# CWBudde/go-pocket-tts

Measured on AMD Instinct MI355X. Metric: synthesized audio sec/sec (xRT), higher is better.
Workload: dtype bf16; 1 GPU; b64_10s_bf16: 64 utterances/GPU x 125 frames (10.0 s each), 25-token prompt + 125-frame voice state, greedy (temperature 0), hipGraph-captured AR step, Mimi decode to 24 kHz PCM written to host; batch_per_gpu=64, frames=125, weights=BF16, kv=bf16, checkpoint=synthetic, shapes of tts_b6369a24 (seed 1234)

## Files before the change

go-pocket-tts_amd/csrc/attn_window.hip:

```cpp
#include <cstdlib>
#include <type_traits>

#include "common.h"
#include "kernels.h"
#include "device_util.h"
#include "mfma_util.h"

namespace ptts {

template <bool KVBF16, bool RAGGED>
__global__ __launch_bounds__(256) void k_attn_window(AttnArgs a, int qtiles) {
    const int lane = threadIdx.x & 63, wave = threadIdx.x >> 6;
    const int h = blockIdx.x;
    const int groups = (qtiles + 3) >> 2;
    const int seg = blockIdx.y / groups, qt = (blockIdx.y % groups) * 4 + wave;
    if (qt >= qtiles) return;
    const int r0 = qt * 32;
    const int seg_row0 = RAGGED ? a.rag_off[seg] : seg * a.rows_per_seg;
    const int seg_rows = RAGGED ? a.rag_off[seg + 1] - seg_row0 : a.rows_per_seg;
    if (r0 >= seg_rows) return;
    const int nq = min(32, seg_rows - r0);
    const int j = lane & 31, half = lane >> 5;
    const int my_q = min(j, nq - 1);
    const int p_first = (RAGGED ? a.rag_pos0[seg] : a.pos_base) + r0, p_last = p_first + nq - 1;
    const int my_pos = p_first + my_q;
    const int ctx = a.context > 0 ? a.context : (1 << 30);
    const int j_lo = max(0, p_first - ctx + 1);
    const RowMap qm{a.q_ld, a.q_rows_per_batch, a.q_batch_stride}, om{a.out_ld, a.o_rows_per_batch, a.o_batch_stride};
    const int row = seg_row0 + r0 + my_q;

    Frag qh[4], ql[4];
    {
        const float* qp = a.q + row_off(qm, row) + a.q_col0 + h * 64 + half * 8;
#pragma unroll
        for (int i = 0; i < 4; i++) {
            const float4 t0 = *reinterpret_cast<const float4*>(qp + 16 * i), t1 = *reinterpret_cast<const float4*>(qp + 16 * i + 4);
            split2(t0.x * 0.125f, t0.y * 0.125f, qh[i].u[0], ql[i].u[0]);
            split2(t0.z * 0.125f, t0.w * 0.125f, qh[i].u[1], ql[i].u[1]);
            split2(t1.x * 0.125f, t1.y * 0.125f, qh[i].u[2], ql[i].u[2]);
            split2(t1.z * 0.125f, t1.w * 0.125f, qh[i].u[3], ql[i].u[3]);
        }
    }
    typedef typename std::conditional<KVBF16, unsigned short, float>::type KvT;
    const KvT* kb = (const KvT*)a.k + (int64_t)seg * a.k_seg_stride + (int64_t)h * a.k_head_stride;
    const KvT* vb = (const KvT*)a.v + (int64_t)seg * a.k_seg_stride + (int64_t)h * a.k_head_stride;
    f32x16 o0, o1;
#pragma unroll
    for (int r = 0; r < 16; r++) { o0[r] = 0.0f; o1[r] = 0.0f; }
    float m = -INFINITY, l = 0.0f;

    for (int kt = j_lo; kt <= p_last; kt += 32) {
        Frag kh[4], kl[4];
        {
            const KvT* kp = kb + (int64_t)min(kt + j, p_last) * a.k_row_stride + half * 8;
            if constexpr (KVBF16) {
#pragma unroll
                for (int i = 0; i < 4; i++) kh[i].q = *reinterpret_cast<const uint4*>(kp + 16 * i);
            } else {
                float4 t[4][2];
#pragma unroll
                for (int i = 0; i < 4; i++) {
                    t[i][0] = *reinterpret_cast<const float4*>(kp + 16 * i);
                    t[i][1] = *reinterpret_cast<const float4*>(kp + 16 * i + 4);
                }
#pragma unroll
                for (int i = 0; i < 4; i++) split8(t[i][0], t[i][1], kh[i], kl[i]);
            }
        }
        float v0[16], v1[16];
#pragma unroll
        for (int r = 0; r < 16; r++) {
            const int key = min(kt + (r & 3) + 8 * (r >> 2) + 4 * half, p_last);
            const KvT* vp = vb + (int64_t)key * a.k_row_stride + j;
            if constexpr (KVBF16) {
                v0[r] = __uint_as_float((unsigned)vp[0] << 16);
                v1[r] = __uint_as_float((unsigned)vp[32] << 16);
            } else {
                v0[r] = vp[0];
                v1[r] = vp[32];
            }
        }
        f32x16 s;
#pragma unroll
        for (int r = 0; r < 16; r++) s[r] = 0.0f;
#pragma unroll
        for (int i = 0; i < 4; i++) {
            s = __builtin_amdgcn_mfma_f32_32x32x16_bf16(kh[i].v, qh[i].v, s, 0, 0, 0);
            if constexpr (!KVBF16) PTTS_LO_MFMA(s = __builtin_amdgcn_mfma_f32_32x32x16_bf16(kl[i].v, qh[i].v, s, 0, 0, 0));
            PTTS_LO_MFMA(s = __builtin_amdgcn_mfma_f32_32x32x16_bf16(kh[i].v, ql[i].v, s, 0, 0, 0));
        }
        float tmax = -INFINITY;
#pragma unroll
        for (int r = 0; r < 16; r++) {
            const int key = kt + (r & 3) + 8 * (r >> 2) + 4 * half;
            const bool ok = key <= my_pos && key > my_pos - ctx;
            s[r] = ok ? s[r] : -INFINITY;
            tmax = fmaxf(tmax, s[r]);
        }
        tmax = fmaxf(tmax, __shfl_xor(tmax, 32, WAVE));
        const float m_new = fmaxf(m, tmax);
        const float m_use = m_new == -INFINITY ? 0.0f : m_new;
        const float alpha = __expf(m - m_use);
        m = m_new;
        l *= alpha;
#pragma unroll
        for (int r = 0; r < 16; r++) { o0[r] *= alpha; o1[r] *= alpha; }
#pragma unroll
        for (int r = 0; r < 16; r++) {
            s[r] = __expf(s[r] - m_use);
            l += s[r];
        }
#pragma unroll
        for (int i = 0; i < 2; i++) {
            Frag ph, pl, vh0, vl0, vh1, vl1;
#pragma unroll
            for (int e = 0; e < 4; e++) {
                split2(s[8 * i + 2 * e], s[8 * i + 2 * e + 1], ph.u[e], pl.u[e]);
                split2(v0[8 * i + 2 * e], v0[8 * i + 2 * e + 1], vh0.u[e], vl0.u[e]);
                split2(v1[8 * i + 2 * e], v1[8 * i + 2 * e + 1], vh1.u[e], vl1.u[e]);
            }
            o0 = __builtin_amdgcn_mfma_f32_32x32x16_bf16(vh0.v, ph.v, o0, 0, 0, 0);
            if constexpr (!KVBF16) PTTS_LO_MFMA(o0 = __builtin_amdgcn_mfma_f32_32x32x16_bf16(vl0.v, ph.v, o0, 0, 0, 0));
            PTTS_LO_MFMA(o0 = __builtin_amdgcn_mfma_f32_32x32x16_bf16(vh0.v, pl.v, o0, 0, 0, 0));
            o1 = __builtin_amdgcn_mfma_f32_32x32x16_bf16(vh1.v, ph.v, o1, 0, 0, 0);
            if constexpr (!KVBF16) PTTS_LO_MFMA(o1 = __builtin_amdgcn_mfma_f32_32x32x16_bf16(vl1.v, ph.v, o1, 0, 0, 0));
            PTTS_LO_MFMA(o1 = __builtin_amdgcn_mfma_f32_32x32x16_bf16(vh1.v, pl.v, o1, 0, 0, 0));
// ... 227 lines not shown
```

go-pocket-tts_amd/csrc/batch.cpp:

```cpp
#include "launch_args.h"

#include <algorithm>
#include <cmath>

namespace ptts {

Batch::~Batch() {
    if (fc_stamps.p) {
        constexpr int kWg = 8 * kFlowClusterMaxTiles;
        std::vector<unsigned long long> h((size_t)kWg * 64);
        if (const char* path = getenv("PTTS_FC_STAMPS"))
            if (hipDeviceSynchronize() == hipSuccess && hipMemcpy(h.data(), fc_stamps.p, h.size() * 8, hipMemcpyDeviceToHost) == hipSuccess)
                if (FILE* f = fopen(path, "a")) {
                    for (int blk = 0; blk < kWg; blk++) {
                        if (!h[(size_t)blk * 64]) continue;
                        fprintf(f, "wg %d:", blk);
                        for (int i = 0; i < 64; i++) fprintf(f, " %llu", h[(size_t)blk * 64 + i]);
                        fprintf(f, "\n");
                    }
                    fprintf(f, "\n");
                    fclose(f);
                }
    }
    drop_graphs();
    if (n_active_pinned) (void)hipHostFree(n_active_pinned);
    if (rows_pinned) (void)hipHostFree(rows_pinned);
}

void Batch::drop_graphs() {
    for (auto& set : graphs) for (auto& row : set) for (hipGraphExec_t& g : row) if (g) { (void)hipGraphExecDestroy(g); g = nullptr; }
    for (auto& gs : graph_steps) gs[0] = gs[1] = 0;
}

Batch* batch_new(Model& m, int n_slots, int cap, int max_steps) {
    if (n_slots <= 0) throw Error(PTTS_EINVAL, "ptts-hip: batch needs at least one slot");
    if (n_slots > kStepMaxRows) throw Error(PTTS_EINVAL, strfmt("ptts-hip: a batch takes at most %d slots (the AR step's kernels), asked for %d", kStepMaxRows, n_slots));
    if (cap <= 0 || cap > ROPE_SEQ) throw Error(PTTS_EINVAL, strfmt("ptts-hip: kv capacity %d outside (0, %d] (RoPE table rows, flow_transformer.go:505)", cap, ROPE_SEQ));
    m.use_device();
    const Desc& d = m.d;
    std::unique_ptr<Batch> b(new Batch());
    b->m = &m;
    b->B = n_slots;
    b->cap = cap;
    b->max_steps = std::max(1, max_steps);
    const size_t B = (size_t)n_slots;
    size_t kvbytes = (size_t)d.n_layers * B * d.heads * cap * d.hd * b->kv_elem();
    b->kcache.ensure(kvbytes);
    b->vcache.ensure(kvbytes);
    PTTS_HIP(hipMemsetAsync(b->kcache.p, 0, kvbytes, m.stream));
    PTTS_HIP(hipMemsetAsync(b->vcache.p, 0, kvbytes, m.stream));
    b->state_i32.ensure((9 * B + 1) * sizeof(int32_t));
    b->state_f32.ensure(B * sizeof(float));
    int32_t* s = b->state_i32.as<int32_t>();
    b->st.kv_len = s; b->st.active = s + B; b->st.step = s + 2 * B; b->st.countdown = s + 3 * B;
    b->st.n_frames = s + 4 * B; b->st.eos_step = s + 5 * B; b->st.max_steps = s + 6 * B;
    b->st.frames_after_eos = s + 7 * B; b->st.broke = s + 8 * B; b->st.n_active = s + 9 * B;
    b->st.eos_threshold = b->state_f32.as<float>();
    b->kv_len_host.assign(B, 0);
    b->pre_k.ensure((size_t)B * sizeof(void*)); b->pre_v.ensure((size_t)B * sizeof(void*)); b->pre_len.ensure((size_t)B * sizeof(int32_t));
    b->pre_k_host.assign(B, nullptr); b->pre_v_host.assign(B, nullptr); b->pre_len_host.assign(B, 0);
    const size_t f = sizeof(float);
    const int NA = d.ada_all.out;
    b->in_raw.ensure(B * d.ldim * f); b->in32.ensure(B * d.ldim * f);
    b->x.ensure(B * d.d_model * f); b->xn.ensure(B * std::max(d.d_model, d.flow_dim) * f);
    b->qkv.ensure(B * 3 * d.d_model * f); b->attn.ensure(B * d.d_model * f);
    b->ff.ensure(B * d.ffn * f); b->last.ensure(B * d.d_model * f); b->eos.ensure(B * f);
    b->sy.ensure(B * d.flow_dim * f); b->ada.ensure(B * NA * f);
    b->fx.ensure(B * d.flow_dim * f); b->fh.ensure(B * d.flow_dim * f); b->fh2.ensure(B * d.flow_dim * f);
    b->cur.ensure(B * d.ldim * f);
    b->partial.ensure((size_t)16 * B * std::max(d.d_model, d.flow_dim) * f);
    b->latents.ensure(B * b->max_steps * d.ldim * f);
    {
        StepFinish sf{b->st, b->eos.as<float>(), b->latents.as<float>(), (int64_t)b->max_steps * d.ldim, (int32_t)d.ldim, StepChain{}};
        StepOpenLinears lin;
        b->chain_ok = open_linears(*b, lin) && step_open_mfma_ok(lin, d.ldim) && ((int64_t)b->max_steps * d.ldim) % 2 == 0 &&
                      (lin.w_bf16 != 0) == (d.final_linear.bf16 != 0 || d.final_linear.wt_i8 != 0);
        b->fx2.ensure(B * d.flow_dim * f); b->cur2.ensure(B * d.ldim * f);
        StepFinish sf2[2] = {sf, sf};
        sf2[0].ch = StepChain{lin.w_in, lin.b_in, lin.x, lin.d_in, lin.w_pj, lin.b_pj, b->fx2.as<float>(), lin.d_pj, m.at<float>(d.bos), b->cur2.as<float>(), lin.w_bf16, b->chain_ok ? 1 : 0};
        sf2[1].ch = StepChain{lin.w_in, lin.b_in, lin.x, lin.d_in, lin.w_pj, lin.b_pj, b->fx.as<float>(), lin.d_pj, m.at<float>(d.bos), b->cur.as<float>(), lin.w_bf16, b->chain_ok ? 1 : 0};
        b->fin_dev.ensure(sizeof sf2);
        h2d(b->fin_dev.p, sf2, sizeof sf2, m.stream);
    }
    {
        const char* sw = getenv("PTTS_FLOW_CLUSTER");
        const bool off = sw && sw[0] == '0';
        bool ok = !off && !m.fc_disabled.load() && d.flow_dim == 512 && d.flow_depth > 0 && d.flow_depth <= FC_MAX_DEPTH && n_slots <= kStepMaxRows &&
                  flow_cluster_fits(n_slots, m.device);
        for (int r = 0; ok && r < d.flow_depth; r++) {
            const auto& rb = d.rb[r];
            for (const Lin* l : {&rb.mlp0, &rb.mlp2}) ok = ok && l->in == 512 && l->out == 512 && l->bf16 && !l->wt_i8 && l->wt != NONE && l->b != NONE;
            ok = ok && rb.ln.w != NONE && rb.ln.b != NONE && rb.ln.d == 512;
        }
        b->fc_ok = ok;
        if (ok) {
            b->fc_xbuf.ensure(flow_cluster_xbuf_bytes(n_slots)); b->fc_sync.ensure(kFlowClusterSyncBytes);
            PTTS_HIP(hipMemsetAsync(b->fc_xbuf.p, 0, flow_cluster_xbuf_bytes(n_slots), m.stream));
            PTTS_HIP(hipMemsetAsync(b->fc_sync.p, 0, kFlowClusterSyncBytes, m.stream));
            if (getenv("PTTS_FC_STAMPS")) { b->fc_stamps.ensure((size_t)8 * kFlowClusterMaxTiles * 64 * 8); PTTS_HIP(hipMemsetAsync(b->fc_stamps.p, 0, (size_t)8 * kFlowClusterMaxTiles * 64 * 8, m.stream)); }
        }
    }
    {
        const char* sw = getenv("PTTS_TALL");
        bool ok = !(sw && sw[0] == '0') && n_slots >= kTallMinRows && (d.d_model == 512 || d.d_model == 1024) && d.ffn % 128 == 0;
        for (int l = 0; ok && l < d.n_layers; l++) {
            const auto& L = d.layers[l];
            for (const Lin* li : {&L.in_proj, &L.l1, &L.l2}) ok = ok && li->bf16 && !li->wt_i8 && li->wt != NONE && li->out % 4 == 0;
            ok = ok && L.in_proj.in == d.d_model && L.l1.in == d.d_model && L.l1.out == d.ffn && L.l2.in == d.ffn && L.l2.out == d.d_model;
            ok = ok && L.n1.w != NONE && L.n1.b != NONE && L.n2.w != NONE && L.n2.b != NONE;
        }
        b->tall_ok = ok;
        if (ok) { b->tp_a.ensure(2 * B * d.d_model * sizeof(uint16_t)); b->tp_f.ensure(2 * B * d.ffn * sizeof(uint16_t)); }
    }
    PTTS_HIP(hipHostMalloc((void**)&b->n_active_pinned, sizeof(int32_t) * (size_t)(2 + 2 * B), hipHostMallocDefault));
    PTTS_HIP(hipHostMalloc((void**)&b->rows_pinned, sizeof(PcmRow) * std::max<size_t>((size_t)B, 1), hipHostMallocDefault));
    batch_reset(*b);
    return b.release();
}

void batch_reset(Batch& b) {
    b.opened = false;
    hipStream_t s = b.m->stream;
    const int B = b.B;
    launch_fill_i32(b.st.kv_len, 0, B, s);
    b.kv_bound = 0;
    PTTS_HIP(hipMemsetAsync(b.latents.p, 0, (size_t)B * b.max_steps * b.m->d.ldim * sizeof(float), s));
    launch_fill_i32(b.st.active, 1, B, s);
    launch_fill_i32(b.st.step, 0, B, s);
    launch_fill_i32(b.st.countdown, -1, B, s);
    launch_fill_i32(b.st.n_frames, 0, B, s);
    launch_fill_i32(b.st.eos_step, -1, B, s);
    launch_fill_i32(b.st.max_steps, 0x7fffffff, B, s);
    launch_fill_i32(b.st.frames_after_eos, 0, B, s);
    launch_fill_i32(b.st.broke, 0, B, s);
    launch_fill_i32(b.st.n_active, B, 1, s);
    std::vector<float> thr((size_t)B, INFINITY);
    h2d(b.st.eos_threshold, thr.data(), thr.size() * sizeof(float), s);
    std::fill(b.kv_len_host.begin(), b.kv_len_host.end(), 0);
    std::fill(b.pre_len_host.begin(), b.pre_len_host.end(), 0);
    launch_fill_i32(b.pre_len.as<int32_t>(), 0, B, s);
    b.has_noise = false;
}

static void check_voice(const Desc& d, const float* const* caches, const int64_t* steps, const int64_t* offsets, int64_t cap) {
    for (int l = 0; l < d.n_layers; l++) {
        if (!caches[l]) throw Error(PTTS_EINVAL, strfmt("native: voice model state module \"transformer.layers.%d.self_attn\" missing cache", l));
        if (offsets[l] < 0) throw Error(PTTS_EINVAL, strfmt("native: voice model state module \"transformer.layers.%d.self_attn\" has negative offset %lld", l, (long long)offsets[l]));
        if (offsets[l] > steps[l]) throw Error(PTTS_EINVAL, strfmt("native: voice model state module \"transformer.layers.%d.self_attn\" offset %lld exceeds cache length %lld", l, (long long)offsets[l], (long long)steps[l]));
        if (offsets[l] != offsets[0]) throw Error(PTTS_EINVAL, "ptts-hip: per-layer voice offsets differ; one offset per utterance is supported");
        if (offsets[l] > cap) throw Error(PTTS_EINVAL, "ptts-hip: voice state longer than the KV capacity");
    }
}

Voice* voice_create(Model& m, const float* const* caches, const int64_t* steps, const int64_t* offsets) {
    const Desc& d = m.d;
    check_voice(d, caches, steps, offsets, ROPE_SEQ);
    std::unique_ptr<Voice> v(new Voice());
    v->m = &m;
    v->device = m.device;
    v->offset = (int)offsets[0];
    const size_t lb = v->layer_bytes();
    v->k.ensure(std::max<size_t>(lb * d.n_layers, 256));
    v->v.ensure(std::max<size_t>(lb * d.n_layers, 256));
    for (int l = 0; l < d.n_layers; l++) {
        size_t n = (size_t)2 * steps[l] * d.heads * d.hd;
        DevBuf& raw = m.work(WORK_VOICE_RAW, n * sizeof(float));
        h2d(raw.p, caches[l], n * sizeof(float), m.stream);
        launch_voice_scatter(raw.as<float>(), (int)steps[l], d.heads, d.hd, v->offset, 0, (char*)v->k.p + lb * l, (char*)v->v.p + lb * l,
                             m.opts.kv == PTTS_KV_BF16, v->offset, m.stream);
        PTTS_HIP(hipStreamSynchronize(m.stream));
    }
    return v.release();
}

bool voice_usable_by(const Voice& v, const Model& m) {
    return v.m == &m || (v.m && v.m->device == m.device && v.m->opts.kv == m.opts.kv && v.m->d.n_layers == m.d.n_layers && v.m->d.heads == m.d.heads &&
                         v.m->d.hd == m.d.hd);
}

void batch_apply_voice(Batch& b, const Voice& v, const std::vector<int32_t>& slots) {
    Model& m = *b.m;
    hipStream_t io = b.io_stream ? b.io_stream : m.stream;
    const Desc& d = m.d;
    if (!voice_usable_by(v, m)) throw Error(PTTS_EINVAL, "ptts-hip: voice belongs to another model");
    if (v.offset > b.cap) throw Error(PTTS_EINVAL, "ptts-hip: voice state longer than the KV capacity");
    DevBuf& ds = m.work(WORK_VOICE_SLOTS, slots.size() * sizeof(int32_t));
    h2d(ds.p, slots.data(), slots.size() * sizeof(int32_t), io);
    const size_t lb = v.layer_bytes();
    for (int l = 0; l < d.n_layers; l++)
        launch_voice_apply((const char*)v.k.p + lb * l, (const char*)v.v.p + lb * l, v.offset, d.heads, d.hd, ds.as<int32_t>(), (int)slots.size(),
                           b.kc(l), b.vc(l), (int)b.kv_elem(), b.cap, io);
    for (int32_t sl : slots) {
        b.kv_len_host[sl] = v.offset;
        b.kv_bound = std::max(b.kv_bound, (int)v.offset);
        b.pre_k_host[sl] = v.k.p; b.pre_v_host[sl] = v.v.p; b.pre_len_host[sl] = v.offset;
    }
    if (b.slot_local) return;
    h2d(b.st.kv_len, b.kv_len_host.data(), (size_t)b.B * sizeof(int32_t), io);
    h2d(b.pre_k.p, b.pre_k_host.data(), (size_t)b.B * sizeof(void*), io);
    h2d(b.pre_v.p, b.pre_v_host.data(), (size_t)b.B * sizeof(void*), io);
    h2d(b.pre_len.p, b.pre_len_host.data(), (size_t)b.B * sizeof(int32_t), io);
}

void batch_set_voice(Batch& b, int slot, const float* const* caches, const int64_t* steps, const int64_t* offsets) {
    Model& m = *b.m;
    hipStream_t io = b.io_stream ? b.io_stream : m.stream;
    const Desc& d = m.d;
    if (slot < 0 || slot >= b.B) throw Error(PTTS_EINVAL, "ptts-hip: voice state slot out of range");
    check_voice(d, caches, steps, offsets, b.cap);
    for (int l = 0; l < d.n_layers; l++) {
        size_t n = (size_t)2 * steps[l] * d.heads * d.hd;
        DevBuf& raw = m.work(WORK_VOICE_RAW, n * sizeof(float));
        h2d(raw.p, caches[l], n * sizeof(float), io);
        launch_voice_scatter(raw.as<float>(), (int)steps[l], d.heads, d.hd, (int)offsets[l], slot, b.kc(l), b.vc(l),
                             m.opts.kv == PTTS_KV_BF16, b.cap, io);
        PTTS_HIP(hipStreamSynchronize(io));
    }
    b.kv_len_host[slot] = (int32_t)offsets[0];
    b.kv_bound = std::max(b.kv_bound, (int)offsets[0]);
    b.pre_len_host[slot] = 0;
    if (b.slot_local) return;
    h2d(b.st.kv_len + slot, &b.kv_len_host[slot], sizeof(int32_t), io);
    h2d(b.pre_len.as<int32_t>() + slot, &b.pre_len_host[slot], sizeof(int32_t), io);
}

void batch_prompt(Batch& b, const float* rows_dev, const int64_t* row_offsets) {
    Model& m = *b.m;
    const Desc& d = m.d;
    hipStream_t s = b.io_stream ? b.io_stream : m.stream;
    const int B = b.B, D = d.d_model;
    const int64_t R64 = row_offsets[B];
    if (R64 == 0) return;
    if (R64 < 0 || R64 > (1 << 24)) throw Error(PTTS_EINVAL, "ptts-hip: prompt row count out of range");
    const int R = (int)R64;
    std::vector<int32_t> off((size_t)B + 1);
    for (int sl = 0; sl < B; sl++) {
        int64_t t = row_offsets[sl + 1] - row_offsets[sl];
        if (t < 0) throw Error(PTTS_EINVAL, "ptts-hip: prompt row offsets must be non-decreasing");
        if (b.kv_len_host[sl] + t > b.cap) throw Error(PTTS_EINVAL, strfmt("ptts-hip: prompt of %lld rows does not fit KV capacity %d (offset %d)", (long long)t, b.cap, b.kv_len_host[sl]));
        off[(size_t)sl] = (int32_t)row_offsets[sl];
    }
    off[(size_t)B] = R;
    const size_t f = sizeof(float);
    const RaggedMeta meta = ragged_meta(off.data(), b.kv_len_host.data(), B);
    int32_t* d_meta = m.work(WORK_PROMPT_META, meta.table.size() * sizeof(int32_t)).as<int32_t>();
    const int32_t* d_slot = meta.row_seg(d_meta);
    const int32_t* d_pos = meta.row_pos(d_meta);
    h2d(d_meta, meta.table.data(), meta.table.size() * sizeof(int32_t), s);
    DevBuf& wsb = m.work(WORK_PROMPT_ACT, ((size_t)R * (size_t)(D + D + 3 * D + D + d.ffn)) * f);
    float* px = wsb.as<float>();
    float* pxn = px + (size_t)R * D;
    float* pqkv = pxn + (size_t)R * D;
    float* pattn = pqkv + (size_t)R * 3 * D;
    float* pff = pattn + (size_t)R * D;
    PTTS_HIP(hipMemcpyAsync(px, rows_dev, (size_t)R * D * f, hipMemcpyDeviceToDevice, s));
    const bool kvb = m.opts.kv == PTTS_KV_BF16;
    PendingSum pend;
    for (int l = 0; l < d.n_layers; l++) {
        const auto& L = d.layers[l];
        {
            LnArgs ln = mkln(m, px, flat(D), L.n1, pxn, D, R);
            ln.pend = pend;
            launch_layernorm(ln, s);
            pend = PendingSum{};
        }
        {
            GemmArgs gq = mk(m, pxn, flat(D), L.in_proj, pqkv, flat(3 * D), R);
            gq.rope_cos = m.at<float>(d.rope_cos); gq.rope_sin = m.at<float>(d.rope_sin);
            gq.rope_cols = 2 * D; gq.rope_hd = d.hd; gq.rope_row_pos = d_pos;
            if (!launch_gemm_rope(gq, s)) {
                gq.rope_cos = gq.rope_sin = nullptr; gq.rope_row_pos = nullptr;
                launch_gemm(gq, s);
                launch_rope_rows(pqkv, flat(3 * D), 0, d.heads, d.hd, d_pos, 0, 0, R, m.at<float>(d.rope_cos), m.at<float>(d.rope_sin), s);
                launch_rope_rows(pqkv, flat(3 * D), D, d.heads, d.hd, d_pos, 0, 0, R, m.at<float>(d.rope_cos), m.at<float>(d.rope_sin), s);
            }
        }
        launch_kv_append(pqkv, 3 * D, D, d.heads, d.hd, d_slot, d_pos, R, b.kc(l), b.vc(l), kvb, b.cap, s);
        if (l == d.n_layers - 1) break;
        launch_attention(attn_ragged_args(kv_layer(b, l), meta, d_meta, pqkv, 3 * D, -1, pattn, D), s);
        GemmArgs go = mk(m, pattn, flat(D), L.out_proj, px, flat(D), R);
        go.R = px; go.epi = EPI_RESADD;
        launch_gemm(go, s);
        launch_layernorm(mkln(m, px, flat(D), L.n2, pxn, D, R), s);
        GemmArgs g1 = mk(m, pxn, flat(D), L.l1, pff, flat(d.ffn), R);
        g1.epi = EPI_GELU;
        launch_gemm(g1, s);
        GemmArgs g2 = mk(m, pff, flat(d.ffn), L.l2, px, flat(D), R);
        const int S = R <= kSkinnyChunkRows ? pick_split(std::min(R, 64), D, d.ffn) : 1;
        GemmArgs g2c = g2;
        g2c.M = std::min(R, 64);
        if (S > 1 && skinny_supported(g2c, S)) {
            DevBuf& pb = m.work(WORK_PREFILL_PLANES, (size_t)S * R * D * f);
            for (int r0 = 0; r0 < R; r0 += 64) {
                g2c = g2;
                g2c.M = std::min(64, R - r0);
                g2c.A = g2.A + (int64_t)r0 * d.ffn;
                g2c.zstride = (int64_t)R * D;
                launch_skinny(g2c, SkinnyFuse{}, S, pb.as<float>() + (size_t)r0 * D, s);
            }
            pend = PendingSum{pb.as<float>(), S, (int64_t)R * D, m.at<float>(L.l2.b)};
        } else {
            GemmArgs gs = g2;
            gs.bias = nullptr; gs.kslice = 1024; gs.zstride = (int64_t)R * D;
            const int Sg = (d.ffn + gs.kslice - 1) / gs.kslice;
            if (R < 16384 && Sg > 1 && Sg <= 8) {
                DevBuf& pb = m.work(WORK_PREFILL_PLANES, (size_t)Sg * R * D * f);
                gs.C = pb.as<float>(); gs.cmap = flat(D);
                if (gemm5_supported(gs) || gemm3_supported(gs)) {
                    if (gemm5_supported(gs)) launch_gemm5(gs, s);
                    else launch_gemm3(gs, s);
                    pend = PendingSum{pb.as<float>(), Sg, (int64_t)R * D, m.at<float>(L.l2.b)};
                    continue;
                }
            }
            g2.R = px; g2.epi = EPI_RESADD;
            launch_gemm(g2, s);
        }
    }
    for (int sl = 0; sl < B; sl++) {
        b.kv_len_host[sl] += (int32_t)(row_offsets[sl + 1] - row_offsets[sl]);
        b.kv_bound = std::max(b.kv_bound, (int)b.kv_len_host[sl]);
    }
    if (!b.slot_local) h2d(b.st.kv_len, b.kv_len_host.data(), (size_t)B * sizeof(int32_t), s);
}

}
```

go-pocket-tts_amd/csrc/capi_hooks.cpp:

```cpp
#include "capi_internal.h"
#include "launch_args.h"
#include "../../include/ptts_debug.h"
#include "scan_block.h"
#include "true_peak.h"

#include <memory>

using namespace ptts;
using namespace ptts::capi;

namespace {

template <class T> class Scoped {
    T& var_;
    T old_;
public:
    Scoped(T& var, T value) : var_(var), old_(var) { var = value; }
    ~Scoped() { var_ = old_; }
    Scoped(const Scoped&) = delete;
    Scoped& operator=(const Scoped&) = delete;
};

using Census = std::map<std::string, int64_t>;

// ... 243 lines not shown
        }
        dsp_windows_device(*h->m, in, n, rows, spec, cuts, n_cuts, out);
    });
}

int ptts_debug_loudness_energies(ptts_model* h, const float* const* in, const int64_t* n, int32_t rows, double* const* out) {
    return guard([&] {
        if (rows < 0 || (rows > 0 && (!in || !n || !out))) throw Error(PTTS_EINVAL, "ptts-hip: loudness: null argument");
        for (int i = 0; i < rows; i++)
            if (n[i] < 0 || (n[i] > 0 && !in[i]) || (n[i] >= kLoudSub && !out[i])) throw Error(PTTS_EINVAL, strfmt("ptts-hip: loudness: row %d is negative or null", i));
        std::vector<std::vector<double>> sub((size_t)rows);
        if (h) {
            if (!h->m) throw Error(PTTS_EINVAL, "native: model is not fully initialized");
            DspSpec spec;
            dsp_spec_loudness(spec, nullptr);
            dsp_rows_device(*h->m, in, n, rows, std::vector<DspSpec>((size_t)rows, spec).data(), false, {nullptr, nullptr, sub.data()});
        } else {
            for (int i = 0; i < rows; i++) loud_sub_energies(in[i], n[i], sub[(size_t)i]);
        }
        for (int i = 0; i < rows; i++)
            if (n[i] >= kLoudSub) std::memcpy(out[i], sub[(size_t)i].data(), (size_t)(n[i] / kLoudSub) * sizeof(double));
    });
}

int ptts_debug_kweighting(int32_t sample_rate, double out[10]) {
    return guard([&] {
        if (!out || sample_rate <= 0) throw Error(PTTS_EINVAL, "ptts-hip: loudness: bad argument");
        loud_kweight_coeffs(sample_rate, out);
    });
}

int64_t ptts_debug_dsp_opts_error(const ptts_dsp_opts* opts, char* out, int64_t cap) {
    const std::string s = opts ? dsp_opts_error(*opts) : std::string();
    put_str(out, cap, s);
    return (int64_t)s.size();
}

int ptts_debug_true_peak_taps(float* out, int32_t* L, int32_t* K, int32_t* dlo) {
    if (L) *L = kTpPhases;
    if (K) *K = kTpTaps;
    if (dlo) *dlo = kTpDlo;
    const TpTaps& t = tp_taps();
    if (out)
        for (int p = 0; p < kTpPhases; p++)
            for (int k = 0; k < kTpTaps; k++) out[p * kTpTaps + k] = t.h[k][p];
    return PTTS_OK;
}

int ptts_debug_true_peak_oversample(const float* samples, int64_t n, float* y) {
    return guard([&] {
        if (n < 0 || (n > 0 && (!samples || !y))) throw Error(PTTS_EINVAL, "ptts-hip: true peak: null argument");
        (void)tp_measure(samples, n, y);
    });
}

int64_t ptts_debug_launch_counts(int32_t on, char* out, int64_t cap) {
    static thread_local Census census;
    const std::string s = census_str(census);
    put_str(out, cap, s);
    census.clear();
    g_launch_census = on ? &census : nullptr;
    return (int64_t)s.size();
}

int ptts_debug_time_skinny(int32_t M, int32_t N, int32_t K, int32_t w_bf16, int32_t splitk, int32_t fuse_ln, int32_t iters, float* avg_us) {
    return guard([&] {
        require_device();
        SkinnyProbe p(M, N, K, w_bf16, splitk, fuse_ln);
        hipEvent_t e0, e1;
        PTTS_HIP(hipEventCreate(&e0)); PTTS_HIP(hipEventCreate(&e1));
        for (int i = 0; i < 5; i++) p.launch(splitk);
        PTTS_HIP(hipDeviceSynchronize());
        PTTS_HIP(hipEventRecord(e0, nullptr));
        for (int i = 0; i < iters; i++) p.launch(splitk);
        PTTS_HIP(hipEventRecord(e1, nullptr));
        PTTS_HIP(hipEventSynchronize(e1));
        float ms = 0;
        PTTS_HIP(hipEventElapsedTime(&ms, e0, e1));
        *avg_us = ms * 1e3f / (float)iters;
        (void)hipEventDestroy(e0); (void)hipEventDestroy(e1);
    });
}

int ptts_debug_skinny_stamps(int32_t M, int32_t N, int32_t K, int32_t w_bf16, int32_t splitk, int32_t fuse_ln, uint64_t* out, int32_t max_blocks,
                             int32_t* n_blocks) {
    return guard([&] {
        require_device();
        SkinnyProbe p(M, N, K, w_bf16, splitk, fuse_ln);
        const int blocks = ((N + 15) / 16) * ((M + 15) / 16) * (splitk > 1 ? splitk : 1);
        Tmp dS((size_t)blocks * 8 * 8);
        PTTS_HIP(hipMemset(dS.p, 0, (size_t)blocks * 64));
        for (int i = 0; i < 3; i++) p.launch(splitk);
        PTTS_HIP(hipDeviceSynchronize());
        {
            Scoped<unsigned long long*> stamped(g_skinny_stamps, dS.as<unsigned long long>());
            p.launch(splitk);
        }
        PTTS_HIP(hipDeviceSynchronize());
        *n_blocks = blocks;
        down(out, dS.p, (size_t)std::min(blocks, max_blocks) * 64);
    });
}

int ptts_debug_step_stamps(ptts_batch* hb, int32_t lsd_steps, uint64_t* out, int64_t cap_blocks, int32_t* desc, int32_t cap_desc, int32_t* n_desc) {
    return guard([&] {
        if (!hb || !hb->b || !out || !desc || !n_desc) throw Error(PTTS_EINVAL, "ptts-hip: null argument");
// ... 894 lines not shown
```

go-pocket-tts_amd/csrc/continuous.cpp:

```cpp
#include <algorithm>
#include <chrono>
#include <cmath>
#include <deque>
#include <map>
#include <mutex>

#include "runtime.h"

namespace ptts {

namespace {
constexpr int kDecoderShare = 2;
constexpr int kDecodeMin = 16;
constexpr int kDecodeSerialFrames = 2400;
constexpr int kDecodeMaxAge = 8;
constexpr int kBandFrames = 16, kBandPercent = 48;

std::mutex g_dec_mu;
std::map<int, std::pair<hipStream_t, int>> g_dec_streams;
hipStream_t decoder_stream_acquire(int device) {
    std::lock_guard<std::mutex> lock(g_dec_mu);
    auto& ent = g_dec_streams[device];
    if (!ent.first) {
        int cus = 0, cur = 0;
// ... 160 lines not shown
        e->dec = decoder_stream_acquire(m.device);
    }
    b.io_stream = e->io;
    for (DevBuf& db : e->adm_dev) db.ensure((size_t)slots * sizeof(SlotAdmit));
    e->stage.ensure((size_t)2 * slots * b.max_steps * m.d.ldim * sizeof(float));
    for (int i = 2 * slots - 1; i >= 0; i--) e->stage_free.push_back(i);
    PTTS_HIP(hipEventCreateWithFlags(&e->ev_steps, hipEventDisableTiming));
    for (hipEvent_t& ev : e->lat_free) PTTS_HIP(hipEventCreateWithFlags(&ev, hipEventDisableTiming));
    for (DevBuf& l : e->lat) l.ensure((size_t)2 * slots * (size_t)max_steps * m.d.ldim * sizeof(float));
    PTTS_HIP(hipHostMalloc((void**)&e->rows_host, sizeof(PcmRow) * ContEngine::kLat * 2 * (size_t)slots, hipHostMallocDefault));
    e->rows_dev.ensure(sizeof(PcmRow) * ContEngine::kLat * 2 * (size_t)slots);
    m.tcomb_for(1);
    { MimiWs w; mimi_setup(m, w, 1, kFramesPerDecode + kFramesPerDecode / 8); }
    m.work(WORK_CONT_PCM, (size_t)(kFramesPerDecode + kFramesPerDecode / 8) * m.d.samples_per_frame * sizeof(float));
    m.work(WORK_EGRESS_S16, (size_t)(kFramesPerDecode + kFramesPerDecode / 8) * m.d.samples_per_frame * sizeof(int16_t));
    m.work(WORK_CONT_RESERVE, (size_t)(kFramesPerDecode + kFramesPerDecode / 8) * m.d.ldim * sizeof(float));
    static const int env_graph = [] { const char* g = getenv("PTTS_GRAPH"); return g ? atoi(g) : -1; }();
    e->use_graph = env_graph >= 0 ? env_graph != 0 : m.opts.use_graph != 0;
    PTTS_HIP(hipStreamSynchronize(m.stream));
    return e.release();
}

void cont_destroy(ContEngine* e) { delete e; }
int cont_free_slots(const ContEngine& e) { return e.free_slots(); }
int cont_busy(const ContEngine& e) { return e.busy(); }
void cont_counts(const ContEngine& e, int64_t* admissions, int64_t* admitted) { *admissions = e.admissions; *admitted = e.admitted; }
void cont_occupancy(const ContEngine& e, int64_t* steps, int64_t* slot_steps) { *steps = e.steps_run; *slot_steps = e.slot_steps; }

bool cont_accepts(const ContEngine& e, const ptts_request& r) {
    if (r.step_callback || r.pcm_callback || r.lsd_steps > 1) return false;
    const int ms = resolve_max_steps(r);
    const int tp = (int)r.n_tokens + (r.voice_embedding ? (int)r.voice_frames : 0);
    const int off = r.voice ? reinterpret_cast<const Voice*>(r.voice)->offset : (r.voice_caches ? (int)r.voice_offsets[0] : 0);
    return ms <= e.max_steps && off + tp + ms <= e.cap && ms <= mimi_frame_limit(e.m.d);
}

void cont_admit(ContEngine& e, const ptts_request* const* reqs, ptts_result* const* results, void* const* tags, int n) {
    struct Timer { ContEngine& e; std::chrono::steady_clock::time_point t0 = std::chrono::steady_clock::now();
                   ~Timer() { e.tr_acc_admit_us += std::chrono::duration<double, std::micro>(std::chrono::steady_clock::now() - t0).count(); } } admit_timer{e};
    if (n <= 0) return;
    e.lock_model();
    Batch& b = *e.b;
    hipStream_t s = e.io;
    const int turn = e.arena_turn;
    e.arena_turn ^= 1;
    UploadScope upload_scope(e.arenas[turn], e.arena_free[turn]);
    std::vector<SlotReq> list((size_t)n);
    for (int i = 0, next = 0; i < n; i++, next++) {
        while (next < e.B && e.slots[(size_t)next].busy) next++;
        if (next >= e.B) throw Error(PTTS_EINVAL, "continuous batch: more requests admitted than free slots");
        list[(size_t)i] = SlotReq{next, reqs[i], resolve_max_steps(*reqs[i])};
        b.kv_len_host[(size_t)next] = 0;
        b.pre_k_host[(size_t)next] = nullptr; b.pre_v_host[(size_t)next] = nullptr; b.pre_len_host[(size_t)next] = 0;
    }
    stage_prompt(b, list, s);
    stage_noise(b, list, s);
    ContEngine::Joining j;
    std::vector<SlotAdmit> adm((size_t)n);
    for (int i = 0; i < n; i++) {
        const ptts_request& r = *reqs[i];
        const int sl = list[(size_t)i].slot;
        adm[(size_t)i] = SlotAdmit{sl, list[(size_t)i].max_steps, r.frames_after_eos, r.eos_threshold, b.kv_len_host[(size_t)sl], b.pre_len_host[(size_t)sl],
                                   b.pre_k_host[(size_t)sl], b.pre_v_host[(size_t)sl]};
        ContEngine::Slot& so = e.slots[(size_t)sl];
        so = ContEngine::Slot{};
        so.busy = true; so.req = reqs[i]; so.res = results[i]; so.tag = tags[i];
        so.ms = list[(size_t)i].max_steps;
        so.base_kv = b.kv_len_host[(size_t)sl];
        so.joining = true;
        j.slots.push_back(sl);
    }
    j.ring = e.adm_turn;
    e.adm_turn = (e.adm_turn + 1) & 3;
    h2d(e.adm_dev[j.ring].p, adm.data(), adm.size() * sizeof(SlotAdmit), s);
    j.ready = e.event();
    j.seq = e.seq;
    PTTS_HIP(hipEventRecord(j.ready, s));
    PTTS_HIP(hipEventRecord(e.arena_free[turn], s));
    e.joining.push_back(std::move(j));
    e.admissions++;
    e.admitted += n;
    e.tr_admitted += n;
    e.last_admit_seq = e.seq;
}

static void activate_ready(ContEngine& e, bool wait) {
    Batch& b = *e.b;
    while (!e.joining.empty()) {
        ContEngine::Joining& j = e.joining.front();
        if (wait) PTTS_HIP(hipEventSynchronize(j.ready));
        else {
            hipError_t q = hipEventQuery(j.ready);
            if (q == hipErrorNotReady) {
                PTTS_HIP(hipStreamWaitEvent(e.m.stream, j.ready, 0));
            } else if (q != hipSuccess) throw Error(PTTS_ENODEVICE, strfmt("hip: hipEventQuery failed: %s", hipGetErrorString(q)));
        }
        launch_slot_admit(b.st, b.pre_len.as<int32_t>(), b.pre_k.as<const void*>(), b.pre_v.as<const void*>(), e.adm_dev[j.ring].as<SlotAdmit>(), (int)j.slots.size(),
                          e.m.stream);
        b.opened = false;
        for (int sl : j.slots) { e.slots[(size_t)sl].joining = false; e.slots[(size_t)sl].admit_seq = e.seq; e.slots[(size_t)sl].seen_seq = e.seq; }
        e.n_gen += (int)j.slots.size();
        e.free_events.push_back(j.ready);
        e.joining.pop_front();
    }
}

static void start_decode(ContEngine& e, std::vector<ContEngine::Staged>& fin) {
    Model& m = e.m;
    Batch& b = *e.b;
// ... 249 lines not shown
```

go-pocket-tts_amd/csrc/generate.cpp:

```cpp
#include "runtime.h"

#include <chrono>

#include <algorithm>
#include <cmath>

namespace ptts {

void stage_prompt(Batch& b, const std::vector<SlotReq>& list, hipStream_t s, hipEvent_t before_prefill) {
    Model& m = *b.m;
    const int D = m.d.d_model;
    std::map<const Voice*, std::vector<int32_t>> by_voice;
    for (const SlotReq& q : list) {
        if (q.req->voice) by_voice[reinterpret_cast<const Voice*>(q.req->voice)].push_back(q.slot);
        else if (q.req->voice_caches) batch_set_voice(b, q.slot, q.req->voice_caches, q.req->voice_cache_steps, q.req->voice_offsets);
    }
    for (auto& kv : by_voice) batch_apply_voice(b, *kv.first, kv.second);
    std::vector<int64_t> row_off((size_t)b.B + 1, 0), ids;
    for (const SlotReq& q : list) {
        row_off[(size_t)q.slot + 1] = q.req->n_tokens + (q.req->voice_embedding ? q.req->voice_frames : 0);
        ids.insert(ids.end(), q.req->tokens, q.req->tokens + q.req->n_tokens);
    }
    for (int sl = 0; sl < b.B; sl++) row_off[(size_t)sl + 1] += row_off[(size_t)sl];
    DevBuf& rows = m.work(WORK_PROMPT_ROWS, (size_t)row_off[(size_t)b.B] * D * sizeof(float));
    DevBuf& dids = m.work(WORK_PROMPT_IDS, ids.size() * sizeof(int64_t));
    h2d(dids.p, ids.data(), ids.size() * sizeof(int64_t), s);
    int64_t id0 = 0, run_id0 = 0, run_n = 0;
    float* run_dst = rows.as<float>();
    auto flush = [&]() {
        if (run_n > 0) launch_embed_gather(m.at<float>(m.d.embed), dids.as<int64_t>() + run_id0, (int)run_n, D, run_dst, s);
        run_n = 0;
    };
    for (const SlotReq& q : list) {
        const ptts_request& r = *q.req;
        float* dst = rows.as<float>() + row_off[(size_t)q.slot] * D;
        const int64_t tv = r.voice_embedding ? r.voice_frames : 0;
        if (tv) {
            flush();
            h2d(dst, r.voice_embedding, (size_t)tv * D * sizeof(float), s);
        }
        if (run_n == 0) { run_id0 = id0; run_dst = dst + tv * D; }
        run_n += r.n_tokens;
        id0 += r.n_tokens;
    }
    flush();
    if (before_prefill) PTTS_HIP(hipEventRecord(before_prefill, s));
    batch_prompt(b, rows.as<float>(), row_off.data());
}

void stage_noise(Batch& b, const std::vector<SlotReq>& list, hipStream_t s) {
    Model& m = *b.m;
    const int ld = m.d.ldim;
    const int64_t slot_rows = (int64_t)b.max_steps * ld;
    float* noise = b.noise.as<float>();
    for (size_t i = 0; i < list.size();) {
        size_t j = i + 1;
        while (j < list.size() && list[j].slot == list[j - 1].slot + 1) j++;
        PTTS_HIP(hipMemsetAsync(noise + list[i].slot * slot_rows, 0, (j - i) * slot_rows * sizeof(float), s));
        i = j;
    }
    std::vector<NoiseSpec> spec((size_t)b.B, NoiseSpec{0, 0.0f, 0});
    int draw_rows = 0;
    for (const SlotReq& q : list) {
        const ptts_request& r = *q.req;
        if (r.noise) h2d(noise + q.slot * slot_rows, r.noise, (size_t)q.max_steps * ld * sizeof(float), s);
        else if (r.temperature > 0.0f) {
            if (ld % 4) throw Error(PTTS_EINVAL, "ptts-hip: the device noise draw needs a latent width that is a multiple of 4");
            spec[(size_t)q.slot] = NoiseSpec{r.noise_seed ? r.noise_seed : m.next_noise_seed(), std::sqrt(r.temperature), q.max_steps};
            draw_rows = std::max(draw_rows, q.max_steps);
        }
    }
    if (draw_rows == 0) return;
    DevBuf& sb = m.work(WORK_NOISE_SPECS, spec.size() * sizeof(NoiseSpec));
    h2d(sb.p, spec.data(), spec.size() * sizeof(NoiseSpec), s);
    launch_noise_fill(sb.as<NoiseSpec>(), b.B, draw_rows, noise, slot_rows, ld, s);
}

const PcmRow* results_alloc(const Model& m, const std::vector<Delivery>& g, PcmRow* host_rows, PcmRow* dev_rows, hipStream_t s) {
    const int64_t spf = m.d.samples_per_frame;
    bool all_pinned = true, converts = false;
    for (size_t i = 0; i < g.size(); i++) {
        if (host_rows) host_rows[i] = PcmRow{nullptr, 0, 0};
        const Delivery& u = g[i];
        if (!u.res || u.filled) continue;
        const int fmt = u.req->pcm_format;
        const bool s16 = fmt == PTTS_PCM_S16;
        const int64_t ns = egress_length(*u.req, u.samples(spf));
        void* p = result_alloc((size_t)std::max<int64_t>(1, ns) * pcm_bytes(fmt));
        set_result_buffer(*u.res, fmt, p);
        if (!p) continue;
        all_pinned = all_pinned && result_is_pinned(p);
        converts = converts || request_converts(*u.req);
        if (host_rows) host_rows[i] = PcmRow{p, (int32_t)std::min<int64_t>(ns, INT32_MAX), s16 ? 1 : 0};
    }
    if (!host_rows || !dev_rows || !all_pinned || converts) return nullptr;
    PTTS_HIP(hipMemcpyAsync(dev_rows, host_rows, g.size() * sizeof(PcmRow), hipMemcpyHostToDevice, s));
    return dev_rows;
}

void results_deliver(Model& m, const std::vector<Delivery>& g, bool stored, const float* pcm, int64_t pcm_stride, const float* lat, int64_t lat_stride,
                     hipStream_t s) {
    const int ld = m.d.ldim;
    const int64_t spf = m.d.samples_per_frame;
    const int64_t n = (int64_t)g.size();
    const int16_t* pcm16 = nullptr;
    std::vector<int64_t> conv;
    if (!stored) {
        std::vector<DspJob> jobs;
        for (int64_t i = 0; i < n; i++) {
            const Delivery& u = g[(size_t)i];
            if (u.res && !u.filled && u.samples(spf) > 0 && (u.req->dsp || u.req->loudness) && result_buffer(*u.res, u.req->pcm_format)) {
                DspJob j{const_cast<float*>(pcm) + i * pcm_stride, u.samples(spf), DspSpec()};
                const std::string e = dsp_resolve(u.req->dsp, &j.spec);
                if (!e.empty()) throw Error(PTTS_EINVAL, "ptts-hip: " + e);
                const double target_lufs = (double)u.req->loudness / 100.0;
                if (u.req->loudness) dsp_spec_loudness(j.spec, &target_lufs);
                if (j.spec.any()) jobs.push_back(j);
            }
        }
        if (!jobs.empty()) dsp_launch(m, jobs, s);
    }
    for (int64_t i = 0; i < n; i++) {
        const Delivery& u = g[(size_t)i];
        if (!u.res) continue;
        ptts_result& r = *u.res;
        const int fmt = u.req->pcm_format;
        r.n_frames = u.nf; r.eos_step = u.eos; r.n_samples = egress_length(*u.req, u.samples(spf));
        const bool s16 = fmt == PTTS_PCM_S16;
// ... 111 lines not shown
    std::chrono::steady_clock::time_point t_last = std::chrono::steady_clock::now();

    ~Chunk() {
        (void)hipStreamSynchronize(m.stream2);
        (void)hipStreamSynchronize(m.stream);
        for (auto& r : stream_ranges) (void)hipHostFree(r->nf);
        for (void* p : stream_host) result_free(p);
    }
    const ptts_request& req(int i) const { return reqs[idx[(size_t)i]]; }
    Error too_long(int frames) const {
        return Error(PTTS_EINVAL, strfmt("generate: mimi_decode: ops: rope cos/sin sequence length too small for pos=0 seq=%lld", (long long)frames * m.d.up_stride));
    }
    void mark(const char* what) {
        static const bool trace = getenv("PTTS_TRACE") != nullptr;
        if (!trace) return;
        (void)hipStreamSynchronize(s);
        (void)hipStreamSynchronize(m.stream2);
        auto now = std::chrono::steady_clock::now();
        fprintf(stderr, "[ptts] %-12s %8.3f ms\n", what, std::chrono::duration<double, std::milli>(now - t_last).count());
        t_last = now;
    }
    hipEvent_t phase_event(int i) {
        if (!m.prof.phases_on) return nullptr;
        if (!m.prof.phase[i]) PTTS_HIP(hipEventCreate(&m.prof.phase[i]));
        return m.prof.phase[i];
    }
    void phase(int i, hipStream_t st) { if (hipEvent_t e = phase_event(i)) PTTS_HIP(hipEventRecord(e, st)); }
    int slot_status(int i, int nf) const { return cancelled[(size_t)i] ? PTTS_ECANCELLED : nf > t_limit ? PTTS_EINVAL : PTTS_OK; }
    void setup(); void decoder_setup(); void ar_loop(); void deliver();
    void deliver_joined(const int32_t* nf, const int32_t* eos);
    void decode_upto(int f1, const PcmRow* rows = nullptr, bool* rows_used = nullptr);
    void decode_rest(int f1, const PcmRow* rows = nullptr, bool* rows_used = nullptr);
    void emit_upto(int f1, bool last = false);
};

void Chunk::setup() {
    int cap_need = 0;
    for (int i = 0; i < B; i++) {
        const ptts_request& r = req(i);
        const int ms = resolve_max_steps(r);
        const int tp = (int)r.n_tokens + (r.voice_embedding ? (int)r.voice_frames : 0);
        const int off = r.voice ? reinterpret_cast<const Voice*>(r.voice)->offset : (r.voice_caches ? (int)r.voice_offsets[0] : 0);
        list.push_back(SlotReq{i, &r, ms});
        cap_need = std::max(cap_need, off + tp + ms);
        ms_max = std::max(ms_max, ms);
    }
    int cap = (cap_need + 63) / 64 * 64;
    if (cap > ROPE_SEQ) throw Error(PTTS_EINVAL, strfmt("ops: rope cos/sin sequence length too small for pos=%d seq=1", cap_need));
    if (!m.cached_batch || m.cached_batch->B != B || m.cached_batch->cap < cap || m.cached_batch->max_steps < ms_max) {
        m.cached_batch.reset();
        m.cached_batch.reset(batch_new(m, B, cap, ms_max));
    }
    b = m.cached_batch.get();
    batch_reset(*b);
    std::vector<int32_t> v_ms((size_t)B), v_fae((size_t)B);
    std::vector<float> v_thr((size_t)B);
    for (int i = 0; i < B; i++) { v_ms[i] = std::min(list[i].max_steps, t_limit + 1); v_fae[i] = req(i).frames_after_eos; v_thr[i] = req(i).eos_threshold; }
    h2d(b->st.max_steps, v_ms.data(), (size_t)B * 4, s);
    h2d(b->st.frames_after_eos, v_fae.data(), (size_t)B * 4, s);
    h2d(b->st.eos_threshold, v_thr.data(), (size_t)B * 4, s);
    mark("setup");
    m.prof.phases = false;
    stage_prompt(*b, list, s, phase_event(0));
    phase(1, s);
    mark("prefill");
    b->has_noise = false;
    for (int i = 0; i < B; i++) b->has_noise |= req(i).noise != nullptr || req(i).temperature > 0.0f;
    if (!b->has_noise) return;
    b->noise.ensure((size_t)B * b->max_steps * ld * sizeof(float));
    stage_noise(*b, list, s);
}

void Chunk::decoder_setup() {
    T = std::min(ms_max, t_limit);
    pcm = &m.work(WORK_PCM, (size_t)B * T * spf * sizeof(float));
    const char* env_chunk = getenv("PTTS_MIMI_CHUNK");
    chunk = env_chunk && atoi(env_chunk) > 0 ? atoi(env_chunk) : 1 << 30;
    for (int i = 0; i < B; i++) streaming |= req(i).pcm_callback != nullptr;
    if (streaming) {
        chunk = 1 << 30;
        bool any_s16 = false;
        for (int i = 0; i < B; i++) {
            const ptts_request& r = req(i);
            if (!r.pcm_callback) continue;
            chunk = std::min(chunk, r.stream_frames > 0 ? (int)r.stream_frames : 12);
            const size_t bytes = (size_t)std::max<int64_t>(1, egress_length(r, (int64_t)list[i].max_steps * spf)) * pcm_bytes(r.pcm_format);
            stream_host[(size_t)i] = result_alloc(bytes);
            if (!stream_host[(size_t)i]) throw Error(PTTS_ENOMEM, "ptts-hip: out of host memory");
            const bool conv = request_converts(r);
            any_s16 |= r.pcm_format == PTTS_PCM_S16 && !conv;
            any_conv |= conv;
            if (conv) stage_row = std::max(stage_row, (bytes + 255) & ~(size_t)255);
        }
        if (any_s16) stream_s16 = &m.work(WORK_STREAM_S16, (size_t)B * T * spf * sizeof(int16_t));
        if (stage_row) stream_stage = m.work(WORK_STREAM_STAGE, stage_row * (size_t)B).as<char>();
    }
    dec_group = (B > kMimiGroup && !streaming && chunk > ms_max) ? kMimiGroup : B;
    mimi_setup(m, mw, dec_group, T);
    mimi_zero_history(m, mw, m.stream2);
}

void Chunk::ar_loop() {
    m.tcomb_for(lsd);
    static const int env_graph = [] { const char* e = getenv("PTTS_GRAPH"); return e ? atoi(e) : -1; }();
    const bool use_graph = (env_graph >= 0 ? env_graph != 0 : m.opts.use_graph != 0) && !m.prof.on;
    bool may_stop = false, any_cb = false, any_cancel_flag = false;
    for (int i = 0; i < B; i++) {
        may_stop |= req(i).eos_threshold < 1e30f;
        any_cb |= req(i).step_callback != nullptr;
        any_cancel_flag |= req(i).cancel != nullptr;
    }
    std::vector<int32_t> act((size_t)B, 1);
    static const int env_gsteps = [] { const char* e = getenv("PTTS_GRAPH_STEPS"); return e ? std::max(1, atoi(e)) : 0; }();
    const int gsteps = (use_graph && !any_cb && !any_cancel_flag && chunk > ms_max) ? (env_gsteps ? env_gsteps : (may_stop ? 5 : 25)) : 1;
    const int ms_loop = std::min(ms_max, t_limit + 1);
    for (int step = 0; step < ms_loop;) {
        int n_cancel = 0;
        for (int i = 0; i < B; i++) {
            const ptts_request& r = req(i);
            if (r.cancel && *r.cancel) cancelled[i] = 1;
            n_cancel += cancelled[i];
        }
        if (n_cancel == B) break;
// ... 595 lines not shown
```

go-pocket-tts_amd/csrc/kernels.h:

```cpp
#pragma once

#include <hip/hip_runtime.h>
#include <atomic>
#include <cstddef>
#include <cstdint>
#include <map>
#include <string>
#include <vector>

#include "deesser.h"
#include "limiter.h"
#include "pitch.h"
#include "tempo.h"
#include "trim.h"

namespace ptts {

struct RowMap {
    int64_t ld = 0;
    int64_t rows_per_batch = 0;
    int64_t batch_stride = 0;
};

enum AOp : int { AOP_NONE = 0, AOP_ELU = 1 };
// ... 436 lines not shown
};
constexpr int kFlowClusterRows = 12;
constexpr int kFlowClusterMaxTiles = (kStepMaxRows + kFlowClusterRows - 1) / kFlowClusterRows;
constexpr size_t kFlowClusterTileBytes = (size_t)2 * 16 * 512 * 8;
constexpr size_t kFlowClusterSyncBytes = (size_t)(32 * kFlowClusterMaxTiles + 32) * 4;
inline size_t flow_cluster_xbuf_bytes(int rows) { return (size_t)((rows + kFlowClusterRows - 1) / kFlowClusterRows) * kFlowClusterTileBytes; }
bool flow_cluster_fits(int rows, int device);
bool flow_cluster_supported(const FlowClusterArgs& a, int C);
void launch_flow_cluster(const FlowClusterArgs& a, hipStream_t stream, hipEvent_t ev0 = nullptr, hipEvent_t ev1 = nullptr);

struct StepState {
    int32_t* kv_len;
    int32_t* active;
    int32_t* step;
    int32_t* countdown;
    int32_t* n_frames;
    int32_t* eos_step;
    int32_t* max_steps;
    int32_t* frames_after_eos;
    float*   eos_threshold;
    int32_t* n_active;
    int32_t* broke;
};
struct StepChain {
    const void* w_in; const float* b_in; float* x; int32_t d_in;
    const void* w_pj; const float* b_pj; float* fx; int32_t d_pj;
    const float* bos; float* x0; int32_t w_bf16; int32_t ok;
};
struct StepFinish {
    StepState s;
    const float* eos_logit;
    float* latents;
    int64_t lat_stride;
    int32_t ldim;
    StepChain ch;
};
struct StepOpenLinears {
    const void* w_in = nullptr; const float* b_in = nullptr; int d_in = 0; float* x = nullptr;
    const void* w_pj = nullptr; const float* b_pj = nullptr; int d_pj = 0; float* fx = nullptr;
    int w_bf16 = 0;
};
bool step_open_mfma_ok(const StepOpenLinears& lin, int ldim);
void launch_step_begin(const StepState& s, const float* latents, int64_t lat_stride, const float* bos, const float* noise, int64_t noise_stride,
                       int ldim, int b, float* in32, float* x0, const StepOpenLinears* lin, hipStream_t stream);
void launch_step_finish(const StepState& s, const float* frame, const float* eos_logit, int ldim, int b, float* latents,
                        int64_t lat_stride, hipStream_t stream);
struct NoiseSpec { uint64_t seed; float sigma; int32_t rows; };
void launch_noise_fill(const NoiseSpec* spec_dev, int n_slots, int max_rows, float* out, int64_t out_stride, int ldim, hipStream_t stream);
struct GatherTable { struct Row { int32_t src_row, dst_off, nf, T; }; Row rows[128]; };
void launch_gather_frames(const GatherTable& t, int n, const float* stage, int64_t row_stride, float* dst, int ld, hipStream_t stream);
void launch_readback_i32(const int32_t* a, int na, const int32_t* b, int nb, int32_t* host, hipStream_t stream);
struct SlotAdmit { int32_t slot, max_steps, frames_after_eos; float eos_threshold; int32_t kv_len, pre_len; const void* pre_k; const void* pre_v; };
void launch_slot_admit(const StepState& s, int32_t* pre_len, const void** pre_k, const void** pre_v, const SlotAdmit* dev, int n, hipStream_t stream);
void launch_slot_retire(const StepState& s, const int32_t* slots_dev, int n, hipStream_t stream);
void launch_fill_i32(int32_t* p, int32_t v, int n, hipStream_t stream);
void launch_add_i32(int32_t* p, const int32_t* inc, int n, hipStream_t stream);

void launch_enc_head(const float* pcm, const void* w, int w_bf16, const float* b, int64_t L, int C, int k, float* out, int64_t ldo, hipStream_t stream);
int enc_ds_splits(int M, int N, int K);
void launch_enc_downsample(const float* A, int64_t lda, const void* W, int w_bf16, const float* bias, int M, int N, int K, float* partial, float* out,
                           hipStream_t stream);

void launch_bct_to_btc(const float* in, int b, int c, int t, float* out, int out_pad_rows, hipStream_t stream);
void launch_btc_to_bct(const float* in, int in_pad_rows, int b, int c, int t, float* out, hipStream_t stream);

}
```

go-pocket-tts_amd/csrc/kernels.hip:

```cpp
#include <cstdlib>
#include "kernels.h"
#include "device_util.h"
#include "gemm_tile.h"
#include "step_open.h"

namespace ptts {

constexpr int GM = 64, GN = 64, GK = 32, GLD = GK + 4;

template <bool WBF16>
__global__ __launch_bounds__(256) void k_gemm(GemmArgs a, int a_vec, int w_vec) {
    __shared__ __attribute__((aligned(16))) float As[GM * GLD];
    __shared__ __attribute__((aligned(16))) float Ws[GN * GLD];
    const int tid = threadIdx.x, lane = tid & 63, wave = tid >> 6;
    const int m0 = blockIdx.y * GM, n0 = blockIdx.x * GN;
    const int wm = wave >> 1, wn = wave & 1;

    int srow[2], sc4[2];
    const float* aptr[2];
    const char* wptr[2];
    bool arow_ok[2], wrow_ok[2];
#pragma unroll
    for (int i = 0; i < 2; i++) {
        int idx = tid + i * 256;
// ... 164 lines not shown
void launch_copy_rows(const float* src, int64_t lds, float* dst, int64_t ldd, int rows, int d, hipStream_t stream) {
    int64_t n = (int64_t)rows * d;
    if (n <= 0) return;
    hipLaunchKernelGGL(k_copy_rows, dim3((unsigned)((n + 255) / 256)), dim3(256), 0, stream, src, lds, dst, ldd, rows, d);
}

__global__ void k_timestep_features(float t, const float* freqs, int nf, float* out) {
    int i = blockIdx.x * blockDim.x + threadIdx.x;
    if (i >= nf) return;
    float arg = t * freqs[i];
    out[i] = (float)cos((double)arg);
    out[nf + i] = (float)sin((double)arg);
}
void launch_timestep_features(float t, const float* freqs, int nf, float* out, hipStream_t stream) {
    hipLaunchKernelGGL(k_timestep_features, dim3((nf + 63) / 64), dim3(64), 0, stream, t, freqs, nf, out);
}

__global__ void k_avg2(const float* a, const float* b, float* y, int n) {
    int i = blockIdx.x * blockDim.x + threadIdx.x;
    if (i < n) y[i] = (a[i] + b[i]) * 0.5f;
}
void launch_avg2(const float* a, const float* b, float* y, int n, hipStream_t stream) {
    hipLaunchKernelGGL(k_avg2, dim3((n + 255) / 256), dim3(256), 0, stream, a, b, y, n);
}

__global__ __launch_bounds__(256) void k_gather_frames(GatherTable t, const float* stage, int64_t row_stride, float* dst, int ld) {
    const GatherTable::Row r = t.rows[blockIdx.x];
    const float4* src = reinterpret_cast<const float4*>(stage + (int64_t)r.src_row * row_stride);
    float4* out = reinterpret_cast<float4*>(dst + r.dst_off);
    const int n_copy = r.nf * ld / 4, n_all = r.T * ld / 4;
    for (int i = threadIdx.x; i < n_all; i += 256) out[i] = i < n_copy ? src[i] : make_float4(0.f, 0.f, 0.f, 0.f);
}
void launch_gather_frames(const GatherTable& t, int n, const float* stage, int64_t row_stride, float* dst, int ld, hipStream_t stream) {
    if (n <= 0) return;
    hipLaunchKernelGGL(k_gather_frames, dim3((unsigned)n), dim3(256), 0, stream, t, stage, row_stride, dst, ld);
}

__global__ void k_readback_i32(const int32_t* a, int na, const int32_t* b, int nb, int32_t* host) {
    const int i = blockIdx.x * blockDim.x + threadIdx.x;
    if (i < na) host[i] = a[i];
    else if (i < na + nb) host[i] = b[i - na];
}
void launch_readback_i32(const int32_t* a, int na, const int32_t* b, int nb, int32_t* host, hipStream_t stream) {
    const int n = na + (b ? nb : 0);
    if (n <= 0) return;
    hipLaunchKernelGGL(k_readback_i32, dim3((unsigned)((n + 255) / 256)), dim3(256), 0, stream, a, na, b, b ? nb : 0, host);
}

__global__ void k_fill_i32(int32_t* p, int32_t v, int n) {
    int i = blockIdx.x * blockDim.x + threadIdx.x;
    if (i < n) p[i] = v;
}
void launch_fill_i32(int32_t* p, int32_t v, int n, hipStream_t stream) {
    hipLaunchKernelGGL(k_fill_i32, dim3((n + 255) / 256), dim3(256), 0, stream, p, v, n);
}
__global__ void k_add_i32(int32_t* p, const int32_t* inc, int n) {
    int i = blockIdx.x * blockDim.x + threadIdx.x;
    if (i < n) p[i] += inc[i];
}
void launch_add_i32(int32_t* p, const int32_t* inc, int n, hipStream_t stream) {
    hipLaunchKernelGGL(k_add_i32, dim3((n + 255) / 256), dim3(256), 0, stream, p, inc, n);
}

__global__ void k_slot_admit(StepState s, int32_t* pre_len, const void** pre_k, const void** pre_v, const SlotAdmit* a, int n) {
    const int i = blockIdx.x * blockDim.x + threadIdx.x;
    if (i >= n) return;
    const int sl = a[i].slot;
    s.kv_len[sl] = a[i].kv_len; pre_len[sl] = a[i].pre_len; pre_k[sl] = a[i].pre_k; pre_v[sl] = a[i].pre_v;
    s.active[sl] = 1; s.step[sl] = 0; s.countdown[sl] = -1; s.n_frames[sl] = 0; s.eos_step[sl] = -1; s.broke[sl] = 0;
    s.max_steps[sl] = a[i].max_steps; s.frames_after_eos[sl] = a[i].frames_after_eos; s.eos_threshold[sl] = a[i].eos_threshold;
    if (i == 0) atomicAdd(s.n_active, n);
}
void launch_slot_admit(const StepState& s, int32_t* pre_len, const void** pre_k, const void** pre_v, const SlotAdmit* dev, int n, hipStream_t stream) {
    if (n > 0) hipLaunchKernelGGL(k_slot_admit, dim3((n + 63) / 64), dim3(64), 0, stream, s, pre_len, pre_k, pre_v, dev, n);
}
__global__ void k_slot_retire(StepState s, const int32_t* slots, int n) {
    const int i = blockIdx.x * blockDim.x + threadIdx.x;
    if (i >= n) return;
    const int sl = slots[i];
    if (s.active[sl]) { s.active[sl] = 0; atomicSub(s.n_active, 1); }
}
void launch_slot_retire(const StepState& s, const int32_t* slots_dev, int n, hipStream_t stream) {
    if (n > 0) hipLaunchKernelGGL(k_slot_retire, dim3((n + 63) / 64), dim3(64), 0, stream, s, slots_dev, n);
}

__global__ void k_rope_rows(float* x, RowMap xmap, int col0, int heads, int hd, const int32_t* pos, int pos_base,
                            int rows_per_seg, int rows, const float* cos_t, const float* sin_t) {
    const int half = hd / 2;
    int64_t i = (int64_t)blockIdx.x * blockDim.x + threadIdx.x;
    int64_t tot = (int64_t)rows * heads * half;
    if (i >= tot) return;
    int j = (int)(i % half);
    int h = (int)((i / half) % heads);
    int r = (int)(i / ((int64_t)half * heads));
    int p = pos ? pos[r] : pos_base + (rows_per_seg ? r % rows_per_seg : r);
    float* v = x + row_off(xmap, r) + col0 + h * hd + 2 * j;
    float a = v[0], b = v[1];
    float c = cos_t[(int64_t)p * half + j], s = sin_t[(int64_t)p * half + j];
    {
#pragma clang fp contract(off)
        v[0] = a * c - b * s;
        v[1] = a * s + b * c;
    }
}
void launch_rope_rows(float* x, RowMap xmap, int col0, int heads, int hd, const int32_t* pos, int pos_base, int rows_per_seg,
                      int rows, const float* cos_t, const float* sin_t, hipStream_t stream) {
    int64_t tot = (int64_t)rows * heads * (hd / 2);
    if (tot <= 0) return;
    hipLaunchKernelGGL(k_rope_rows, dim3((unsigned)((tot + 255) / 256)), dim3(256), 0, stream, x, xmap, col0, heads, hd, pos,
                       pos_base, rows_per_seg, rows, cos_t, sin_t);
}

template <bool KVBF16>
__global__ void k_kv_append(const float* qkv, int64_t ld, int d_model, int heads, int hd, const int32_t* row_slot,
                            const int32_t* row_pos, int rows, void* kc, void* vc, int64_t cap) {
    int64_t i = (int64_t)blockIdx.x * blockDim.x + threadIdx.x;
    int64_t tot = (int64_t)rows * d_model;
    if (i >= tot) return;
    int c = (int)(i % d_model), r = (int)(i / d_model);
    int h = c / hd, e = c % hd;
    int64_t dst = (((int64_t)row_slot[r] * heads + h) * cap + row_pos[r]) * hd + e;
    float kv = qkv[(int64_t)r * ld + d_model + c], vv = qkv[(int64_t)r * ld + 2 * d_model + c];
    if (KVBF16) {
        reinterpret_cast<unsigned short*>(kc)[dst] = f32_to_bf16_bits(kv);
        reinterpret_cast<unsigned short*>(vc)[dst] = f32_to_bf16_bits(vv);
    } else {
        reinterpret_cast<float*>(kc)[dst] = kv;
        reinterpret_cast<float*>(vc)[dst] = vv;
    }
}
void launch_kv_append(const float* qkv, int64_t ld, int d_model, int heads, int hd, const int32_t* row_slot,
                      const int32_t* row_pos, int rows, void* kcache, void* vcache, int kv_bf16, int64_t cap,
                      hipStream_t stream) {
    int64_t tot = (int64_t)rows * d_model;
    if (tot <= 0) return;
    dim3 g((unsigned)((tot + 255) / 256));
    if (kv_bf16) hipLaunchKernelGGL(k_kv_append<true>, g, dim3(256), 0, stream, qkv, ld, d_model, heads, hd, row_slot, row_pos, rows, kcache, vcache, cap);
    else hipLaunchKernelGGL(k_kv_append<false>, g, dim3(256), 0, stream, qkv, ld, d_model, heads, hd, row_slot, row_pos, rows, kcache, vcache, cap);
}

template <bool KVBF16> __device__ __forceinline__ float4 load_kv4(const void* base, int64_t elem_off) {
    if (KVBF16) {
        uint2 raw = *reinterpret_cast<const uint2*>(reinterpret_cast<const unsigned short*>(base) + elem_off);
        return make_float4(__uint_as_float(raw.x << 16), __uint_as_float(raw.x & 0xffff0000u), __uint_as_float(raw.y << 16),
                           __uint_as_float(raw.y & 0xffff0000u));
    }
    return *reinterpret_cast<const float4*>(reinterpret_cast<const float*>(base) + elem_off);
}

template <int WPQ, bool KVBF16>
__global__ __launch_bounds__(256) void k_attention(AttnArgs a) {
    extern __shared__ __attribute__((aligned(16))) float smem[];
    constexpr int QPB = 4 / WPQ;
    const int tid = threadIdx.x, lane = tid & 63, wave = tid >> 6;
    const int qi = wave / WPQ, wq = wave % WPQ;
    const int h = blockIdx.x;
    const int row = blockIdx.y * QPB + qi;
    const bool row_ok = row < a.rows;
    float* sc = smem + (size_t)qi * a.max_keys;
    float* part = smem + (size_t)QPB * a.max_keys + (size_t)qi * WPQ * 64;
    float* qs = smem + (size_t)QPB * a.max_keys + (size_t)QPB * WPQ * 64;

    int seg = 0, pos = -1;
    if (row_ok) {
        seg = a.row_seg ? a.row_seg[row] : (a.rows_per_seg ? row / a.rows_per_seg : row);
        pos = a.seg_len ? a.seg_len[seg] : (a.row_pos ? a.row_pos[row] : a.pos_base + (a.rows_per_seg ? row % a.rows_per_seg : row));
    }
    const bool live = row_ok && (!a.active || a.active[seg]);
    const char* kbase = (const char*)a.k + ((int64_t)seg * a.k_seg_stride + (int64_t)h * a.k_head_stride) * (KVBF16 ? 2 : 4);
    const char* vbase = (const char*)a.v + ((int64_t)seg * a.k_seg_stride + (int64_t)h * a.k_head_stride) * (KVBF16 ? 2 : 4);

    if (a.fused_step) {
        if (live) {
            const float* qr = a.qkv + (int64_t)row * a.qkv_ld + h * 64;
            if (tid < 32) {
                float c = a.cos_t[(int64_t)pos * 32 + tid], s = a.sin_t[(int64_t)pos * 32 + tid];
                float q0 = qr[2 * tid], q1 = qr[2 * tid + 1];
                qs[2 * tid] = q0 * c - q1 * s;
                qs[2 * tid + 1] = q0 * s + q1 * c;
                float k0 = qr[a.d_model + 2 * tid], k1 = qr[a.d_model + 2 * tid + 1];
                float r0 = k0 * c - k1 * s, r1 = k0 * s + k1 * c;
                int64_t dst = (int64_t)pos * 64 + 2 * tid;
                if (KVBF16) {
                    reinterpret_cast<unsigned short*>(const_cast<char*>(kbase))[dst] = f32_to_bf16_bits(r0);
                    reinterpret_cast<unsigned short*>(const_cast<char*>(kbase))[dst + 1] = f32_to_bf16_bits(r1);
                } else {
                    reinterpret_cast<float*>(const_cast<char*>(kbase))[dst] = r0;
                    reinterpret_cast<float*>(const_cast<char*>(kbase))[dst + 1] = r1;
// ... 208 lines not shown
        hipLaunchKernelGGL(k_upsample_dw4, dim3((unsigned)(b * (f1 - f0))), dim3(128), 0, stream, in, w0, w1, bias, t, f0, f1 - f0, c, stride, out, out_pad_rows);
        return;
    }
    hipLaunchKernelGGL(k_upsample_dw, dim3((unsigned)((tot + 255) / 256)), dim3(256), 0, stream, in, w0, w1, bias, b, t, f0, f1, c, stride, out, out_pad_rows);
}

template <bool KVBF16>
__global__ void k_voice_scatter(const float* raw, int t, int heads, int hd, int offset, int slot, void* kc, void* vc, int64_t cap) {
    int64_t i = (int64_t)blockIdx.x * blockDim.x + threadIdx.x;
    int64_t tot = (int64_t)offset * heads * hd;
    if (i >= tot) return;
    int e = (int)(i % hd);
    int h = (int)((i / hd) % heads);
    int step = (int)(i / ((int64_t)hd * heads));
    float kv = raw[((int64_t)step * heads + h) * hd + e];
    float vv = raw[(((int64_t)t + step) * heads + h) * hd + e];
    int64_t dst = (((int64_t)slot * heads + h) * cap + step) * hd + e;
    if (KVBF16) {
        reinterpret_cast<unsigned short*>(kc)[dst] = f32_to_bf16_bits(kv);
        reinterpret_cast<unsigned short*>(vc)[dst] = f32_to_bf16_bits(vv);
    } else {
        reinterpret_cast<float*>(kc)[dst] = kv;
        reinterpret_cast<float*>(vc)[dst] = vv;
    }
}
void launch_voice_scatter(const float* raw, int t, int heads, int hd, int offset, int slot, void* kcache, void* vcache,
                          int kv_bf16, int64_t cap, hipStream_t stream) {
    int64_t tot = (int64_t)offset * heads * hd;
    if (tot <= 0) return;
    dim3 g((unsigned)((tot + 255) / 256));
    if (kv_bf16) hipLaunchKernelGGL(k_voice_scatter<true>, g, dim3(256), 0, stream, raw, t, heads, hd, offset, slot, kcache, vcache, cap);
    else hipLaunchKernelGGL(k_voice_scatter<false>, g, dim3(256), 0, stream, raw, t, heads, hd, offset, slot, kcache, vcache, cap);
}

__global__ void k_voice_apply(const uint4* vk, const uint4* vv, int offset, int heads, int row16, const int32_t* slots, int n_slots,
                              uint4* kc, uint4* vc, int64_t cap) {
    int64_t per_slot = (int64_t)heads * offset * row16;
    int64_t i = (int64_t)blockIdx.x * blockDim.x + threadIdx.x;
    if (i >= per_slot * n_slots) return;
    int si = (int)(i / per_slot);
    int64_t r = i % per_slot;
    int c = (int)(r % row16);
    int row = (int)((r / row16) % offset);
    int h = (int)(r / ((int64_t)row16 * offset));
    int64_t dst = (((int64_t)slots[si] * heads + h) * cap + row) * row16 + c;
    kc[dst] = vk[r];
    vc[dst] = vv[r];
}
void launch_voice_apply(const void* vk, const void* vv, int offset, int heads, int hd, const int32_t* slots, int n_slots,
                        void* kcache, void* vcache, int elem_bytes, int64_t cap, hipStream_t stream) {
    int row16 = hd * elem_bytes / 16;
    int64_t tot = (int64_t)heads * offset * row16 * n_slots;
    if (tot <= 0) return;
    hipLaunchKernelGGL(k_voice_apply, dim3((unsigned)((tot + 255) / 256)), dim3(256), 0, stream, (const uint4*)vk, (const uint4*)vv, offset,
                       heads, row16, slots, n_slots, (uint4*)kcache, (uint4*)vcache, cap);
}

__global__ void k_voice_extract(const uint4* kc, const uint4* vc, int B, int64_t cap, int heads, int row16, const VoiceDst* dst) {
    const VoiceDst o = dst[blockIdx.y];
    const int l = blockIdx.z;
    const int64_t per_layer = (int64_t)heads * o.offset * row16;
    const int64_t i = (int64_t)blockIdx.x * blockDim.x + threadIdx.x;
    if (i >= per_layer) return;
    const int c = (int)(i % row16);
    const int row = (int)((i / row16) % o.offset);
    const int h = (int)(i / ((int64_t)row16 * o.offset));
    const int64_t src = ((((int64_t)l * B + o.slot) * heads + h) * cap + row) * row16 + c;
    reinterpret_cast<uint4*>(o.k)[(int64_t)l * per_layer + i] = kc[src];
    reinterpret_cast<uint4*>(o.v)[(int64_t)l * per_layer + i] = vc[src];
}
void launch_voice_extract(const void* kcache, const void* vcache, int B, int64_t cap, int heads, int hd, int elem_bytes, int n_layers,
                          const VoiceDst* dst_dev, int n_voices, int max_offset, hipStream_t stream) {
    const int row16 = hd * elem_bytes / 16;
    const int64_t per_layer = (int64_t)heads * max_offset * row16;
    if (per_layer <= 0 || n_voices <= 0 || n_layers <= 0) return;
    note_launch("k_voice_extract");
    hipLaunchKernelGGL(k_voice_extract, dim3((unsigned)((per_layer + 255) / 256), (unsigned)n_voices, (unsigned)n_layers), dim3(256), 0, stream,
                       (const uint4*)kcache, (const uint4*)vcache, B, cap, heads, row16, dst_dev);
}

template <bool KVBF16>
__global__ void k_voice_export(const uint4* vk, const uint4* vv, int offset, int heads, int hd, int n_layers, float* out) {
    constexpr int V = KVBF16 ? 8 : 4;
    const int hdv = hd / V;
    const int64_t per_which = (int64_t)offset * heads * hdv;
    const int64_t i = (int64_t)blockIdx.x * blockDim.x + threadIdx.x;
    if (i >= per_which * 2 * n_layers) return;
    const int c = (int)(i % hdv);
    const int h = (int)((i / hdv) % heads);
    const int t = (int)((i / ((int64_t)hdv * heads)) % offset);
    const int which = (int)((i / per_which) % 2);
    const int l = (int)(i / (per_which * 2));
    const int64_t src = ((int64_t)l * heads * offset + (int64_t)h * offset + t) * hdv + c;
    const uint4 q = (which ? vv : vk)[src];
    float4* o = reinterpret_cast<float4*>(out + i * V);
    if (KVBF16) {
        const unsigned w[4] = {q.x, q.y, q.z, q.w};
        #pragma unroll
        for (int j = 0; j < 2; j++)
            o[j] = make_float4(bf16_bits_to_f32((unsigned short)(w[2 * j] & 0xffff)), bf16_bits_to_f32((unsigned short)(w[2 * j] >> 16)),
                               bf16_bits_to_f32((unsigned short)(w[2 * j + 1] & 0xffff)), bf16_bits_to_f32((unsigned short)(w[2 * j + 1] >> 16)));
    } else {
        o[0] = make_float4(__uint_as_float(q.x), __uint_as_float(q.y), __uint_as_float(q.z), __uint_as_float(q.w));
    }
}
void launch_voice_export(const void* vk, const void* vv, int offset, int heads, int hd, int n_layers, int kv_bf16, float* out, hipStream_t stream) {
    const int V = kv_bf16 ? 8 : 4;
// ... 301 lines not shown
```

go-pocket-tts_amd/csrc/launch_args.h:

```cpp
#pragma once

#include <algorithm>

#include "runtime.h"

namespace ptts {

inline RowMap flat(int64_t ld) { return RowMap{ld, 0, 0}; }
inline RowMap seg(int64_t ld, int64_t rows_per_batch, int64_t batch_stride) { return RowMap{ld, rows_per_batch, batch_stride}; }

inline GemmArgs mk(const Model& m, const float* A, RowMap am, const Lin& l, float* C, RowMap cm, int M) {
    GemmArgs g;
    g.A = A; g.amap = am;
    g.W = m.arena + l.w; g.w_bf16 = l.bf16; g.ldw = l.in;
    g.Wt = l.wt == NONE ? nullptr : m.arena + l.wt;
    g.wt_i8 = l.wt_i8; g.wscale = m.at<float>(l.wscale);
    g.bias = m.at<float>(l.b);
    g.C = C; g.cmap = cm;
    g.M = M; g.N = l.out; g.K = l.in;
    return g;
}
inline GemmArgs mk_rows(const Model& m, const float* A, RowMap am, const Lin& l, float* C, RowMap cm, int M) {
    GemmArgs g = mk(m, A, am, l, C, cm, M);
    g.Wt = nullptr;
// ... 10 lines not shown
}

struct KvLayer { const void* k; const void* v; int bf16, heads, cap, hd; };
inline KvLayer kv_layer(const Batch& b, int layer) { return KvLayer{b.kc(layer), b.vc(layer), b.m->opts.kv == PTTS_KV_BF16 ? 1 : 0, b.m->d.heads, b.cap, b.m->d.hd}; }
inline void attn_on_cache(AttnArgs& a, const KvLayer& c) {
    a.k = c.k; a.v = c.v; a.kv_bf16 = c.bf16;
    a.k_seg_stride = (int64_t)c.heads * c.cap * c.hd; a.k_head_stride = (int64_t)c.cap * c.hd; a.k_row_stride = c.hd;
    a.heads = c.heads; a.hd = c.hd;
}

struct StepAttnRows {
    const float* qkv; int64_t qkv_ld; int d_model;
    const float* cos_t; const float* sin_t;
    const int32_t* seg_len; const int32_t* active;
    const void* const* pre_k; const void* const* pre_v; const int32_t* pre_len;
    int rows;
};
inline AttnArgs attn_step_args(const KvLayer& c, const StepAttnRows& r, int layer, int keys_now, float* out, int64_t out_ld) {
    AttnArgs a;
    attn_on_cache(a, c);
    a.seg_len = r.seg_len; a.active = r.active;
    a.context = -1;
    a.out = out; a.out_ld = out_ld;
    a.rows = r.rows; a.max_keys = c.cap;
    a.keys_now = keys_now;
    a.fused_step = 1; a.qkv = r.qkv; a.qkv_ld = r.qkv_ld; a.d_model = r.d_model;
    a.cos_t = r.cos_t; a.sin_t = r.sin_t; a.cap = c.cap;
    a.pre_k = r.pre_k; a.pre_v = r.pre_v; a.pre_len = r.pre_len; a.layer = layer;
    return a;
}

struct RaggedMeta {
    std::vector<int32_t> table;
    int rows = 0, segs = 0, longest = 0, max_pos = 0;
    const int32_t* row_seg(const int32_t* dev) const { return dev; }
    const int32_t* row_pos(const int32_t* dev) const { return dev + rows; }
};
inline RaggedMeta ragged_meta(const int32_t* rag_off, const int32_t* pos0, int segs) {
    RaggedMeta t;
    t.rows = rag_off[segs]; t.segs = segs;
    t.table.resize((size_t)2 * t.rows + 2 * segs + 1);
    int32_t* const row_seg = t.table.data();
    int32_t* const row_pos = row_seg + t.rows;
    for (int s = 0; s < segs; s++) {
        const int n = rag_off[s + 1] - rag_off[s];
        t.longest = std::max(t.longest, n);
        if (n > 0) t.max_pos = std::max(t.max_pos, pos0[s] + n - 1);
        for (int i = 0; i < n; i++) { row_seg[rag_off[s] + i] = s; row_pos[rag_off[s] + i] = pos0[s] + i; }
    }
    std::copy(rag_off, rag_off + segs + 1, row_pos + t.rows);
    std::copy(pos0, pos0 + segs, row_pos + t.rows + segs + 1);
    return t;
}
inline AttnArgs attn_ragged_args(const KvLayer& c, const RaggedMeta& t, const int32_t* meta_dev, const float* q, int64_t q_ld, int context, float* out, int64_t out_ld) {
    AttnArgs a;
    attn_on_cache(a, c);
    a.q = q; a.q_ld = q_ld; a.q_col0 = 0;
    a.row_seg = t.row_seg(meta_dev); a.row_pos = t.row_pos(meta_dev);
    a.rag_off = a.row_pos + t.rows; a.rag_pos0 = a.rag_off + t.segs + 1; a.rag_segs = t.segs; a.rows_per_seg = t.longest;
    a.context = context;
    a.out = out; a.out_ld = out_ld;
    a.rows = t.rows; a.max_keys = t.max_pos + 1;
    return a;
}

inline AttnArgs attn_dense_args(const float* qkv, int64_t ld, int D, int segs, int T1, int t0, int CT, int heads, int hd, int context, float* out, int64_t out_ld) {
    AttnArgs a;
    a.q = qkv + (size_t)t0 * ld; a.q_ld = ld; a.q_col0 = 0; a.q_rows_per_batch = CT; a.q_batch_stride = (int64_t)T1 * ld;
    a.k = qkv + D; a.v = qkv + 2 * D; a.kv_bf16 = 0;
    a.k_seg_stride = (int64_t)T1 * ld; a.k_head_stride = hd; a.k_row_stride = ld;
    a.rows_per_seg = CT; a.pos_base = t0;
    a.context = context;
    a.out = out; a.out_ld = out_ld;
    a.rows = segs * CT; a.heads = heads; a.hd = hd; a.max_keys = std::min(T1, context);
    return a;
}

}
```

go-pocket-tts_amd/csrc/runtime.h:

```cpp
#pragma once

#include <atomic>
#include <functional>
#include <type_traits>

#include "kernels.h"
#include "model.h"
#include "row_ring.h"
#include "dsp_spec.h"
#include "host_rows.h"
#include "join.h"

namespace ptts {

struct DevBuf {
    void* p = nullptr;
    size_t n = 0;
    DevBuf() = default;
    DevBuf(const DevBuf&) = delete;
    DevBuf& operator=(const DevBuf&) = delete;
    ~DevBuf() { release(); }
    void release() {
        if (p) (void)hipFree(p);
        p = nullptr;
// ... 4 lines not shown
        release();
        if (bytes == 0) bytes = 256;
        PTTS_HIP(hipMalloc(&p, bytes));
        n = bytes;
    }
    template <class T> T* as() const { return reinterpret_cast<T*>(p); }
};

struct Batch;

struct PinnedBuf {
    void* p = nullptr;
    size_t n = 0;
    PinnedBuf() = default;
    PinnedBuf(const PinnedBuf&) = delete;
    PinnedBuf& operator=(const PinnedBuf&) = delete;
    ~PinnedBuf() { if (p) (void)hipHostFree(p); }
    void* ensure(size_t bytes) {
        if (bytes <= n && p) return p;
        if (p) (void)hipHostFree(p);
        p = nullptr;
        n = 0;
        PTTS_HIP(hipHostMalloc(&p, std::max<size_t>(bytes, 256), hipHostMallocDefault));
        n = std::max<size_t>(bytes, 256);
        return p;
    }
};

enum WorkSlot : size_t {
    WORK_TCOMB = 0,
    WORK_VOICE_RAW = 1,
    WORK_PROMPT_META = 2,
    WORK_PROMPT_ACT = 3,
    WORK_DECODER = 4,
    WORK_PROMPT_ROWS = 5,
    WORK_TEXT_ROWS = 5,
    WORK_PROMPT_UPLOAD = 5,
    WORK_PROMPT_IDS = 6,
    WORK_TEXT_IDS = 6,
    WORK_PCM = 7,
    WORK_CONT_PCM = 7,
    WORK_STREAM_S16 = 8,
    WORK_EGRESS_S16 = 8,
    WORK_DECODE_IO = 8,
    WORK_SPEAKER_IO = 8,
    WORK_NOISE_ROWS = 8,
    WORK_PREFILL_PLANES = 9,
    WORK_FLOW_DIRECTION = 9,
    WORK_VOICE_SLOTS = 10,
    WORK_PCM_ROWS = 11,
    WORK_NOISE_SPECS = 12,
    WORK_NOISE_ROWS_SPEC = 12,
    WORK_CONT_RESERVE = 13,
    WORK_CONT_RETIRE = 15,
    WORK_ENCODER = 16,
    WORK_ENCODER_LATENTS = 17,
    WORK_EMBEDDING_IO = 17,
    WORK_VOICE_BUILD_ROWS = 18,
    WORK_VOICE_EXPORT = 19,
    WORK_VOICE_BUILD_TABLE = 20,
    WORK_EGRESS_PAGEABLE = 24,
    WORK_CONVERT_IN = 25,
    WORK_CONVERT_OUT = 26,
    WORK_ENCODER_CLIP = 26,
    WORK_STREAM_SNAP = 27,
    WORK_STREAM_STAGE = 28,
    WORK_DSP_SCRATCH = 29,
    WORK_HOST_ROWS = 30,
    WORK_JOINED = 31,
    WORK_TRIMMED = 32,
    WORK_TRIM_SCRATCH = 33,
    WORK_TEMPO = 34,
    WORK_TEMPO_SCRATCH = 35,
    WORK_JOIN_CARRY = 36,
    WORK_JOIN_STAGE = 37,
    WORK_PITCH = 38,
    WORK_FORMANT_COEFFS = 39,
    WORK_FORMANT_RESIDUAL = 40,
    WORK_FORMANT_SHIFTED = 41,
    WORK_PART_LEVEL = 42,
};
constexpr size_t kWorkSlots = 43;

constexpr int kNativeRate = 24000;
constexpr int kResampleMaxL = 512;
constexpr int kResampleMaxTaps = 65536;
struct RateFilter {
    int L = 1, M = 1, K = 0, dlo = 0, tile = 0;
    int64_t A = 0;
    size_t n_taps = 0;
    float* staged = nullptr;
    DevBuf taps;
    hipEvent_t ready = nullptr;
    hipStream_t up = nullptr;
    RateFilter() = default;
    RateFilter(const RateFilter&) = delete;
    RateFilter& operator=(const RateFilter&) = delete;
    ~RateFilter();
};
struct UploadedTable {
    void* staged = nullptr;
    DevBuf image;
    hipEvent_t ready = nullptr;
    hipStream_t up = nullptr;
    UploadedTable() = default;
    UploadedTable(const UploadedTable&) = delete;
// ... 45 lines not shown
    std::unique_ptr<UploadedTable> formant_tables;
    PinnedBuf part_gains;
    PinnedBuf trim_info;
    RowRing<DspRow, kDspMaxEq * kDspEqBytes> dsp_ring;
    int fc_inject = 0;
    std::atomic<int64_t> fc_fallbacks{0};
    std::atomic<bool> fc_disabled{false};

    ~Model();
    template <class T> const T* at(size_t off) const { return off == NONE ? nullptr : reinterpret_cast<const T*>(arena + off); }
    UploadArena upload;
    DevBuf& work(WorkSlot slot, size_t bytes) {
        ws[slot].ensure(bytes);
        return ws[slot];
    }
    static_assert(!std::is_convertible<int, WorkSlot>::value && !std::is_convertible<size_t, WorkSlot>::value, "Model::work takes a WorkSlot name, never a number");
    void use_device() const { PTTS_HIP(hipSetDevice(device)); }
    uint64_t noise_state = 0;
    uint64_t next_noise_seed() {
        uint64_t z = (noise_state += 0x9E3779B97F4A7C15ull);
        z = (z ^ (z >> 30)) * 0xBF58476D1CE4E5B9ull;
        z = (z ^ (z >> 27)) * 0x94D049BB133111EBull;
        z ^= z >> 31;
        return z ? z : 1;
    }
    const float* tcomb_for(int lsd_steps);
    void compute_tcomb(float s, float t, float* dst );
};

struct PackedRows {
    std::vector<size_t> bytes, off;
    char* base = nullptr;
    PackedRows(Model& m, WorkSlot slot, std::vector<size_t> row_bytes, const bool* skip = nullptr) : bytes(std::move(row_bytes)), off(bytes.size()) {
        base = m.work(slot, std::max<size_t>(pack_rows(bytes.data(), skip, (int)bytes.size(), off.data()), kRowAlign)).as<char>();
    }
    char* row(int i) const { return base + off[(size_t)i]; }
    void upload(int i, const void* src, hipStream_t s) const { PTTS_HIP(hipMemcpyAsync(row(i), src, bytes[(size_t)i], hipMemcpyHostToDevice, s)); }
    void download(int i, void* dst, hipStream_t s) const { PTTS_HIP(hipMemcpyAsync(dst, row(i), bytes[(size_t)i], hipMemcpyDeviceToHost, s)); }
};

struct Batch {
    Model* m = nullptr;
    int B = 0;
    int cap = 0;
    int max_steps = 0;
    DevBuf kcache, vcache;
    DevBuf state_i32;
    DevBuf state_f32;
    StepState st{};
    std::vector<int32_t> kv_len_host;
    DevBuf pre_k, pre_v, pre_len;
    std::vector<const void*> pre_k_host, pre_v_host;
    std::vector<int32_t> pre_len_host;
    DevBuf in_raw, in32, x, xn, qkv, attn, ff, last, eos, sy, ada, fx, fh, fh2, cur, noise_step, partial;
    DevBuf latents;
    DevBuf noise;
    bool has_noise = false;
    bool opened = false;
    bool chain_ok = false;
    DevBuf fx2, cur2;
    DevBuf fc_xbuf, fc_sync, fc_stamps;
    bool fc_ok = false;
    DevBuf tp_a, tp_f;
    bool tall_ok = false;
    bool tail_fused = false;
    unsigned* fc_fault() const { return fc_sync.as<unsigned>() + 32 * kFlowClusterMaxTiles; }
    int par = 0;
    float* fx_now() const { return (par ? fx2 : fx).as<float>(); }
    float* cur_now() const { return (par ? cur2 : cur).as<float>(); }
    hipStream_t io_stream = nullptr;
    bool slot_local = false;
    int kv_bound = 0;
    bool capturing = false;
    hipGraphExec_t graphs[2][17][3] = {};
    int graph_steps[2][2] = {{0, 0}, {0, 0}};
    int graph_lsd = 0;
    int capture_keys = 0;
    int32_t* n_active_pinned = nullptr;
    PcmRow* rows_pinned = nullptr;
    DevBuf fin_dev;

    ~Batch();
    void drop_graphs();
    size_t kv_elem() const { return m->opts.kv == PTTS_KV_BF16 ? 2 : 4; }
    void* kc(int layer) const { return (char*)kcache.p + (size_t)layer * B * m->d.heads * cap * m->d.hd * kv_elem(); }
    void* vc(int layer) const { return (char*)vcache.p + (size_t)layer * B * m->d.heads * cap * m->d.hd * kv_elem(); }
};

void* result_alloc(size_t bytes);
void result_free(void* p);
bool result_is_pinned(const void* p);

struct Voice {
    Model* m = nullptr;
    int device = 0;
    int offset = 0;
    DevBuf k, v;
    size_t layer_bytes() const { return (size_t)m->d.heads * offset * m->d.hd * (m->opts.kv == PTTS_KV_BF16 ? 2 : 4); }
};
Voice* voice_create(Model& m, const float* const* caches, const int64_t* steps, const int64_t* offsets);
void batch_apply_voice(Batch& b, const Voice& v, const std::vector<int32_t>& slots);
bool voice_usable_by(const Voice& v, const Model& m);
std::vector<std::unique_ptr<Voice>> voice_build(Model& m, const float* const* emb, const int64_t* frames, int64_t width, int n);
void voice_export(const Voice& v, int layer0, int n_layers, float* out);
void voice_read_state(const Voice& v, int layer, float* out);
std::vector<uint8_t> voice_state_bytes(const Voice& v);

struct MimiWs {
    int B = 0, T = 0, P0 = 0;
    int Ls[4] = {0, 0, 0, 0}, Ps[4] = {0, 0, 0, 0};
    float *xp = nullptr, *up = nullptr, *n1 = nullptr, *qkv[MAX_LAYERS] = {nullptr}, *attn = nullptr, *ff = nullptr, *c0 = nullptr;
    float *u[3] = {nullptr, nullptr, nullptr}, *uo[3] = {nullptr, nullptr, nullptr}, *h[3] = {nullptr, nullptr, nullptr};
    bool zeroed = false;
};
constexpr int kMimiGroup = 64;
void mimi_setup(Model& m, MimiWs& w, int B, int T);
void mimi_range(Model& m, MimiWs& w, const float* lat, int64_t lat_bstride, int f0, int f1, float* pcm, float* mimi_latent, hipStream_t s,
                const PcmRow* pcm_rows = nullptr, bool* rows_used = nullptr, float* xformer_out = nullptr);

void mimi_layer_qkv(Model& m, int layer, const float* x, RowMap xmap, int R, float* qkv, RowMap qmap, int pos0, int rows_per_seg, float* n1, hipStream_t s);
void mimi_layer_ffn(Model& m, int layer, float* x, RowMap xmap, int R, float* n1, float* ffb, hipStream_t s);
void mimi_layer_qkv(Model& m, const Desc::ML& L, const float* x, RowMap xmap, int R, float* qkv, RowMap qmap, int pos0, int rows_per_seg, float* n1, hipStream_t s);
void mimi_layer_ffn(Model& m, const Desc::ML& L, float* x, RowMap xmap, int R, float* n1, float* ffb, hipStream_t s);

constexpr int kEncStages = 10;
int64_t mimi_encode_max_frames(const Desc& d);
void mimi_encode(Model& m, const float* const* pcm, const int64_t* n_samples, int n_clips, float* const* latent_out, float* const* stages = nullptr,
                 const int32_t* rates = nullptr);
int64_t mimi_encode_clip(Model& m, const float* pcm, int64_t n_samples, float* lat_dev, float* const* stages = nullptr, int rate = kNativeRate);
int64_t mimi_encode_samples(int64_t n_samples, int rate);
void require_encoder(const Desc& d);
void mimi_encode_stage_shapes(const Desc& d, int64_t n_samples, int64_t* shapes );
Model* model_open(Plan* plan, void* device_arena, int fill);
void profile_read(Model& m, ptts_profile* out);
Batch* batch_new(Model& m, int n_slots, int cap, int max_steps);
void batch_reset(Batch& b);
void batch_set_voice(Batch& b, int slot, const float* const* caches, const int64_t* steps, const int64_t* offsets);
void batch_prompt(Batch& b, const float* rows_dev, const int64_t* row_offsets);
bool step_core(Batch& b, int lsd_steps, bool opened = false, bool fuse_finish = false, bool chain = false);
void step_open(Batch& b);
struct FlowClusterFault : Error { using Error::Error; };
void flow_cluster_recover(Batch& b);
void flow_cluster_fault(Batch& b);
void step_flow_again(Batch& b, int lsd_steps);
void mimi_decode(Model& m, const float* lat_dev, int64_t lat_bstride, int B, int T, float* pcm_dev, float* mimi_latent_dev, float* xformer_out = nullptr);
struct UploadScope { UploadScope(UploadArena& a, hipStream_t s); UploadScope(UploadArena& a, hipEvent_t last_use); ~UploadScope(); };
void h2d(void* dst, const void* src, size_t bytes, hipStream_t s);
void d2h(void* dst, const void* src, size_t bytes, hipStream_t s);
int resolve_max_steps(const ptts_request& r);
inline int request_lsd(const ptts_request& r) { return r.lsd_steps <= 0 ? 1 : r.lsd_steps; }
inline int mimi_frame_limit(const Desc& d) { return ROPE_SEQ / d.up_stride; }
void enqueue_step(Batch& b, int lsd, bool use_graph, int nsteps = 1);
int pick_split(int M, int N, int K, bool w_bf16 = false);
bool open_linears(Batch& b, StepOpenLinears& lin);
void mimi_zero_history(Model& m, MimiWs& w, hipStream_t s);
struct SlotReq { int slot; const ptts_request* req; int max_steps; };
void stage_prompt(Batch& b, const std::vector<SlotReq>& list, hipStream_t s, hipEvent_t before_prefill = nullptr);
void stage_noise(Batch& b, const std::vector<SlotReq>& list, hipStream_t s);
struct Delivery {
    const ptts_request* req = nullptr;
    ptts_result* res = nullptr;
    int nf = 0, eos = -1;
    bool filled = false;
    int64_t n24 = -1;
    int64_t samples(int64_t spf) const { return n24 >= 0 ? n24 : (int64_t)nf * spf; }
};
const PcmRow* results_alloc(const Model& m, const std::vector<Delivery>& g, PcmRow* host_rows, PcmRow* dev_rows, hipStream_t s);
void results_deliver(Model& m, const std::vector<Delivery>& g, bool stored, const float* pcm, int64_t pcm_stride, const float* lat, int64_t lat_stride,
                     hipStream_t s);
std::string rate_error(int64_t rate, bool input);
std::string rate_pair_error(int in_rate, int out_rate);
int64_t resample_length(int64_t n_in, int in_rate, int out_rate);
const RateFilter* rate_filter(Model& m, int in_rate, int out_rate, hipStream_t s);
int64_t resample_ready(const RateFilter* f, int64_t n_dec);
ResampleRow resample_row(const RateFilter* f, const float* src, int64_t n_in, void* dst, int64_t o0, int64_t o1, int fmt);
void resample_launch(Model& m, const std::vector<ResampleRow>& rows, hipStream_t s);
inline int request_rate(const ptts_request& r) { return r.sample_rate ? r.sample_rate : kNativeRate; }
inline bool request_postprocesses(const ptts_request& r) { return dsp_active(r.dsp) || (r.dsp && r.dsp->ext) || r.loudness != 0; }
inline bool request_converts(const ptts_request& r) {
    return request_rate(r) != kNativeRate || r.pcm_format == PTTS_PCM_ULAW || r.pcm_format == PTTS_PCM_ALAW || request_postprocesses(r);
}
double loud_target_power(double target_lufs);
inline void dsp_spec_loudness(DspSpec& spec, const double* target_lufs) { spec.loud = true; spec.target_power = target_lufs ? loud_target_power(*target_lufs) : 1.0; }
struct DspJob {
    float* x; int64_t n; DspSpec spec; double* loud_out = nullptr; uint32_t* tp_out = nullptr;
    int64_t t0 = 0; bool open = false; int64_t n_row = INT64_MAX; double* carry = nullptr;
};
void dsp_launch(Model& m, std::vector<DspJob>& jobs, hipStream_t s, bool apply = true);
struct DspRowsOut { float* const* out = nullptr; double* M = nullptr; std::vector<double>* sub = nullptr; float* true_peaks = nullptr; };
void dsp_rows_device(Model& m, const float* const* in, const int64_t* n, int32_t rows, const DspSpec* per_row, bool apply, const DspRowsOut& o);
void dsp_windows_device(Model& m, const float* const* in, const int64_t* n, int32_t rows, const DspSpec& spec, const int64_t* cuts, int32_t n_cuts, float* const* out);
inline size_t pcm_bytes(int fmt) { return fmt == PTTS_PCM_F32 ? 4 : fmt == PTTS_PCM_S16 ? 2 : 1; }
inline void* result_buffer(const ptts_result& r, int fmt) {
    return fmt == PTTS_PCM_F32 ? (void*)r.pcm : fmt == PTTS_PCM_S16 ? (void*)r.pcm16 : (void*)r.pcm8;
}
inline void set_result_buffer(ptts_result& r, int fmt, void* p) {
    if (fmt == PTTS_PCM_F32) r.pcm = (float*)p;
    else if (fmt == PTTS_PCM_S16) r.pcm16 = (int16_t*)p;
    else r.pcm8 = (uint8_t*)p;
}
inline int64_t egress_length(const ptts_request& r, int64_t n24) {
    return request_rate(r) == kNativeRate ? n24 : resample_length(n24, kNativeRate, request_rate(r));
}
Model* model_share(Model& base);
Model* model_replicate(Model& base, int device);
void generate(Model& m, const ptts_request* reqs, int n, ptts_result* res);
std::string request_error(const Desc& d, const ptts_request& q);
struct JoinPartsList { const ptts_part_opts* po; float* gains; };
void generate_joined(Model& m, const ptts_request* reqs, int n, const ptts_join_opts& o, const ptts_join_stream_opts* so, ptts_result* out, ptts_join_part* parts,
                     const JoinPartsList* list = nullptr);
void join_launch(Model& m, const std::vector<JoinRow>& rows, hipStream_t s);
void join_rows_device(Model& m, const float* const* in, const int64_t* n, int32_t rows, const JoinLens& l, float* out);
struct PartGain { bool fixed = false; float g = 1.0f; const float* word = nullptr; };
void level_launch(Model& m, const std::vector<const float*>& x, const std::vector<int64_t>& n, const std::vector<double>& target, std::vector<const float*>& words,
                  hipStream_t s);
void join_gain_launch(Model& m, const std::vector<JoinGainRow>& rows, hipStream_t s);
JoinGainRow join_gain_row(const JoinRow& r, const PartGain& mine, const PartGain* prev);
std::vector<PartGain> part_gains_launch(Model& m, const std::vector<const float*>& x, const std::vector<int64_t>& n, const std::vector<PartVolume>& vol, hipStream_t s);
void join_parts_rows_device(Model& m, const float* const* in, const int64_t* n, int32_t rows, const JoinSeams& seams, const std::vector<PartVolume>& vol, float* out,
                            float* gains);
struct PartStages { const TrimScan* trim = nullptr; const PitchScan* pitch = nullptr; const TempoScan* tempo = nullptr; bool formant = false; };
struct PartRow {
    const float* src; int64_t n; PartStages st;
    float* trimmed = nullptr; float* shifted = nullptr; float* scaled = nullptr;
    const float* out = nullptr; int64_t n_out = 0; ptts_trim_info info{};
};
void parts_launch(Model& m, std::vector<PartRow>& rows, hipStream_t s, const std::function<void(const char*)>& phase = nullptr, const char* unit = "row");
void part_rows_device(Model& m, const PartStages* per_row, const float* const* in, const int64_t* n, int32_t rows, float* const* out, int64_t* n_out,
                      ptts_trim_info* info);

void staged_text_embeddings(Model& m, const int64_t* ids, int64_t n, float* out);
void staged_prompt(Batch& b, const float* emb, const int64_t* row_offsets);
void staged_step(Batch& b, const float* frames_in, int lsd_steps, const float* noise, float* frames_out, float* eos_logits, float* last_hidden);
void staged_read_kv(const Batch& b, int slot, int layer, float* k, float* v);
void staged_decode(Model& m, const float* latents, int n_utt, int frames, float* pcm, float* mimi_latent, float* transformer_out);
void staged_noise_rows(Model& m, uint64_t seed, float temperature, int rows, float* out);
void staged_flow_direction(Model& m, const float* c, float sv, float tv, const float* x, int n, float* out);
void staged_convert(Model& m, const float* const* in, const int64_t* n_in, int32_t n, const RateFilter* f, const int64_t* n_out, int fmt, void* const* out);
void speaker_project_device(Model& m, const float* lat, int64_t frames, float* out);
void staged_speaker_project(Model& m, const float* latent, int64_t frames, float* out);
int64_t voice_embedding_device(Model& m, const float* pcm, int64_t n_samples, float* out, int rate = kNativeRate);

struct TextChunk {
    std::string text;
    std::vector<int64_t> token_ids;
    int num_words = 0, max_frames = 0, frames_after_eos = 0;
};
typedef std::function<std::vector<int64_t>(const std::string&)> TextEncodeFn;
int text_count_words(const std::string& s);
int text_estimate_max_frames(int64_t token_count, double frame_rate);
int text_frames_after_eos(int64_t num_words);
std::string text_prepare(const std::string& input);
std::vector<std::string> text_split_sentences(const std::string& text);
std::vector<TextChunk> text_chunks(const std::string& input, const TextEncodeFn& encode, int max_tokens, double frame_rate);

struct Tokenizer;
Tokenizer* tokenizer_from_bytes(const void* data, size_t len);
Tokenizer* tokenizer_from_path(const std::string& path);
std::vector<int64_t> tokenizer_encode(const Tokenizer& t, const std::string& text);
size_t tokenizer_vocab(const Tokenizer& t);
void tokenizer_free(Tokenizer* t);
std::string nfkc_utf8(const std::string& s);

struct VoiceFile {
    StFile st;
    int kind = 0;
    std::vector<float> emb; std::vector<int64_t> emb_shape;
    std::string emb_error;
    struct Tensor { std::vector<int64_t> shape; std::vector<float> data; };
    struct Module { std::string name; std::map<std::string, Tensor> tensors; };
    std::vector<Module> modules;
    std::string state_error;
};
VoiceFile* voice_file_from_path(const std::string& path);
VoiceFile* voice_file_from_bytes(const void* data, size_t len);
void voice_file_embedding(const VoiceFile& v, const float** data, int64_t shape[3]);
void voice_file_require_state(const VoiceFile& v);
void voice_file_state(const VoiceFile& v, int n_layers, int heads, int head_dim, const float** caches, int64_t* steps, int64_t* offsets);
std::vector<uint8_t> voice_state_file(const float* const* caches, int64_t offset, int n_layers, int heads, int head_dim);
std::vector<uint8_t> voice_embedding_file(const float* emb, int64_t frames, int64_t dim);
void write_file(const std::string& path, const std::vector<uint8_t>& bytes);

void dsp_peak_normalize(float* s, int64_t n);
void dsp_dc_block(float* s, int64_t n, int sample_rate);
void dsp_fade_in(float* s, int64_t n, int sample_rate, double ms);
void dsp_fade_out(float* s, int64_t n, int sample_rate, double ms);
struct DspScan;
// ... 41 lines not shown
```

go-pocket-tts_amd/csrc/staged.cpp:

```cpp
#include "launch_args.h"

#include <cmath>
#include <cstring>

namespace ptts {

void staged_text_embeddings(Model& m, const int64_t* ids, int64_t n, float* out) {
    DevBuf& dids = m.work(WORK_TEXT_IDS, (size_t)n * sizeof(int64_t));
    DevBuf& rows = m.work(WORK_TEXT_ROWS, (size_t)n * m.d.d_model * sizeof(float));
    PTTS_HIP(hipMemcpyAsync(dids.p, ids, (size_t)n * sizeof(int64_t), hipMemcpyHostToDevice, m.stream));
    launch_embed_gather(m.at<float>(m.d.embed), dids.as<int64_t>(), (int)n, m.d.d_model, rows.as<float>(), m.stream);
    PTTS_HIP(hipMemcpyAsync(out, rows.p, (size_t)n * m.d.d_model * sizeof(float), hipMemcpyDeviceToHost, m.stream));
    PTTS_HIP(hipStreamSynchronize(m.stream));
}

void staged_prompt(Batch& b, const float* emb, const int64_t* row_offsets) {
    Model& m = *b.m;
    const int64_t R = row_offsets[b.B];
    DevBuf& rows = m.work(WORK_PROMPT_UPLOAD, (size_t)std::max<int64_t>(R, 1) * m.d.d_model * sizeof(float));
    if (R > 0) {
        PTTS_HIP(hipMemcpyAsync(rows.p, emb, (size_t)R * m.d.d_model * sizeof(float), hipMemcpyHostToDevice, m.stream));
        PTTS_HIP(hipStreamSynchronize(m.stream));
    }
    batch_prompt(b, rows.as<float>(), row_offsets);
    PTTS_HIP(hipStreamSynchronize(m.stream));
}

void staged_step(Batch& b, const float* frames_in, int lsd_steps, const float* noise, float* frames_out, float* eos_logits, float* last_hidden) {
    Model& m = *b.m;
    hipStream_t s = m.stream;
    const int B = b.B, ld = m.d.ldim;
    m.tcomb_for(lsd_steps);
    PTTS_HIP(hipMemcpyAsync(b.in_raw.p, frames_in, (size_t)B * ld * sizeof(float), hipMemcpyHostToDevice, s));
    launch_replace_nan(b.in_raw.as<float>(), m.at<float>(m.d.bos), B, ld, b.in32.as<float>(), s);
    if (noise) PTTS_HIP(hipMemcpyAsync(b.cur.p, noise, (size_t)B * ld * sizeof(float), hipMemcpyHostToDevice, s));
    else PTTS_HIP(hipMemsetAsync(b.cur.p, 0, (size_t)B * ld * sizeof(float), s));
    if (b.fc_ok) PTTS_HIP(hipMemcpyAsync(b.cur2.p, b.cur.p, (size_t)B * ld * sizeof(float), hipMemcpyDeviceToDevice, s));
    const bool clustered = b.fc_ok;
    step_core(b, lsd_steps);
    if (clustered) {
        unsigned fault = 0;
        PTTS_HIP(hipMemcpyAsync(&fault, b.fc_fault(), sizeof fault, hipMemcpyDeviceToHost, s));
        PTTS_HIP(hipStreamSynchronize(s));
        if (fault) {
            flow_cluster_recover(b);
            PTTS_HIP(hipMemcpyAsync(b.cur.p, b.cur2.p, (size_t)B * ld * sizeof(float), hipMemcpyDeviceToDevice, s));
            step_flow_again(b, lsd_steps);
        }
    }
    for (int i = 0; i < B; i++) b.kv_len_host[i] += 1;
    PTTS_HIP(hipMemcpyAsync(b.st.kv_len, b.kv_len_host.data(), (size_t)B * sizeof(int32_t), hipMemcpyHostToDevice, s));
    if (frames_out) PTTS_HIP(hipMemcpyAsync(frames_out, b.cur.p, (size_t)B * ld * sizeof(float), hipMemcpyDeviceToHost, s));
    if (eos_logits) PTTS_HIP(hipMemcpyAsync(eos_logits, b.eos.p, (size_t)B * sizeof(float), hipMemcpyDeviceToHost, s));
    if (last_hidden) PTTS_HIP(hipMemcpyAsync(last_hidden, b.last.p, (size_t)B * m.d.d_model * sizeof(float), hipMemcpyDeviceToHost, s));
    PTTS_HIP(hipStreamSynchronize(s));
}

void staged_read_kv(const Batch& b, int slot, int layer, float* k, float* v) {
    const Desc& d = b.m->d;
    const int n = b.kv_len_host[slot];
    const size_t es = b.kv_elem();
    std::vector<uint8_t> tmp((size_t)n * d.hd * es);
    for (int which = 0; which < 2; which++) {
        const char* base = (const char*)(which ? b.vc(layer) : b.kc(layer));
        float* dst = which ? v : k;
        for (int h = 0; h < d.heads; h++) {
            const char* src = base + (((size_t)slot * d.heads + h) * b.cap) * d.hd * es;
            PTTS_HIP(hipMemcpy(tmp.data(), src, tmp.size(), hipMemcpyDeviceToHost));
            float* o = dst + (size_t)h * n * d.hd;
            if (es == 4) std::memcpy(o, tmp.data(), tmp.size());
            else for (size_t i = 0; i < (size_t)n * d.hd; i++) { uint16_t bb; std::memcpy(&bb, tmp.data() + 2 * i, 2); o[i] = bf16_to_f32(bb); }
        }
    }
}

void staged_decode(Model& m, const float* latents, int n_utt, int frames, float* pcm, float* mimi_latent, float* transformer_out) {
    const Desc& d = m.d;
    size_t nl = (size_t)n_utt * frames * d.ldim, np = (size_t)n_utt * frames * d.samples_per_frame, nm = (size_t)n_utt * d.mimi_dim * frames;
    size_t nx = transformer_out ? (size_t)n_utt * frames * d.up_stride * d.mimi_dim : 0;
    DevBuf& io = m.work(WORK_DECODE_IO, (nl + np + nm + nx) * sizeof(float));
    float* dl = io.as<float>();
    float* dp = dl + nl;
    float* dm = dp + np;
    float* dx = dm + nm;
    PTTS_HIP(hipMemcpyAsync(dl, latents, nl * sizeof(float), hipMemcpyHostToDevice, m.stream));
    mimi_decode(m, dl, (int64_t)frames * d.ldim, n_utt, frames, dp, mimi_latent ? dm : nullptr, transformer_out ? dx : nullptr);
    if (pcm) PTTS_HIP(hipMemcpyAsync(pcm, dp, np * sizeof(float), hipMemcpyDeviceToHost, m.stream));
    if (mimi_latent) PTTS_HIP(hipMemcpyAsync(mimi_latent, dm, nm * sizeof(float), hipMemcpyDeviceToHost, m.stream));
    if (transformer_out) PTTS_HIP(hipMemcpyAsync(transformer_out, dx, nx * sizeof(float), hipMemcpyDeviceToHost, m.stream));
    PTTS_HIP(hipStreamSynchronize(m.stream));
}

void staged_noise_rows(Model& m, uint64_t seed, float temperature, int rows, float* out) {
    const int ld = m.d.ldim;
    NoiseSpec sp{seed, temperature > 0.0f ? std::sqrt(temperature) : 0.0f, rows};
    DevBuf& sb = m.work(WORK_NOISE_ROWS_SPEC, sizeof sp);
    DevBuf& ob = m.work(WORK_NOISE_ROWS, (size_t)rows * ld * sizeof(float));
    PTTS_HIP(hipMemcpyAsync(sb.p, &sp, sizeof sp, hipMemcpyHostToDevice, m.stream));
    PTTS_HIP(hipStreamSynchronize(m.stream));
    launch_noise_fill(sb.as<NoiseSpec>(), 1, rows, ob.as<float>(), (int64_t)rows * ld, ld, m.stream);
    PTTS_HIP(hipMemcpyAsync(out, ob.p, (size_t)rows * ld * sizeof(float), hipMemcpyDeviceToHost, m.stream));
    PTTS_HIP(hipStreamSynchronize(m.stream));
}

void staged_flow_direction(Model& m, const float* c, float sv, float tv, const float* x, int B, float* out) {
    const Desc& d = m.d;
    const int C = d.flow_dim, D = d.d_model, NA = d.ada_all.out;
    hipStream_t s = m.stream;
    DevBuf& wsb = m.work(WORK_FLOW_DIRECTION, ((size_t)B * (D + d.ldim + d.ldim + 4 * C + NA) + C) * sizeof(float));
    float* dc = wsb.as<float>();
    float* dx = dc + (size_t)B * D;
    float* dout = dx + (size_t)B * d.ldim;
// ... 90 lines not shown
```

go-pocket-tts_amd/runtime.py:

```python
from __future__ import annotations

import ctypes as C
import os
import subprocess
import sys
from dataclasses import dataclass, field
from typing import Callable, Optional, Sequence

import numpy as np

_HERE = os.path.dirname(os.path.abspath(__file__))
LIB_PATH = os.environ.get("PTTS_LIB_PATH") or os.path.join(_HERE, "libptts_hip.so")

PTTS_OK, PTTS_EINVAL, PTTS_EIO, PTTS_EFORMAT, PTTS_ENODEVICE, PTTS_ECANCELLED, PTTS_ENOMEM = range(7)
WEIGHTS_F32, WEIGHTS_BF16, WEIGHTS_INT8 = 0, 1, 2
KV_F32, KV_BF16 = 0, 1
PCM_F32, PCM_S16, PCM_ULAW, PCM_ALAW = 0, 1, 2, 3
_PCM_DTYPES = {PCM_F32: "<f4", PCM_S16: "<i2", PCM_ULAW: "|u1", PCM_ALAW: "|u1"}

_FP = C.POINTER(C.c_float)
_IP = C.POINTER(C.c_int64)
_DP = C.POINTER(C.c_double)
_I32P = C.POINTER(C.c_int32)
_U16P = C.POINTER(C.c_uint16)
# ... 175 lines not shown


class _Result(C.Structure):
    _fields_ = [("pcm", _FP), ("n_samples", C.c_int64), ("latents", _FP), ("n_frames", C.c_int32), ("eos_step", C.c_int32),
                ("status", C.c_int32), ("pcm16", C.POINTER(C.c_int16)), ("pcm8", C.POINTER(C.c_uint8))]


_RESULT_DTYPE = np.dtype({"names": ["pcm", "n_samples", "latents", "n_frames", "eos_step", "status", "pcm16", "pcm8"],
                          "formats": ["<u8", "<i8", "<u8", "<i4", "<i4", "<i4", "<u8", "<u8"],
                          "offsets": [_Result.pcm.offset, _Result.n_samples.offset, _Result.latents.offset, _Result.n_frames.offset,
                                      _Result.eos_step.offset, _Result.status.offset, _Result.pcm16.offset, _Result.pcm8.offset],
                          "itemsize": C.sizeof(_Result)})

class _VoiceTensor(C.Structure):
    _fields_ = [("data", C.POINTER(C.c_float)), ("count", C.c_int64), ("rank", C.c_int32), ("reserved", C.c_int32), ("shape", C.c_int64 * 8)]


_lib = None

ABI_SYMBOLS = [
    "ptts_default_opts", "ptts_model_open", "ptts_model_open_bytes", "ptts_model_close", "ptts_model_info", "ptts_last_error",
    "ptts_plan_create", "ptts_plan_create_bytes", "ptts_plan_arena_bytes", "ptts_model_open_planned", "ptts_plan_free",
    "ptts_generate", "ptts_free_result", "ptts_text_embeddings", "ptts_batch_new", "ptts_batch_free", "ptts_batch_reset",
    "ptts_batch_set_voice_state", "ptts_batch_prompt", "ptts_batch_step", "ptts_batch_offsets", "ptts_batch_read_kv",
    "ptts_decode_latents", "ptts_noise_rows", "ptts_speaker_project", "ptts_mimi_encode", "ptts_mimi_encode_frames", "ptts_voice_encode_audio", "ptts_flow_direction", "ptts_op_linear", "ptts_op_layernorm", "ptts_op_rope",
    "ptts_op_attention_positions", "ptts_op_conv1d_leftpad", "ptts_op_convtr1d_righttrim", "ptts_version",
        "ptts_voice_create", "ptts_voice_free", "ptts_profile_enable", "ptts_profile_read", "ptts_plan_fill_host", "ptts_wav_header_streaming", "ptts_op_pcm16",
    "ptts_dispatcher_create", "ptts_dispatcher_create_custom", "ptts_dispatch_generate", "ptts_dispatcher_stats", "ptts_dispatcher_close",
    "ptts_model_share", "ptts_model_replicate", "ptts_model_set_use_graph", "ptts_model_set_max_batch", "ptts_text_estimate_max_frames", "ptts_text_frames_after_eos", "ptts_text_prepare", "ptts_text_chunks", "ptts_chunks_count",
    "ptts_chunks_get", "ptts_chunks_free",
    "ptts_tokenizer_open", "ptts_tokenizer_open_bytes", "ptts_tokenizer_free", "ptts_tokenizer_vocab_size", "ptts_tokenizer_encode",
    "ptts_tokenizer_encode_cb", "ptts_text_nfkc", "ptts_rccl_unique_id", "ptts_rccl_broadcast", "ptts_dsp_apply",
    "ptts_voice_file_open", "ptts_voice_file_open_bytes", "ptts_voice_file_close", "ptts_voice_file_kind", "ptts_voice_file_embedding",
    "ptts_voice_file_modules", "ptts_voice_file_module", "ptts_voice_file_state", "ptts_voice_open", "ptts_voice_open_bytes",
    "ptts_voice_from_embeddings", "ptts_voice_from_audio", "ptts_voice_offset", "ptts_voice_read_state", "ptts_voice_write", "ptts_voice_write_bytes",
    "ptts_voice_state_write_bytes", "ptts_voice_embedding_write", "ptts_free_bytes",
    "ptts_resample_length", "ptts_resample", "ptts_pcm_encode", "ptts_mimi_encode_rates", "ptts_voice_from_audio_rates", "ptts_wav_header",
    "ptts_dsp_rows", "ptts_loudness", "ptts_loudness_normalize", "ptts_loudness_rows", "ptts_loudness_normalize_rows",
    "ptts_eq_design", "ptts_eq_response", "ptts_eq_create", "ptts_eq_free", "ptts_eq_apply", "ptts_eq_rows",
    "ptts_dsp_ext_create", "ptts_dsp_ext_free", "ptts_true_peak", "ptts_true_peak_limit", "ptts_true_peak_rows",
    "ptts_dsp_ext_set_compressor", "ptts_compress_gain", "ptts_compress_apply", "ptts_compress_rows",
    "ptts_dsp_ext_set_limiter", "ptts_limit_apply", "ptts_limit_rows",
    "ptts_dsp_ext_set_deesser", "ptts_deess_apply", "ptts_deess_band", "ptts_deess_rows",
    "ptts_join_length", "ptts_join", "ptts_join_rows", "ptts_generate_joined", "ptts_generate_joined_streamed", "ptts_join_stream_ready",
    "ptts_join_parts_length", "ptts_join_parts", "ptts_join_parts_rows", "ptts_join_parts_stream_ready", "ptts_generate_joined_parts",
    "ptts_trim_plan", "ptts_trim_apply", "ptts_trim_rows", "ptts_dsp_ext_set_trim",
    "ptts_tempo_length", "ptts_tempo_plan", "ptts_tempo_apply", "ptts_tempo_rows", "ptts_dsp_ext_set_tempo",
    "ptts_pitch_speed", "ptts_pitch_resample_length", "ptts_pitch_resample", "ptts_pitch_length", "ptts_pitch_apply", "ptts_pitch_table",
    "ptts_pitch_rows", "ptts_dsp_ext_set_pitch",
    "ptts_formant_frames", "ptts_formant_analyse", "ptts_formant_whiten", "ptts_formant_shape", "ptts_formant_apply", "ptts_formant_rows",
    "ptts_dsp_ext_set_formant",
    ]
HOOK_SYMBOLS = [
    "ptts_decode_stages", "ptts_mimi_layer_piece", "ptts_debug_last_attention_kernel", "ptts_debug_launch_counts", "ptts_debug_flow_cluster_inject",
    "ptts_debug_time_skinny", "ptts_debug_skinny_stamps", "ptts_debug_gemm", "ptts_debug_step_stamps", "ptts_debug_tall",
    "ptts_debug_encode_stages", "ptts_debug_resample_launches", "ptts_debug_dsp_blocked_host",
    "ptts_debug_loudness_energies", "ptts_debug_kweighting", "ptts_debug_step_linear", "ptts_debug_true_peak_taps", "ptts_debug_true_peak_oversample",
    "ptts_debug_dsp_opts_error", "ptts_debug_resblock", "ptts_debug_resblock_plan", "ptts_debug_seanet_pack", "ptts_debug_plan_seanet_frags",
    "ptts_debug_gemm_rows", "ptts_debug_attn_step", "ptts_debug_attn_step_rounds", "ptts_debug_attn_window", "ptts_debug_flow_cluster",
    "ptts_debug_mimi_fused", "ptts_debug_mimi_pack", "ptts_debug_dsp_windows", "ptts_debug_step_edge",
]


def build(force: bool = False) -> str:
    args = ["make", "-s", "-C", _HERE, "-j8"]
    if force:
        args.append("-B")
    subprocess.check_call(args)
    return LIB_PATH


def lib():
    global _lib
    if _lib is None:
        if not os.path.exists(LIB_PATH):
            raise PttsError(PTTS_ENODEVICE, f"{LIB_PATH} is missing: run __graft_entry__.build() (no CPU fallback exists)")
        if "torch" not in sys.modules and not os.environ.get("PTTS_NO_TORCH_PRELOAD"):
            try:
                import torch
            except Exception:
                pass
        L = C.CDLL(LIB_PATH)
        L.ptts_last_error.restype = C.c_char_p
        L.ptts_version.restype = C.c_char_p
        L.ptts_plan_arena_bytes.restype = C.c_size_t
        L.ptts_plan_arena_bytes.argtypes = [C.c_void_p]
        L.ptts_plan_free.argtypes = [C.c_void_p]
        L.ptts_model_close.argtypes = [C.c_void_p]
        L.ptts_batch_free.argtypes = [C.c_void_p]
        L.ptts_model_open.argtypes = [C.c_char_p, C.POINTER(_Opts), C.POINTER(C.c_void_p)]
        L.ptts_model_open_bytes.argtypes = [C.c_void_p, C.c_size_t, C.POINTER(_Opts), C.POINTER(C.c_void_p)]
        L.ptts_plan_create.argtypes = [C.c_char_p, C.POINTER(_Opts), C.POINTER(C.c_void_p)]
        L.ptts_plan_create_bytes.argtypes = [C.c_void_p, C.c_size_t, C.POINTER(_Opts), C.POINTER(C.c_void_p)]
        L.ptts_model_open_planned.argtypes = [C.c_void_p, C.c_void_p, C.c_int, C.POINTER(C.c_void_p)]
        L.ptts_plan_fill_host.argtypes = [C.c_void_p, C.c_void_p]
        L.ptts_model_info.argtypes = [C.c_void_p, C.POINTER(_Info)]
        L.ptts_generate.argtypes = [C.c_void_p, C.POINTER(_Request), C.c_int32, C.POINTER(_Result)]
        L.ptts_free_result.argtypes = [C.POINTER(_Result)]
        L.ptts_text_embeddings.argtypes = [C.c_void_p, _IP, C.c_int64, _FP]
        L.ptts_batch_new.argtypes = [C.c_void_p, C.c_int32, C.c_int32, C.POINTER(C.c_void_p)]
        L.ptts_batch_reset.argtypes = [C.c_void_p]
        L.ptts_batch_set_voice_state.argtypes = [C.c_void_p, C.c_int32, C.POINTER(_FP), _IP, _IP]
        L.ptts_batch_prompt.argtypes = [C.c_void_p, _FP, _IP]
        L.ptts_batch_step.argtypes = [C.c_void_p, _FP, C.c_int32, _FP, _FP, _FP, _FP]
        L.ptts_batch_offsets.argtypes = [C.c_void_p, _IP]
        L.ptts_batch_read_kv.argtypes = [C.c_void_p, C.c_int32, C.c_int32, _FP, _FP]
        L.ptts_decode_latents.argtypes = [C.c_void_p, _FP, C.c_int32, C.c_int32, _FP, _FP]
# ... 70 lines not shown
        L.ptts_trim_plan.argtypes = [C.POINTER(TrimOpts), _FP, C.c_int64, C.POINTER(TrimInfo)]
        L.ptts_trim_apply.argtypes = [C.POINTER(TrimOpts), _FP, C.c_int64, _FP, C.POINTER(TrimInfo)]
        L.ptts_trim_rows.argtypes = [C.c_void_p, C.POINTER(C.POINTER(TrimOpts)), C.POINTER(_FP), _IP, C.c_int32, C.POINTER(_FP), C.POINTER(TrimInfo)]
        L.ptts_dsp_ext_set_trim.argtypes = [C.c_void_p, C.POINTER(TrimOpts)]
        L.ptts_tempo_length.argtypes = [C.POINTER(TempoOpts), C.c_int64]
        L.ptts_tempo_length.restype = C.c_int64
        L.ptts_tempo_plan.argtypes = [C.POINTER(TempoOpts), _FP, C.c_int64, C.POINTER(C.c_int32)]
        L.ptts_tempo_apply.argtypes = [C.POINTER(TempoOpts), _FP, C.c_int64, _FP]
        L.ptts_tempo_rows.argtypes = [C.c_void_p, C.POINTER(C.POINTER(TempoOpts)), C.POINTER(_FP), _IP, C.c_int32, C.POINTER(_FP), _IP]
        L.ptts_dsp_ext_set_tempo.argtypes = [C.c_void_p, C.POINTER(TempoOpts)]
        L.ptts_pitch_speed.argtypes = [C.POINTER(PitchOpts), C.POINTER(TempoOpts)]
        L.ptts_pitch_speed.restype = C.c_int32
        L.ptts_pitch_resample_length.argtypes = [C.POINTER(PitchOpts), C.c_int64]
        L.ptts_pitch_resample_length.restype = C.c_int64
        L.ptts_pitch_resample.argtypes = [C.POINTER(PitchOpts), _FP, C.c_int64, _FP]
        L.ptts_pitch_length.argtypes = [C.POINTER(PitchOpts), C.POINTER(TempoOpts), C.c_int64]
        L.ptts_pitch_length.restype = C.c_int64
        L.ptts_pitch_apply.argtypes = [C.POINTER(PitchOpts), C.POINTER(TempoOpts), _FP, C.c_int64, _FP]
        L.ptts_pitch_table.argtypes = [C.POINTER(_FP), C.POINTER(_FP), C.POINTER(C.c_int32)]
        L.ptts_pitch_rows.argtypes = [C.c_void_p, C.POINTER(C.POINTER(PitchOpts)), C.POINTER(C.POINTER(TempoOpts)), C.POINTER(_FP), _IP, C.c_int32,
                                      C.POINTER(_FP), _IP]
        L.ptts_dsp_ext_set_pitch.argtypes = [C.c_void_p, C.POINTER(PitchOpts)]
        L.ptts_formant_frames.argtypes = [C.c_int64]
        L.ptts_formant_frames.restype = C.c_int32
        L.ptts_formant_analyse.argtypes = [_FP, C.c_int64, _FP]
        L.ptts_formant_whiten.argtypes = [_FP, _FP, C.c_int64, _FP]
        L.ptts_formant_shape.argtypes = [_FP, C.c_int64, C.c_int32, _FP, C.c_int64, _FP]
        L.ptts_formant_apply.argtypes = [C.POINTER(FormantOpts), C.POINTER(PitchOpts), C.POINTER(TempoOpts), _FP, C.c_int64, _FP]
        L.ptts_formant_rows.argtypes = [C.c_void_p, C.POINTER(C.POINTER(FormantOpts)), C.POINTER(C.POINTER(PitchOpts)), C.POINTER(C.POINTER(TempoOpts)),
                                        C.POINTER(_FP), _IP, C.c_int32, C.POINTER(_FP), _IP]
        L.ptts_dsp_ext_set_formant.argtypes = [C.c_void_p, C.POINTER(FormantOpts)]
        L.ptts_loudness_rows.argtypes = [C.c_void_p, C.POINTER(_FP), _IP, C.c_int32, _DP]
        L.ptts_loudness_normalize_rows.argtypes = [C.c_void_p, C.POINTER(_FP), _IP, C.c_int32, C.c_double, C.POINTER(_FP), _DP]
        L.ptts_mimi_encode_rates.argtypes = [C.c_void_p, C.POINTER(_FP), _IP, C.POINTER(C.c_int32), C.c_int32, C.POINTER(_FP)]
        L.ptts_voice_from_audio_rates.argtypes = [C.c_void_p, C.POINTER(_FP), _IP, C.POINTER(C.c_int32), C.c_int32, C.POINTER(C.c_void_p)]
        L.ptts_wav_header.argtypes = [C.c_void_p, C.c_int32, C.c_int32, C.c_int32, C.c_int64]
        _lib = L
    return _lib


HOOKS_PATH = os.path.join(_HERE, "libptts_hooks.so")
_hooks = None


def hooks():
    global _hooks
    if _hooks is None:
        lib()
        if not os.path.exists(HOOKS_PATH):
            raise PttsError(PTTS_ENODEVICE, f"{HOOKS_PATH} is missing: run __graft_entry__.build()")
        H = C.CDLL(HOOKS_PATH, mode=C.RTLD_GLOBAL)
        H.ptts_decode_stages.argtypes = [C.c_void_p, _FP, C.c_int32, C.c_int32, _FP, _FP, _FP]
        H.ptts_debug_last_attention_kernel.restype = C.c_char_p
        H.ptts_debug_launch_counts.restype = C.c_int64
        H.ptts_debug_launch_counts.argtypes = [C.c_int32, C.c_char_p, C.c_int64]
        H.ptts_mimi_layer_piece.argtypes = [C.c_void_p, C.c_int32, C.c_int32, _FP, C.c_int64, C.c_int32, C.c_int32, _FP]
        H.ptts_debug_flow_cluster_inject.argtypes = [C.c_void_p, C.c_int32]
        H.ptts_debug_loudness_energies.argtypes = [C.c_void_p, C.POINTER(_FP), _IP, C.c_int32, C.POINTER(_DP)]
        H.ptts_debug_dsp_windows.argtypes = [C.c_void_p, C.POINTER(_FP), _IP, C.c_int32, C.POINTER(DspOpts), _IP, C.c_int32, C.POINTER(_FP)]
        H.ptts_debug_dsp_opts_error.restype = C.c_int64
        H.ptts_debug_dsp_opts_error.argtypes = [C.POINTER(DspOpts), C.c_char_p, C.c_int64]
        for name, args in (("flow_cluster", _FlowClusterArgs), ("step_linear", _StepLinearArgs), ("step_edge", _StepEdgeArgs), ("attn_step", _AttnStepArgs), ("attn_window", _AttnWindowArgs),
                           ("gemm_rows", _GemmRowsArgs), ("mimi_fused", _MimiFusedArgs), ("resblock", _ResblockArgs)):
            getattr(H, "ptts_debug_" + name).argtypes = [C.POINTER(args)]
        _hooks = H
    return _hooks


def _check(rc: int):
    if rc != PTTS_OK:
        msg = lib().ptts_last_error().decode(errors="replace")
        raise (Cancelled if rc == PTTS_ECANCELLED else PttsError)(rc, msg)


def _f32(a) -> np.ndarray:
    return np.ascontiguousarray(np.asarray(a, dtype=np.float32))


def _row_ptrs(arrays, ptr=_FP):
    return (ptr * max(len(arrays), 1))(*[C.cast(a.ctypes.data, ptr) for a in arrays])


def _rows_in(x):
    single = not isinstance(x, (list, tuple))
    rows = [_f32(x).reshape(-1)] if single else [_f32(r).reshape(-1) for r in x]
    return single, rows, len(rows), _row_ptrs(rows), np.array([r.size for r in rows] or [0], np.int64)


def _tempo_size(r, t):
    return r.size if t is None else r.size * 1000 // min(max(int(t.speed_permille), 500), 2000)


def _fp(a: Optional[np.ndarray]):
    return C.cast(a.ctypes.data, _FP) if a is not None else None


def _ip(a: np.ndarray):
    return C.cast(a.ctypes.data, _IP)


class _Keep:

    def __init__(self):
        self.arrays = []

    def _ptr(self, a, dtype, ptr):
# ... 771 lines not shown
        mod = state.modules.get(name)
        if mod is None:
            raise PttsError(PTTS_EINVAL, f'native: voice model state missing module "{name}"')
        if "cache" not in mod:
            raise PttsError(PTTS_EINVAL, f'native: voice model state module "{name}" missing cache')
        if "offset" not in mod:
            raise PttsError(PTTS_EINVAL, f'native: voice model state module "{name}" missing offset')
        c = _f32(mod["cache"])
        if c.ndim != 5 or c.shape[0] != 2:
            raise PttsError(PTTS_EINVAL, f'native: voice model state module "{name}" cache shape {list(c.shape)}, want [2,B,T,H,D]')
        if c.shape[1] != 1:
            raise PttsError(PTTS_EINVAL, f'native: voice model state module "{name}" batch {c.shape[1]}, want 1')
        if c.shape[3] != 16 or c.shape[4] != 64:
            raise PttsError(PTTS_EINVAL, f'native: voice model state module "{name}" heads {c.shape[3]}, want 16')
        off = np.asarray(mod["offset"], np.float32).reshape(-1)
        if off.size == 0:
            raise PttsError(PTTS_EINVAL, f'native: voice model state module "{name}" has empty offset tensor')
        if np.float32(int(off[0])) != off[0]:
            raise PttsError(PTTS_EINVAL, f'native: voice model state module "{name}" offset {off[0]} is not an integer')
        caches.append(c)
        steps.append(c.shape[2])
        offs.append(int(off[0]))
    ptrs = (_FP * n_layers)(*[_fp(c) for c in caches])
    return ptrs, np.array(steps, np.int64), np.array(offs, np.int64), caches


class Batch:

    def __init__(self, model: Model, n_slots: int, kv_capacity: int):
        self.model, self.n = model, n_slots
        h = C.c_void_p()
        _check(lib().ptts_batch_new(model.h, n_slots, kv_capacity, C.byref(h)))
        self.h = h.value

    def close(self):
        if self.h:
            lib().ptts_batch_free(self.h)
            self.h = None

    def __del__(self):
        if sys is None or sys.is_finalizing():
            return
        try:
            self.close()
        except Exception:
            pass

    def reset(self):
        _check(lib().ptts_batch_reset(self.h))

    def set_voice_state(self, slot: int, state: VoiceModelState):
        ptrs, steps, offs, arrs = _voice_arrays(state, self.model.info.n_layers)
        _check(lib().ptts_batch_set_voice_state(self.h, slot, ptrs, _ip(steps), _ip(offs)))

    def prompt(self, embs: Sequence[np.ndarray]):
        d = self.model.info.d_model
        rows = [_f32(e).reshape(-1, d) for e in embs]
        offs = np.zeros(self.n + 1, np.int64)
        offs[1:] = np.cumsum([r.shape[0] for r in rows])
        cat = np.concatenate(rows, 0) if offs[-1] else np.zeros((0, d), np.float32)
        cat = np.ascontiguousarray(cat)
        _check(lib().ptts_batch_prompt(self.h, _fp(cat), _ip(offs)))

    def step(self, frames_in, lsd_steps: int = 1, noise=None):
        m = self.model.info
        fi = _f32(frames_in).reshape(self.n, m.ldim)
        nz = _f32(noise).reshape(self.n, m.ldim) if noise is not None else None
        fo = np.empty((self.n, m.ldim), np.float32)
        eos = np.empty(self.n, np.float32)
        last = np.empty((self.n, m.d_model), np.float32)
        _check(lib().ptts_batch_step(self.h, _fp(fi), lsd_steps, _fp(nz), _fp(fo), _fp(eos), _fp(last)))
        return fo, eos, last

    def offsets(self) -> np.ndarray:
        o = np.zeros(self.n, np.int64)
        _check(lib().ptts_batch_offsets(self.h, _ip(o)))
        return o

    def read_kv(self, slot: int, layer: int):
        n = int(self.offsets()[slot])
        k = np.empty((self.model.info.n_heads, n, 64), np.float32)
        v = np.empty_like(k)
        _check(lib().ptts_batch_read_kv(self.h, slot, layer, _fp(k), _fp(v)))
        return k, v


class Runtime:

    def __init__(self, model: Model):
        self.model = model

    def generate_audio(self, tokens: Sequence[int], cfg: RuntimeGenerateConfig) -> np.ndarray:
        if self.model is None or self.model.h is None:
            raise PttsError(PTTS_EINVAL, "native-safetensors runtime unavailable")
        return self.model.generate_batch([tokens], [cfg])[0].pcm

    def generate(self, tokens: Sequence[int], cfg: RuntimeGenerateConfig) -> GenerateResult:
        if self.model is None or self.model.h is None:
            raise PttsError(PTTS_EINVAL, "native-safetensors runtime unavailable")
        return self.model.generate_batch([tokens], [cfg])[0]

    def mimi_timing(self) -> tuple[float, float, int]:
        i = self.model.info
        return i.frame_rate, i.encoder_frame_rate, i.steps_per_latent

    def close(self):
# ... 1358 lines not shown
```

include/ptts_debug.h:

```cpp
#ifndef PTTS_DEBUG_H
#define PTTS_DEBUG_H

#include "ptts.h"

#ifdef __cplusplus
extern "C" {
#endif

#define PTTS_MIMI_PIECE_QKV 0
#define PTTS_MIMI_PIECE_FFN 1
int  ptts_mimi_layer_piece(ptts_model* m, int32_t layer, int32_t which, const float* x, int64_t rows, int32_t pos0, int32_t rows_per_seg, float* out);

int  ptts_decode_stages(ptts_model* m, const float* latents, int32_t n_utt, int32_t frames,
                        float* pcm, float* mimi_latent, float* transformer_out);

int  ptts_debug_encode_stages(ptts_model* m, const float* pcm, int64_t n_samples, float* const* stages, int64_t* shapes);

int ptts_debug_time_skinny(int32_t M, int32_t N, int32_t K, int32_t w_bf16, int32_t splitk, int32_t fuse_ln, int32_t iters, float* avg_us);
int ptts_debug_skinny_stamps(int32_t M, int32_t N, int32_t K, int32_t w_bf16, int32_t splitk, int32_t fuse_ln, uint64_t* out ,
                             int32_t max_blocks, int32_t* n_blocks);
int ptts_debug_step_stamps(ptts_batch* b, int32_t lsd_steps, uint64_t* out , int64_t cap_blocks, int32_t* desc ,
                           int32_t cap_desc, int32_t* n_desc);
int ptts_debug_gemm(int32_t M, int32_t N, int32_t K, int32_t w_bf16, int32_t variant, int32_t epi, int32_t iters, float* avg_us,
                    float* maxdiff);
// ... 52 lines not shown
    const void* pre_k[4];
    const void* pre_v[4];
    int32_t pre_rows[4];
    void *k, *v;
    float* out;
    char* kernel;
    int32_t* info;
} ptts_attn_step_args;
int ptts_debug_attn_step(const ptts_attn_step_args* a);
int ptts_debug_attn_step_rounds(int32_t keys, int32_t kv_bf16, int32_t* keys_per_round);

typedef struct ptts_attn_window_args {
    int32_t form, ragged, kv_bf16, heads, segs, context, T1, t0, CT, cap, rows, reserved;
    int64_t ld, out_ld, kernel_cap, launched_cap;
    const float* qkv;
    const void *k, *v;
    const int32_t *rag_off, *rag_pos0;
    float* out;
    char *kernel, *launched;
} ptts_attn_window_args;
int ptts_debug_attn_window(const ptts_attn_window_args* a);

typedef struct ptts_gemm_rows_args {
    int32_t M, N, K, ldw, w_bf16, aop, epi, kernel, cfg, rgl, r_in_c, ldg, rope_cols, rope_hd, rope_pos0, rope_rows_per_seg, n_pos, kslice, win_taps, win_c;
    float alpha;
    int32_t reserved;
    int64_t a_elems, a_ld, a_rows_per_batch, a_batch_stride, a_off, c_elems, c_ld, c_rows_per_batch, c_batch_stride, c_off, zstride, launched_cap;
    const float *A, *W, *bias, *addvec, *scale, *gate, *R, *rope_cos, *rope_sin;
    const int32_t* rope_row_pos;
    float* C;
    char* launched;
    int32_t* info;
} ptts_gemm_rows_args;
int ptts_debug_gemm_rows(const ptts_gemm_rows_args* a);

typedef struct ptts_resblock_args {
    int32_t B, L, t0, t1, C, H, pad, slack, w_bf16, final_conv, form, grid, fuse_up, x_pad, x_L, x_slack;
    const float *u, *w1, *w2, *wf, *b1, *b2, *bf, *xin, *wup, *bup;
    const int32_t* rows;
    float *uo, *pcm;
    uint8_t* row_out;
    int64_t row_bytes;
    int32_t* launched;
} ptts_resblock_args;
int ptts_debug_resblock(const ptts_resblock_args* a);
int ptts_debug_resblock_plan(int32_t C, int32_t final_conv, int32_t w_bf16, int32_t fuse_up, int32_t B, int32_t rows, int32_t form, int32_t grid, int32_t cus,
                             int32_t* out);
int ptts_debug_seanet_pack(int32_t kind, const float* rm, int32_t out, int32_t in, uint16_t* hi, uint16_t* lo);
int ptts_debug_plan_seanet_frags(ptts_plan* p, int32_t item, uint16_t* hi, uint16_t* lo, int64_t cap, int64_t* count, int32_t* dims);

const char* ptts_debug_last_attention_kernel(void);

int64_t ptts_debug_launch_counts(int32_t on, char* out, int64_t cap);
int64_t ptts_debug_resample_launches(int32_t reset);

int ptts_debug_dsp_blocked_host(const float* in, int64_t n, float* out);

int ptts_debug_dsp_windows(ptts_model* m, const float* const* in, const int64_t* n, int32_t rows, const ptts_dsp_opts* opts,
                           const int64_t* cuts, int32_t n_cuts, float* const* out);

int ptts_debug_loudness_energies(ptts_model* m, const float* const* in, const int64_t* n, int32_t rows, double* const* out);
int ptts_debug_kweighting(int32_t sample_rate, double out[10]);

int ptts_debug_flow_cluster_inject(ptts_model* m, int32_t block);

typedef struct ptts_flow_cluster_args {
    int32_t rows, depth, n_launch, in_place;
    uint32_t tag_base0;
    int32_t reserved;
    int64_t ldmod, launched_cap;
    const float *fx, *ada, *ln_w, *ln_b, *b0, *b2, *eps, *w0, *w2;
    const int32_t* launch_rows;
    float *out, *fx_back;
    uint32_t* state;
    char* launched;
} ptts_flow_cluster_args;
int ptts_debug_flow_cluster(const ptts_flow_cluster_args* a);

typedef struct ptts_mimi_fused_args {
    int32_t kind, M, D, F, n_pos, rope_cols, pos0, rows_per_seg, ls_off, reserved;
    float eps, reserved_f;
    int64_t x_elems, x_ld, x_rows_per_batch, x_batch_stride, x_off, y_elems, y_ld, y_rows_per_batch, y_batch_stride, y_off, launched_cap;
    const float *x, *ln_w, *ln_b, *w1, *w2, *ls, *rope_cos, *rope_sin;
    float* out;
    char* launched;
} ptts_mimi_fused_args;
int ptts_debug_mimi_fused(const ptts_mimi_fused_args* a);
int ptts_debug_mimi_pack(int32_t kind, const float* w1, const float* w2, int32_t n, uint16_t* dst);

int64_t ptts_debug_dsp_opts_error(const ptts_dsp_opts* opts, char* out, int64_t cap);
int ptts_debug_true_peak_taps(float* out , int32_t* L, int32_t* K, int32_t* dlo);
int ptts_debug_true_peak_oversample(const float* samples, int64_t n, float* y );

#ifdef __cplusplus
}
#endif
#endif
```

Before: 12800 x real-time.

## Read voice prefix KV in place during prefill instead of copying into slots

Prompt prefill attention now reads the shared voice-state KV prefix directly from the voice buffers through per-slot prefix pointers, instead of first copying the prefix into every slot's KV cache. The copy is deferred and only materialised when needed (eager mode, unsupported attention, or reading KV back). Prompt metadata and prefix tables are packed into one host-to-device upload, and the first layer reads prompt rows directly rather than via a device copy. This removes per-slot, per-layer voice copies and some small transfers during admission. In exchange, the attention kernel takes a branch per key, and decode steps after prefill must still see the prefix correctly.

```diff
diff --git a/go-pocket-tts_amd/csrc/attn_window.hip b/go-pocket-tts_amd/csrc/attn_window.hip
--- a/go-pocket-tts_amd/csrc/attn_window.hip
+++ b/go-pocket-tts_amd/csrc/attn_window.hip
@@ -44,6 +44,16 @@
     typedef typename std::conditional<KVBF16, unsigned short, float>::type KvT;
     const KvT* kb = (const KvT*)a.k + (int64_t)seg * a.k_seg_stride + (int64_t)h * a.k_head_stride;
     const KvT* vb = (const KvT*)a.v + (int64_t)seg * a.k_seg_stride + (int64_t)h * a.k_head_stride;
+    int pre = 0;
+    const KvT* pk = kb;
+    const KvT* pv = vb;
+    if constexpr (RAGGED) {
+        if (a.pre_len && (pre = a.pre_len[seg]) > 0) {
+            const int64_t po = ((int64_t)a.layer * a.heads + h) * pre * 64;
+            pk = (const KvT*)a.pre_k[seg] + po;
+            pv = (const KvT*)a.pre_v[seg] + po;
+        }
+    }
     f32x16 o0, o1;
 #pragma unroll
     for (int r = 0; r < 16; r++) { o0[r] = 0.0f; o1[r] = 0.0f; }
@@ -52,7 +62,8 @@
     for (int kt = j_lo; kt <= p_last; kt += 32) {
         Frag kh[4], kl[4];
         {
-            const KvT* kp = kb + (int64_t)min(kt + j, p_last) * a.k_row_stride + half * 8;
+            const int kk = min(kt + j, p_last);
+            const KvT* kp = (RAGGED && kk < pre ? pk + (int64_t)kk * 64 : kb + (int64_t)kk * a.k_row_stride) + half * 8;
             if constexpr (KVBF16) {
 #pragma unroll
                 for (int i = 0; i < 4; i++) kh[i].q = *reinterpret_cast<const uint4*>(kp + 16 * i);
@@ -71,7 +82,7 @@
 #pragma unroll
         for (int r = 0; r < 16; r++) {
             const int key = min(kt + (r & 3) + 8 * (r >> 2) + 4 * half, p_last);
-            const KvT* vp = vb + (int64_t)key * a.k_row_stride + j;
+            const KvT* vp = (RAGGED && key < pre ? pv + (int64_t)key * 64 : vb + (int64_t)key * a.k_row_stride) + j;
             if constexpr (KVBF16) {
                 v0[r] = __uint_as_float((unsigned)vp[0] << 16);
                 v1[r] = __uint_as_float((unsigned)vp[32] << 16);
diff --git a/go-pocket-tts_amd/csrc/batch.cpp b/go-pocket-tts_amd/csrc/batch.cpp
--- a/go-pocket-tts_amd/csrc/batch.cpp
+++ b/go-pocket-tts_amd/csrc/batch.cpp
@@ -2,6 +2,7 @@
 
 #include <algorithm>
 #include <cmath>
+#include <cstring>
 
 namespace ptts {
 
@@ -59,6 +60,7 @@
     b->kv_len_host.assign(B, 0);
     b->pre_k.ensure((size_t)B * sizeof(void*)); b->pre_v.ensure((size_t)B * sizeof(void*)); b->pre_len.ensure((size_t)B * sizeof(int32_t));
     b->pre_k_host.assign(B, nullptr); b->pre_v_host.assign(B, nullptr); b->pre_len_host.assign(B, 0);
+    b->pre_in_slot.assign(B, 0);
     const size_t f = sizeof(float);
     const int NA = d.ada_all.out;
     b->in_raw.ensure(B * d.ldim * f); b->in32.ensure(B * d.ldim * f);
@@ -118,12 +120,19 @@
     return b.release();
 }
 
+void batch_reset_host(Batch& b) {
+    b.opened = false;
+    b.kv_bound = 0;
+    std::fill(b.kv_len_host.begin(), b.kv_len_host.end(), 0);
+    std::fill(b.pre_len_host.begin(), b.pre_len_host.end(), 0);
+    b.has_noise = false;
+}
+
 void batch_reset(Batch& b) {
-    b.opened = false;
+    batch_reset_host(b);
     hipStream_t s = b.m->stream;
     const int B = b.B;
     launch_fill_i32(b.st.kv_len, 0, B, s);
-    b.kv_bound = 0;
     PTTS_HIP(hipMemsetAsync(b.latents.p, 0, (size_t)B * b.max_steps * b.m->d.ldim * sizeof(float), s));
     launch_fill_i32(b.st.active, 1, B, s);
     launch_fill_i32(b.st.step, 0, B, s);
@@ -136,10 +145,7 @@
     launch_fill_i32(b.st.n_active, B, 1, s);
     std::vector<float> thr((size_t)B, INFINITY);
     h2d(b.st.eos_threshold, thr.data(), thr.size() * sizeof(float), s);
-    std::fill(b.kv_len_host.begin(), b.kv_len_host.end(), 0);
-    std::fill(b.pre_len_host.begin(), b.pre_len_host.end(), 0);
     launch_fill_i32(b.pre_len.as<int32_t>(), 0, B, s);
-    b.has_noise = false;
 }
 
 static void check_voice(const Desc& d, const float* const* caches, const int64_t* steps, const int64_t* offsets, int64_t cap) {
@@ -178,31 +184,51 @@
                          v.m->d.hd == m.d.hd);
 }
 
-void batch_apply_voice(Batch& b, const Voice& v, const std::vector<int32_t>& slots) {
-    Model& m = *b.m;
-    hipStream_t io = b.io_stream ? b.io_stream : m.stream;
-    const Desc& d = m.d;
-    if (!voice_usable_by(v, m)) throw Error(PTTS_EINVAL, "ptts-hip: voice belongs to another model");
+bool batch_prefix_lazy(const Batch& b) {
+    const Model& m = *b.m;
+    const int D = m.d.d_model;
+    const StepAttnRows rows{b.qkv.as<float>(), 3 * D, D, m.at<float>(m.d.rope_cos), m.at<float>(m.d.rope_sin), b.st.kv_len, b.st.active,
+                            b.pre_k.as<const void*>(), b.pre_v.as<const void*>(), b.pre_len.as<int32_t>(), b.B};
+    static const bool off = [] { const char* e = getenv("PTTS_VOICE_IN_PLACE"); return e && e[0] == '0'; }();
+    return !off && !b.eager_prefix && m.d.hd == 64 && D % 4 == 0 && attn_step_supported(attn_step_args(kv_layer(b, 0), rows, 0, 0, b.attn.as<float>(), D));
+}
+
+void batch_voice_host(Batch& b, const Voice& v, const std::vector<int32_t>& slots) {
+    if (!voice_usable_by(v, *b.m)) throw Error(PTTS_EINVAL, "ptts-hip: voice belongs to another model");
     if (v.offset > b.cap) throw Error(PTTS_EINVAL, "ptts-hip: voice state longer than the KV capacity");
-    DevBuf& ds = m.work(WORK_VOICE_SLOTS, slots.size() * sizeof(int32_t));
-    h2d(ds.p, slots.data(), slots.size() * sizeof(int32_t), io);
-    const size_t lb = v.layer_bytes();
-    for (int l = 0; l < d.n_layers; l++)
-        launch_voice_apply((const char*)v.k.p + lb * l, (const char*)v.v.p + lb * l, v.offset, d.heads, d.hd, ds.as<int32_t>(), (int)slots.size(),
-                           b.kc(l), b.vc(l), (int)b.kv_elem(), b.cap, io);
     for (int32_t sl : slots) {
         b.kv_len_host[sl] = v.offset;
         b.kv_bound = std::max(b.kv_bound, (int)v.offset);
         b.pre_k_host[sl] = v.k.p; b.pre_v_host[sl] = v.v.p; b.pre_len_host[sl] = v.offset;
-    }
-    if (b.slot_local) return;
-    h2d(b.st.kv_len, b.kv_len_host.data(), (size_t)b.B * sizeof(int32_t), io);
-    h2d(b.pre_k.p, b.pre_k_host.data(), (size_t)b.B * sizeof(void*), io);
-    h2d(b.pre_v.p, b.pre_v_host.data(), (size_t)b.B * sizeof(void*), io);
-    h2d(b.pre_len.p, b.pre_len_host.data(), (size_t)b.B * sizeof(int32_t), io);
-}
-
-void batch_set_voice(Batch& b, int slot, const float* const* caches, const int64_t* steps, const int64_t* offsets) {
+        b.pre_in_slot[sl] = 0;
+    }
+}
+
+static void prefix_copy(Batch& b, const void* vk, const void* vv, int offset, const int32_t* slots_dev, int n, hipStream_t s) {
+    const Desc& d = b.m->d;
+    const size_t lb = (size_t)d.heads * offset * d.hd * b.kv_elem();
+    for (int l = 0; l < d.n_layers; l++)
+        launch_voice_apply((const char*)vk + lb * l, (const char*)vv + lb * l, offset, d.heads, d.hd, slots_dev, n, b.kc(l), b.vc(l), (int)b.kv_elem(), b.cap, s);
+}
+
+void batch_voice_copy(Batch& b, const Voice& v, const std::vector<int32_t>& slots, const int32_t* slots_dev) {
+    prefix_copy(b, v.k.p, v.v.p, v.offset, slots_dev, (int)slots.size(), b.io_stream ? b.io_stream : b.m->stream);
+    for (int32_t sl : slots) b.pre_in_slot[sl] = 1;
+}
+
+void batch_materialise_prefix(Batch& b, int slot, hipStream_t s) {
+    for (int sl = slot < 0 ? 0 : slot; sl < (slot < 0 ? b.B : slot + 1); sl++) {
+        if (b.pre_len_host[sl] <= 0 || b.pre_in_slot[sl]) continue;
+        const int32_t one = sl;
+        DevBuf& ds = b.m->work(WORK_VOICE_SLOTS, sizeof one);
+        h2d(ds.p, &one, sizeof one, s);
+        prefix_copy(b, b.pre_k_host[sl], b.pre_v_host[sl], b.pre_len_host[sl], ds.as<int32_t>(), 1, s);
+        PTTS_HIP(hipStreamSynchronize(s));
+        b.pre_in_slot[sl] = 1;
+    }
+}
+
+void batch_set_voice(Batch& b, int slot, const float* const* caches, const int64_t* steps, const int64_t* offsets, bool upload_state) {
     Model& m = *b.m;
     hipStream_t io = b.io_stream ? b.io_stream : m.stream;
     const Desc& d = m.d;
@@ -219,18 +245,15 @@
     b.kv_len_host[slot] = (int32_t)offsets[0];
     b.kv_bound = std::max(b.kv_bound, (int)offsets[0]);
     b.pre_len_host[slot] = 0;
-    if (b.slot_local) return;
+    if (b.slot_local || !upload_state) return;
     h2d(b.st.kv_len + slot, &b.kv_len_host[slot], sizeof(int32_t), io);
     h2d(b.pre_len.as<int32_t>() + slot, &b.pre_len_host[slot], sizeof(int32_t), io);
 }
 
-void batch_prompt(Batch& b, const float* rows_dev, const int64_t* row_offsets) {
-    Model& m = *b.m;
-    const Desc& d = m.d;
-    hipStream_t s = b.io_stream ? b.io_stream : m.stream;
-    const int B = b.B, D = d.d_model;
+RaggedMeta prompt_plan(const Batch& b, const int64_t* row_offsets) {
+    const int B = b.B;
     const int64_t R64 = row_offsets[B];
-    if (R64 == 0) return;
+    if (R64 == 0) return RaggedMeta{};
     if (R64 < 0 || R64 > (1 << 24)) throw Error(PTTS_EINVAL, "ptts-hip: prompt row count out of range");
     const int R = (int)R64;
     std::vector<int32_t> off((size_t)B + 1);
@@ -241,25 +264,54 @@
         off[(size_t)sl] = (int32_t)row_offsets[sl];
     }
     off[(size_t)B] = R;
+    return ragged_meta(off.data(), b.kv_len_host.data(), B);
+}
+
+void batch_prompt(Batch& b, const float* rows_dev, const int64_t* row_offsets) {
+    Model& m = *b.m;
+    hipStream_t s = b.io_stream ? b.io_stream : m.stream;
+    const RaggedMeta meta = prompt_plan(b, row_offsets);
+    if (meta.rows == 0) return;
+    const bool in_place = batch_prefix_lazy(b);
+    if (!in_place) batch_materialise_prefix(b, -1, s);
+    const size_t B = (size_t)b.B, n_off = meta.table.size() * sizeof(int32_t), k_off = (n_off + B * sizeof(int32_t) + 15) & ~(size_t)15, v_off = k_off + B * sizeof(void*);
+    std::vector<char> img(v_off + B * sizeof(void*));
+    std::memcpy(img.data(), meta.table.data(), n_off);
+    for (size_t sl = 0; sl < B; sl++) {
+        const int32_t n = in_place && !b.pre_in_slot[sl] ? b.pre_len_host[sl] : 0;
+        std::memcpy(img.data() + n_off + sl * sizeof n, &n, sizeof n);
+    }
+    std::memcpy(img.data() + k_off, b.pre_k_host.data(), B * sizeof(void*));
+    std::memcpy(img.data() + v_off, b.pre_v_host.data(), B * sizeof(void*));
+    const char* dev = m.work(WORK_PROMPT_META, img.size()).as<char>();
+    h2d(const_cast<char*>(dev), img.data(), img.size(), s);
+    batch_prefill(b, rows_dev, meta, reinterpret_cast<const int32_t*>(dev),
+                  PrefixDev{reinterpret_cast<const int32_t*>(dev + n_off), reinterpret_cast<const void* const*>(dev + k_off), reinterpret_cast<const void* const*>(dev + v_off)});
+    if (!b.slot_local) h2d(b.st.kv_len, b.kv_len_host.data(), (size_t)b.B * sizeof(int32_t), s);
+}
+
+void batch_prefill(Batch& b, const float* rows_dev, const RaggedMeta& meta, const int32_t* d_meta, PrefixDev pre) {
+    Model& m = *b.m;
+    const Desc& d = m.d;
+    hipStream_t s = b.io_stream ? b.io_stream : m.stream;
+    const int B = b.B, D = d.d_model;
+    const int R = meta.rows;
+    if (R == 0) return;
     const size_t f = sizeof(float);
-    const RaggedMeta meta = ragged_meta(off.data(), b.kv_len_host.data(), B);
-    int32_t* d_meta = m.work(WORK_PROMPT_META, meta.table.size() * sizeof(int32_t)).as<int32_t>();
     const int32_t* d_slot = meta.row_seg(d_meta);
     const int32_t* d_pos = meta.row_pos(d_meta);
-    h2d(d_meta, meta.table.data(), meta.table.size() * sizeof(int32_t), s);
     DevBuf& wsb = m.work(WORK_PROMPT_ACT, ((size_t)R * (size_t)(D + D + 3 * D + D + d.ffn)) * f);
     float* px = wsb.as<float>();
     float* pxn = px + (size_t)R * D;
     float* pqkv = pxn + (size_t)R * D;
     float* pattn = pqkv + (size_t)R * 3 * D;
     float* pff = pattn + (size_t)R * D;
-    PTTS_HIP(hipMemcpyAsync(px, rows_dev, (size_t)R * D * f, hipMemcpyDeviceToDevice, s));
     const bool kvb = m.opts.kv == PTTS_KV_BF16;
     PendingSum pend;
     for (int l = 0; l < d.n_layers; l++) {
         const auto& L = d.layers[l];
         {
-            LnArgs ln = mkln(m, px, flat(D), L.n1, pxn, D, R);
+            LnArgs ln = mkln(m, l == 0 ? rows_dev : px, flat(D), L.n1, pxn, D, R);
             ln.pend = pend;
             launch_layernorm(ln, s);
             pend = PendingSum{};
@@ -277,9 +329,9 @@
         }
         launch_kv_append(pqkv, 3 * D, D, d.heads, d.hd, d_slot, d_pos, R, b.kc(l), b.vc(l), kvb, b.cap, s);
         if (l == d.n_layers - 1) break;
-        launch_attention(attn_ragged_args(kv_layer(b, l), meta, d_meta, pqkv, 3 * D, -1, pattn, D), s);
+        launch_attention(attn_ragged_args(kv_layer(b, l), meta, d_meta, pqkv, 3 * D, -1, pattn, D, pre, l), s);
         GemmArgs go = mk(m, pattn, flat(D), L.out_proj, px, flat(D), R);
-        go.R = px; go.epi = EPI_RESADD;
+        go.R = l == 0 ? rows_dev : px; go.epi = EPI_RESADD;
         launch_gemm(go, s);
         launch_layernorm(mkln(m, px, flat(D), L.n2, pxn, D, R), s);
         GemmArgs g1 = mk(m, pxn, flat(D), L.l1, pff, flat(d.ffn), R);
@@ -317,11 +369,11 @@
             launch_gemm(g2, s);
         }
     }
+    const int32_t* rag_off = meta.table.data() + 2 * (size_t)R;
     for (int sl = 0; sl < B; sl++) {
-        b.kv_len_host[sl] += (int32_t)(row_offsets[sl + 1] - row_offsets[sl]);
+        b.kv_len_host[sl] += rag_off[sl + 1] - rag_off[sl];
         b.kv_bound = std::max(b.kv_bound, (int)b.kv_len_host[sl]);
     }
-    if (!b.slot_local) h2d(b.st.kv_len, b.kv_len_host.data(), (size_t)B * sizeof(int32_t), s);
-}
-
-}
+}
+
+}
diff --git a/go-pocket-tts_amd/csrc/capi_hooks.cpp b/go-pocket-tts_amd/csrc/capi_hooks.cpp
--- a/go-pocket-tts_amd/csrc/capi_hooks.cpp
+++ b/go-pocket-tts_amd/csrc/capi_hooks.cpp
@@ -319,6 +319,35 @@
         if (n < 0 || (n > 0 && (!samples || !y))) throw Error(PTTS_EINVAL, "ptts-hip: true peak: null argument");
         (void)tp_measure(samples, n, y);
     });
+}
+
+int ptts_debug_batch_apply_voice(ptts_batch* hb, const ptts_voice* voice, const int32_t* slots, int32_t n, int32_t eager) {
+    return guard([&] {
+        if (!hb || !hb->b || !voice || !slots || n <= 0) throw Error(PTTS_EINVAL, "ptts_debug_batch_apply_voice: null argument");
+        Model& m = *hb->m;
+        Batch& b = *hb->b;
+        const Voice& v = *reinterpret_cast<const Voice*>(voice);
+        std::vector<int32_t> list(slots, slots + n);
+        for (int32_t sl : list) if (sl < 0 || sl >= b.B) throw Error(PTTS_EINVAL, "ptts_debug_batch_apply_voice: slot out of range");
+        const Locked lock(m);
+        if (eager) b.eager_prefix = true;
+        batch_voice_host(b, v, list);
+        if (!batch_prefix_lazy(b)) {
+            Tmp ds(list.size() * sizeof(int32_t));
+            up(ds.p, list.data(), list.size() * sizeof(int32_t));
+            batch_voice_copy(b, v, list, ds.as<int32_t>());
+            PTTS_HIP(hipStreamSynchronize(m.stream));
+        }
+        h2d(b.st.kv_len, b.kv_len_host.data(), (size_t)b.B * sizeof(int32_t), m.stream);
+        h2d(b.pre_k.p, b.pre_k_host.data(), (size_t)b.B * sizeof(void*), m.stream);
+        h2d(b.pre_v.p, b.pre_v_host.data(), (size_t)b.B * sizeof(void*), m.stream);
+        h2d(b.pre_len.p, b.pre_len_host.data(), (size_t)b.B * sizeof(int32_t), m.stream);
+    });
+}
+
+int ptts_debug_batch_prefix_in_slot(ptts_batch* hb, int32_t slot) {
+    if (!hb || !hb->b || slot < 0 || slot >= hb->b->B) return -1;
+    return hb->b->pre_len_host[(size_t)slot] > 0 && hb->b->pre_in_slot[(size_t)slot] ? 1 : 0;
 }
 
 int64_t ptts_debug_launch_counts(int32_t on, char* out, int64_t cap) {
diff --git a/go-pocket-tts_amd/csrc/continuous.cpp b/go-pocket-tts_amd/csrc/continuous.cpp
--- a/go-pocket-tts_amd/csrc/continuous.cpp
+++ b/go-pocket-tts_amd/csrc/continuous.cpp
@@ -236,9 +236,9 @@
         list[(size_t)i] = SlotReq{next, reqs[i], resolve_max_steps(*reqs[i])};
         b.kv_len_host[(size_t)next] = 0;
         b.pre_k_host[(size_t)next] = nullptr; b.pre_v_host[(size_t)next] = nullptr; b.pre_len_host[(size_t)next] = 0;
-    }
-    stage_prompt(b, list, s);
-    stage_noise(b, list, s);
+        b.pre_in_slot[(size_t)next] = 0;
+    }
+    stage_call(b, list, s, true);
     ContEngine::Joining j;
     std::vector<SlotAdmit> adm((size_t)n);
     for (int i = 0; i < n; i++) {
diff --git a/go-pocket-tts_amd/csrc/generate.cpp b/go-pocket-tts_amd/csrc/generate.cpp
--- a/go-pocket-tts_amd/csrc/generate.cpp
+++ b/go-pocket-tts_amd/csrc/generate.cpp
@@ -1,4 +1,4 @@
-#include "runtime.h"
+#include "launch_args.h"
 
 #include <chrono>
 
@@ -7,28 +7,85 @@
 
 namespace ptts {
 
-void stage_prompt(Batch& b, const std::vector<SlotReq>& list, hipStream_t s, hipEvent_t before_prefill) {
+namespace {
+struct CallRecord {
+    std::vector<char> host;
+    size_t put(const void* src, size_t bytes) {
+        const size_t off = (host.size() + 15) & ~(size_t)15;
+        host.resize(off + bytes);
+        if (bytes) std::memcpy(host.data() + off, src, bytes);
+        return off;
+    }
+};
+}
+
+void stage_call(Batch& b, const std::vector<SlotReq>& list, hipStream_t s, bool with_noise, std::vector<SlotAdmit>* init, StageEvents ev) {
     Model& m = *b.m;
-    const int D = m.d.d_model;
-    std::map<const Voice*, std::vector<int32_t>> by_voice;
-    for (const SlotReq& q : list) {
-        if (q.req->voice) by_voice[reinterpret_cast<const Voice*>(q.req->voice)].push_back(q.slot);
-        else if (q.req->voice_caches) batch_set_voice(b, q.slot, q.req->voice_caches, q.req->voice_cache_steps, q.req->voice_offsets);
-    }
-    for (auto& kv : by_voice) batch_apply_voice(b, *kv.first, kv.second);
+    const int D = m.d.d_model, ld = m.d.ldim;
+    CallRecord rec;
+    struct VoiceRun { const Voice* v; std::vector<int32_t> slots; size_t off; };
+    std::vector<VoiceRun> voices;
+    const bool in_place = batch_prefix_lazy(b);
+    {
+        std::map<const Voice*, std::vector<int32_t>> by_voice;
+        for (const SlotReq& q : list) {
+            if (q.req->voice) by_voice[reinterpret_cast<const Voice*>(q.req->voice)].push_back(q.slot);
+            else if (q.req->voice_caches) batch_set_voice(b, q.slot, q.req->voice_caches, q.req->voice_cache_steps, q.req->voice_offsets, init == nullptr);
+        }
+        for (auto& kv : by_voice) {
+            batch_voice_host(b, *kv.first, kv.second);
+            if (!in_place) { const size_t off = rec.put(kv.second.data(), kv.second.size() * sizeof(int32_t)); voices.push_back(VoiceRun{kv.first, kv.second, off}); }
+        }
+    }
     std::vector<int64_t> row_off((size_t)b.B + 1, 0), ids;
     for (const SlotReq& q : list) {
         row_off[(size_t)q.slot + 1] = q.req->n_tokens + (q.req->voice_embedding ? q.req->voice_frames : 0);
         ids.insert(ids.end(), q.req->tokens, q.req->tokens + q.req->n_tokens);
     }
     for (int sl = 0; sl < b.B; sl++) row_off[(size_t)sl + 1] += row_off[(size_t)sl];
+    const size_t ids_off = rec.put(ids.data(), ids.size() * sizeof(int64_t));
+    std::vector<int32_t> pre_n((size_t)b.B);
+    for (int sl = 0; sl < b.B; sl++) pre_n[(size_t)sl] = in_place && !b.pre_in_slot[(size_t)sl] ? b.pre_len_host[(size_t)sl] : 0;
+    const size_t pre_n_off = rec.put(pre_n.data(), pre_n.size() * sizeof(int32_t));
+    const size_t pre_k_off = rec.put(b.pre_k_host.data(), b.pre_k_host.size() * sizeof(void*));
+    const size_t pre_v_off = rec.put(b.pre_v_host.data(), b.pre_v_host.size() * sizeof(void*));
+    const RaggedMeta meta = prompt_plan(b, row_off.data());
+    const size_t meta_off = rec.put(meta.table.data(), meta.table.size() * sizeof(int32_t));
+    size_t spec_off = 0;
+    int draw_rows = 0, steps_most = 0;
+    for (const SlotReq& q : list) steps_most = std::max(steps_most, q.max_steps);
+    if (with_noise) {
+        std::vector<NoiseSpec> spec((size_t)b.B, NoiseSpec{0, 0.0f, 0});
+        for (const SlotReq& q : list) {
+            const ptts_request& r = *q.req;
+            if (r.noise || !(r.temperature > 0.0f)) continue;
+            if (ld % 4) throw Error(PTTS_EINVAL, "ptts-hip: the device noise draw needs a latent width that is a multiple of 4");
+            spec[(size_t)q.slot] = NoiseSpec{r.noise_seed ? r.noise_seed : m.next_noise_seed(), std::sqrt(r.temperature), q.max_steps};
+            draw_rows = std::max(draw_rows, q.max_steps);
+        }
+        if (draw_rows) spec_off = rec.put(spec.data(), spec.size() * sizeof(NoiseSpec));
+    }
+    size_t init_off = 0;
+    if (init) {
+        for (SlotAdmit& a : *init) {
+            const size_t sl = (size_t)a.slot;
+            a.kv_len = b.kv_len_host[sl] + (int32_t)(row_off[sl + 1] - row_off[sl]);
+            a.pre_len = b.pre_len_host[sl]; a.pre_k = b.pre_k_host[sl]; a.pre_v = b.pre_v_host[sl];
+        }
+        init_off = rec.put(init->data(), init->size() * sizeof(SlotAdmit));
+    }
+    const char* dev = m.work(WORK_CALL_RECORD, (rec.host.size() + 4095) & ~(size_t)4095).as<char>();
+    h2d(const_cast<char*>(dev), rec.host.data(), rec.host.size(), s);
+    if (init)
+        launch_call_unpack(b.st, b.pre_len.as<int32_t>(), b.pre_k.as<const void*>(), b.pre_v.as<const void*>(), reinterpret_cast<const SlotAdmit*>(dev + init_off),
+                           (int)init->size(), b.latents.as<float>(), (int64_t)b.max_steps * ld, (int64_t)std::min(steps_most, b.max_steps) * ld, s);
+    for (const VoiceRun& v : voices) batch_voice_copy(b, *v.v, v.slots, reinterpret_cast<const int32_t*>(dev + v.off));
     DevBuf& rows = m.work(WORK_PROMPT_ROWS, (size_t)row_off[(size_t)b.B] * D * sizeof(float));
-    DevBuf& dids = m.work(WORK_PROMPT_IDS, ids.size() * sizeof(int64_t));
-    h2d(dids.p, ids.data(), ids.size() * sizeof(int64_t), s);
+    const int64_t* dids = reinterpret_cast<const int64_t*>(dev + ids_off);
     int64_t id0 = 0, run_id0 = 0, run_n = 0;
     float* run_dst = rows.as<float>();
     auto flush = [&]() {
-        if (run_n > 0) launch_embed_gather(m.at<float>(m.d.embed), dids.as<int64_t>() + run_id0, (int)run_n, D, run_dst, s);
+        if (run_n > 0) launch_embed_gather(m.at<float>(m.d.embed), dids + run_id0, (int)run_n, D, run_dst, s);
         run_n = 0;
     };
     for (const SlotReq& q : list) {
@@ -44,13 +101,11 @@
         id0 += r.n_tokens;
     }
     flush();
-    if (before_prefill) PTTS_HIP(hipEventRecord(before_prefill, s));
-    batch_prompt(b, rows.as<float>(), row_off.data());
-}
-
-void stage_noise(Batch& b, const std::vector<SlotReq>& list, hipStream_t s) {
-    Model& m = *b.m;
-    const int ld = m.d.ldim;
+    if (ev.before_prefill) PTTS_HIP(hipEventRecord(ev.before_prefill, s));
+    batch_prefill(b, rows.as<float>(), meta, reinterpret_cast<const int32_t*>(dev + meta_off),
+                  PrefixDev{reinterpret_cast<const int32_t*>(dev + pre_n_off), reinterpret_cast<const void* const*>(dev + pre_k_off), reinterpret_cast<const void* const*>(dev + pre_v_off)});
+    if (ev.after_prefill) PTTS_HIP(hipEventRecord(ev.after_prefill, s));
+    if (!with_noise) return;
     const int64_t slot_rows = (int64_t)b.max_steps * ld;
     float* noise = b.noise.as<float>();
     for (size_t i = 0; i < list.size();) {
@@ -59,21 +114,9 @@
         PTTS_HIP(hipMemsetAsync(noise + list[i].slot * slot_rows, 0, (j - i) * slot_rows * sizeof(float), s));
         i = j;
     }
-    std::vector<NoiseSpec> spec((size_t)b.B, NoiseSpec{0, 0.0f, 0});
-    int draw_rows = 0;
-    for (const SlotReq& q : list) {
-        const ptts_request& r = *q.req;
-        if (r.noise) h2d(noise + q.slot * slot_rows, r.noise, (size_t)q.max_steps * ld * sizeof(float), s);
-        else if (r.temperature > 0.0f) {
-            if (ld % 4) throw Error(PTTS_EINVAL, "ptts-hip: the device noise draw needs a latent width that is a multiple of 4");
-            spec[(size_t)q.slot] = NoiseSpec{r.noise_seed ? r.noise_seed : m.next_noise_seed(), std::sqrt(r.temperature), q.max_steps};
-            draw_rows = std::max(draw_rows, q.max_steps);
-        }
-    }
-    if (draw_rows == 0) return;
-    DevBuf& sb = m.work(WORK_NOISE_SPECS, spec.size() * sizeof(NoiseSpec));
-    h2d(sb.p, spec.data(), spec.size() * sizeof(NoiseSpec), s);
-    launch_noise_fill(sb.as<NoiseSpec>(), b.B, draw_rows, noise, slot_rows, ld, s);
+    for (const SlotReq& q : list)
+        if (q.req->noise) h2d(noise + q.slot * slot_rows, q.req->noise, (size_t)q.max_steps * ld * sizeof(float), s);
+    if (draw_rows) launch_noise_fill(reinterpret_cast<const NoiseSpec*>(dev + spec_off), b.B, draw_rows, noise, slot_rows, ld, s);
 }
 
 const PcmRow* results_alloc(const Model& m, const std::vector<Delivery>& g, PcmRow* host_rows, PcmRow* dev_rows, hipStream_t s) {
@@ -291,23 +334,16 @@
         m.cached_batch.reset(batch_new(m, B, cap, ms_max));
     }
     b = m.cached_batch.get();
-    batch_reset(*b);
-    std::vector<int32_t> v_ms((size_t)B), v_fae((size_t)B);
-    std::vector<float> v_thr((size_t)B);
-    for (int i = 0; i < B; i++) { v_ms[i] = std::min(list[i].max_steps, t_limit + 1); v_fae[i] = req(i).frames_after_eos; v_thr[i] = req(i).eos_threshold; }
-    h2d(b->st.max_steps, v_ms.data(), (size_t)B * 4, s);
-    h2d(b->st.frames_after_eos, v_fae.data(), (size_t)B * 4, s);
-    h2d(b->st.eos_threshold, v_thr.data(), (size_t)B * 4, s);
+    batch_reset_host(*b);
+    std::vector<SlotAdmit> init((size_t)B);
+    for (int i = 0; i < B; i++) init[(size_t)i] = SlotAdmit{i, std::min(list[i].max_steps, t_limit + 1), req(i).frames_after_eos, req(i).eos_threshold, 0, 0, nullptr, nullptr};
     mark("setup");
     m.prof.phases = false;
-    stage_prompt(*b, list, s, phase_event(0));
-    phase(1, s);
-    mark("prefill");
     b->has_noise = false;
     for (int i = 0; i < B; i++) b->has_noise |= req(i).noise != nullptr || req(i).temperature > 0.0f;
-    if (!b->has_noise) return;
-    b->noise.ensure((size_t)B * b->max_steps * ld * sizeof(float));
-    stage_noise(*b, list, s);
+    if (b->has_noise) b->noise.ensure((size_t)B * b->max_steps * ld * sizeof(float));
+    stage_call(*b, list, s, b->has_noise, &init, StageEvents{phase_event(0), phase_event(1)});
+    mark("prefill");
 }
 
 void Chunk::decoder_setup() {
diff --git a/go-pocket-tts_amd/csrc/kernels.h b/go-pocket-tts_amd/csrc/kernels.h
--- a/go-pocket-tts_amd/csrc/kernels.h
+++ b/go-pocket-tts_amd/csrc/kernels.h
@@ -512,6 +512,8 @@
 void launch_readback_i32(const int32_t* a, int na, const int32_t* b, int nb, int32_t* host, hipStream_t stream);
 struct SlotAdmit { int32_t slot, max_steps, frames_after_eos; float eos_threshold; int32_t kv_len, pre_len; const void* pre_k; const void* pre_v; };
 void launch_slot_admit(const StepState& s, int32_t* pre_len, const void** pre_k, const void** pre_v, const SlotAdmit* dev, int n, hipStream_t stream);
+void launch_call_unpack(const StepState& s, int32_t* pre_len, const void** pre_k, const void** pre_v, const SlotAdmit* dev, int n, float* latents,
+                        int64_t lat_stride, int64_t zero_words, hipStream_t stream);
 void launch_slot_retire(const StepState& s, const int32_t* slots_dev, int n, hipStream_t stream);
 void launch_fill_i32(int32_t* p, int32_t v, int n, hipStream_t stream);
 void launch_add_i32(int32_t* p, const int32_t* inc, int n, hipStream_t stream);
diff --git a/go-pocket-tts_amd/csrc/kernels.hip b/go-pocket-tts_amd/csrc/kernels.hip
--- a/go-pocket-tts_amd/csrc/kernels.hip
+++ b/go-pocket-tts_amd/csrc/kernels.hip
@@ -240,6 +240,7 @@
     if (i < n) p[i] = v;
 }
 void launch_fill_i32(int32_t* p, int32_t v, int n, hipStream_t stream) {
+    note_launch("k_fill_i32");
     hipLaunchKernelGGL(k_fill_i32, dim3((n + 255) / 256), dim3(256), 0, stream, p, v, n);
 }
 __global__ void k_add_i32(int32_t* p, const int32_t* inc, int n) {
@@ -250,17 +251,45 @@
     hipLaunchKernelGGL(k_add_i32, dim3((n + 255) / 256), dim3(256), 0, stream, p, inc, n);
 }
 
+__device__ __forceinline__ void slot_admit_one(const StepState& s, int32_t* pre_len, const void** pre_k, const void** pre_v, const SlotAdmit& a) {
+    const int sl = a.slot;
+    s.kv_len[sl] = a.kv_len; pre_len[sl] = a.pre_len; pre_k[sl] = a.pre_k; pre_v[sl] = a.pre_v;
+    s.active[sl] = 1; s.step[sl] = 0; s.countdown[sl] = -1; s.n_frames[sl] = 0; s.eos_step[sl] = -1; s.broke[sl] = 0;
+    s.max_steps[sl] = a.max_steps; s.frames_after_eos[sl] = a.frames_after_eos; s.eos_threshold[sl] = a.eos_threshold;
+}
 __global__ void k_slot_admit(StepState s, int32_t* pre_len, const void** pre_k, const void** pre_v, const SlotAdmit* a, int n) {
     const int i = blockIdx.x * blockDim.x + threadIdx.x;
     if (i >= n) return;
-    const int sl = a[i].slot;
-    s.kv_len[sl] = a[i].kv_len; pre_len[sl] = a[i].pre_len; pre_k[sl] = a[i].pre_k; pre_v[sl] = a[i].pre_v;
-    s.active[sl] = 1; s.step[sl] = 0; s.countdown[sl] = -1; s.n_frames[sl] = 0; s.eos_step[sl] = -1; s.broke[sl] = 0;
-    s.max_steps[sl] = a[i].max_steps; s.frames_after_eos[sl] = a[i].frames_after_eos; s.eos_threshold[sl] = a[i].eos_threshold;
+    slot_admit_one(s, pre_len, pre_k, pre_v, a[i]);
     if (i == 0) atomicAdd(s.n_active, n);
 }
 void launch_slot_admit(const StepState& s, int32_t* pre_len, const void** pre_k, const void** pre_v, const SlotAdmit* dev, int n, hipStream_t stream) {
     if (n > 0) hipLaunchKernelGGL(k_slot_admit, dim3((n + 63) / 64), dim3(64), 0, stream, s, pre_len, pre_k, pre_v, dev, n);
+}
+__global__ __launch_bounds__(256) void k_call_unpack(StepState s, int32_t* pre_len, const void** pre_k, const void** pre_v, const SlotAdmit* a, int n,
+                                                     float* latents, int64_t lat_stride, int64_t zero_words) {
+    const SlotAdmit rec = a[blockIdx.x];
+    if (blockIdx.y == 0 && threadIdx.x == 0) {
+        slot_admit_one(s, pre_len, pre_k, pre_v, rec);
+        if (blockIdx.x == 0) *s.n_active = n;
+    }
+    float* row = latents + (int64_t)rec.slot * lat_stride;
+    const int64_t tid = (int64_t)blockIdx.y * 256 + threadIdx.x, nth = (int64_t)gridDim.y * 256;
+    int64_t done = 0;
+    if (lat_stride % 4 == 0) {
+        const int64_t n4 = zero_words / 4;
+        for (int64_t i = tid; i < n4; i += nth) reinterpret_cast<float4*>(row)[i] = make_float4(0.f, 0.f, 0.f, 0.f);
+        done = n4 * 4;
+    }
+    for (int64_t i = done + tid; i < zero_words; i += nth) row[i] = 0.f;
+}
+void launch_call_unpack(const StepState& s, int32_t* pre_len, const void** pre_k, const void** pre_v, const SlotAdmit* dev, int n, float* latents,
+                        int64_t lat_stride, int64_t zero_words, hipStream_t stream) {
+    if (n <= 0) return;
+    note_launch("k_call_unpack");
+    const int parts = (int)std::min<int64_t>(16, std::max<int64_t>(1, (zero_words + 4095) / 4096));
+    hipLaunchKernelGGL(k_call_unpack, dim3((unsigned)n, (unsigned)parts), dim3(256), 0, stream, s, pre_len, pre_k, pre_v, dev, n, latents, lat_stride,
+                       zero_words);
 }
 __global__ void k_slot_retire(StepState s, const int32_t* slots, int n) {
     const int i = blockIdx.x * blockDim.x + threadIdx.x;
@@ -322,6 +351,7 @@
                       hipStream_t stream) {
     int64_t tot = (int64_t)rows * d_model;
     if (tot <= 0) return;
+    note_launch("k_kv_append");
     dim3 g((unsigned)((tot + 255) / 256));
     if (kv_bf16) hipLaunchKernelGGL(k_kv_append<true>, g, dim3(256), 0, stream, qkv, ld, d_model, heads, hd, row_slot, row_pos, rows, kcache, vcache, cap);
     else hipLaunchKernelGGL(k_kv_append<false>, g, dim3(256), 0, stream, qkv, ld, d_model, heads, hd, row_slot, row_pos, rows, kcache, vcache, cap);
@@ -636,7 +666,8 @@
     int row16 = hd * elem_bytes / 16;
     int64_t tot = (int64_t)heads * offset * row16 * n_slots;
     if (tot <= 0) return;
-    hipLaunchKernelGGL(k_voice_apply, dim3((unsigned)((tot + 255) / 256)), dim3(256), 0, stream, (const uint4*)vk, (const uint4*)vv, offset,
+    note_launch("k_voice_apply");
+    hipLaunchKernelGGL(k_voice_apply,dim3((unsigned)((tot + 255) / 256)), dim3(256), 0, stream, (const uint4*)vk, (const uint4*)vv, offset,
                        heads, row16, slots, n_slots, (uint4*)kcache, (uint4*)vcache, cap);
 }
 
diff --git a/go-pocket-tts_amd/csrc/launch_args.h b/go-pocket-tts_amd/csrc/launch_args.h
--- a/go-pocket-tts_amd/csrc/launch_args.h
+++ b/go-pocket-tts_amd/csrc/launch_args.h
@@ -86,7 +86,9 @@
     std::copy(pos0, pos0 + segs, row_pos + t.rows + segs + 1);
     return t;
 }
-inline AttnArgs attn_ragged_args(const KvLayer& c, const RaggedMeta& t, const int32_t* meta_dev, const float* q, int64_t q_ld, int context, float* out, int64_t out_ld) {
+struct PrefixDev { const int32_t* len = nullptr; const void* const* k = nullptr; const void* const* v = nullptr; };
+inline AttnArgs attn_ragged_args(const KvLayer& c, const RaggedMeta& t, const int32_t* meta_dev, const float* q, int64_t q_ld, int context, float* out, int64_t out_ld,
+                                 PrefixDev pre = PrefixDev{}, int layer = 0) {
     AttnArgs a;
     attn_on_cache(a, c);
     a.q = q; a.q_ld = q_ld; a.q_col0 = 0;
@@ -95,6 +97,7 @@
     a.context = context;
     a.out = out; a.out_ld = out_ld;
     a.rows = t.rows; a.max_keys = t.max_pos + 1;
+    a.pre_len = pre.len; a.pre_k = pre.k; a.pre_v = pre.v; a.layer = layer;
     return a;
 }
 
diff --git a/go-pocket-tts_amd/csrc/runtime.h b/go-pocket-tts_amd/csrc/runtime.h
--- a/go-pocket-tts_amd/csrc/runtime.h
+++ b/go-pocket-tts_amd/csrc/runtime.h
@@ -80,6 +80,7 @@
     WORK_NOISE_SPECS = 12,
     WORK_NOISE_ROWS_SPEC = 12,
     WORK_CONT_RESERVE = 13,
+    WORK_CALL_RECORD = 14,
     WORK_CONT_RETIRE = 15,
     WORK_ENCODER = 16,
     WORK_ENCODER_LATENTS = 17,
@@ -231,6 +232,8 @@
     DevBuf pre_k, pre_v, pre_len;
     std::vector<const void*> pre_k_host, pre_v_host;
     std::vector<int32_t> pre_len_host;
+    std::vector<uint8_t> pre_in_slot;
+    bool eager_prefix = false;
     DevBuf in_raw, in32, x, xn, qkv, attn, ff, last, eos, sy, ada, fx, fh, fh2, cur, noise_step, partial;
     DevBuf latents;
     DevBuf noise;
@@ -278,7 +281,10 @@
     size_t layer_bytes() const { return (size_t)m->d.heads * offset * m->d.hd * (m->opts.kv == PTTS_KV_BF16 ? 2 : 4); }
 };
 Voice* voice_create(Model& m, const float* const* caches, const int64_t* steps, const int64_t* offsets);
-void batch_apply_voice(Batch& b, const Voice& v, const std::vector<int32_t>& slots);
+void batch_voice_host(Batch& b, const Voice& v, const std::vector<int32_t>& slots);
+void batch_voice_copy(Batch& b, const Voice& v, const std::vector<int32_t>& slots, const int32_t* slots_dev);
+bool batch_prefix_lazy(const Batch& b);
+void batch_materialise_prefix(Batch& b, int slot, hipStream_t s);
 bool voice_usable_by(const Voice& v, const Model& m);
 std::vector<std::unique_ptr<Voice>> voice_build(Model& m, const float* const* emb, const int64_t* frames, int64_t width, int n);
 void voice_export(const Voice& v, int layer0, int n_layers, float* out);
@@ -314,8 +320,13 @@
 void profile_read(Model& m, ptts_profile* out);
 Batch* batch_new(Model& m, int n_slots, int cap, int max_steps);
 void batch_reset(Batch& b);
-void batch_set_voice(Batch& b, int slot, const float* const* caches, const int64_t* steps, const int64_t* offsets);
+void batch_reset_host(Batch& b);
+void batch_set_voice(Batch& b, int slot, const float* const* caches, const int64_t* steps, const int64_t* offsets, bool upload_state = true);
 void batch_prompt(Batch& b, const float* rows_dev, const int64_t* row_offsets);
+struct RaggedMeta;
+struct PrefixDev;
+RaggedMeta prompt_plan(const Batch& b, const int64_t* row_offsets);
+void batch_prefill(Batch& b, const float* rows_dev, const RaggedMeta& meta, const int32_t* meta_dev, PrefixDev pre);
 bool step_core(Batch& b, int lsd_steps, bool opened = false, bool fuse_finish = false, bool chain = false);
 void step_open(Batch& b);
 struct FlowClusterFault : Error { using Error::Error; };
@@ -334,8 +345,8 @@
 bool open_linears(Batch& b, StepOpenLinears& lin);
 void mimi_zero_history(Model& m, MimiWs& w, hipStream_t s);
 struct SlotReq { int slot; const ptts_request* req; int max_steps; };
-void stage_prompt(Batch& b, const std::vector<SlotReq>& list, hipStream_t s, hipEvent_t before_prefill = nullptr);
-void stage_noise(Batch& b, const std::vector<SlotReq>& list, hipStream_t s);
+struct StageEvents { hipEvent_t before_prefill = nullptr, after_prefill = nullptr; };
+void stage_call(Batch& b, const std::vector<SlotReq>& list, hipStream_t s, bool with_noise, std::vector<SlotAdmit>* init = nullptr, StageEvents ev = StageEvents{});
 struct Delivery {
     const ptts_request* req = nullptr;
     ptts_result* res = nullptr;
@@ -411,7 +422,7 @@
 void staged_text_embeddings(Model& m, const int64_t* ids, int64_t n, float* out);
 void staged_prompt(Batch& b, const float* emb, const int64_t* row_offsets);
 void staged_step(Batch& b, const float* frames_in, int lsd_steps, const float* noise, float* frames_out, float* eos_logits, float* last_hidden);
-void staged_read_kv(const Batch& b, int slot, int layer, float* k, float* v);
+void staged_read_kv(Batch& b, int slot, int layer, float* k, float* v);
 void staged_decode(Model& m, const float* latents, int n_utt, int frames, float* pcm, float* mimi_latent, float* transformer_out);
 void staged_noise_rows(Model& m, uint64_t seed, float temperature, int rows, float* out);
 void staged_flow_direction(Model& m, const float* c, float sv, float tv, const float* x, int n, float* out);
diff --git a/go-pocket-tts_amd/csrc/staged.cpp b/go-pocket-tts_amd/csrc/staged.cpp
--- a/go-pocket-tts_amd/csrc/staged.cpp
+++ b/go-pocket-tts_amd/csrc/staged.cpp
@@ -56,8 +56,9 @@
     PTTS_HIP(hipStreamSynchronize(s));
 }
 
-void staged_read_kv(const Batch& b, int slot, int layer, float* k, float* v) {
+void staged_read_kv(Batch& b, int slot, int layer, float* k, float* v) {
     const Desc& d = b.m->d;
+    batch_materialise_prefix(b, slot, b.m->stream);
     const int n = b.kv_len_host[slot];
     const size_t es = b.kv_elem();
     std::vector<uint8_t> tmp((size_t)n * d.hd * es);
diff --git a/go-pocket-tts_amd/runtime.py b/go-pocket-tts_amd/runtime.py
--- a/go-pocket-tts_amd/runtime.py
+++ b/go-pocket-tts_amd/runtime.py
@@ -251,7 +251,7 @@
     "ptts_dsp_ext_set_formant",
     ]
 HOOK_SYMBOLS = [
-    "ptts_decode_stages", "ptts_mimi_layer_piece", "ptts_debug_last_attention_kernel", "ptts_debug_launch_counts", "ptts_debug_flow_cluster_inject",
+    "ptts_decode_stages", "ptts_mimi_layer_piece", "ptts_debug_last_attention_kernel", "ptts_debug_launch_counts", "ptts_debug_batch_apply_voice", "ptts_debug_batch_prefix_in_slot", "ptts_debug_flow_cluster_inject",
     "ptts_debug_time_skinny", "ptts_debug_skinny_stamps", "ptts_debug_gemm", "ptts_debug_step_stamps", "ptts_debug_tall",
     "ptts_debug_encode_stages", "ptts_debug_resample_launches", "ptts_debug_dsp_blocked_host",
     "ptts_debug_loudness_energies", "ptts_debug_kweighting", "ptts_debug_step_linear", "ptts_debug_true_peak_taps", "ptts_debug_true_peak_oversample",
@@ -428,6 +428,8 @@
         H = C.CDLL(HOOKS_PATH, mode=C.RTLD_GLOBAL)
         H.ptts_decode_stages.argtypes = [C.c_void_p, _FP, C.c_int32, C.c_int32, _FP, _FP, _FP]
         H.ptts_debug_last_attention_kernel.restype = C.c_char_p
+        H.ptts_debug_batch_apply_voice.argtypes = [C.c_void_p, C.c_void_p, C.POINTER(C.c_int32), C.c_int32, C.c_int32]
+        H.ptts_debug_batch_prefix_in_slot.argtypes = [C.c_void_p, C.c_int32]
         H.ptts_debug_launch_counts.restype = C.c_int64
         H.ptts_debug_launch_counts.argtypes = [C.c_int32, C.c_char_p, C.c_int64]
         H.ptts_mimi_layer_piece.argtypes = [C.c_void_p, C.c_int32, C.c_int32, _FP, C.c_int64, C.c_int32, C.c_int32, _FP]
@@ -1305,6 +1307,13 @@
     def set_voice_state(self, slot: int, state: VoiceModelState):
         ptrs, steps, offs, arrs = _voice_arrays(state, self.model.info.n_layers)
         _check(lib().ptts_batch_set_voice_state(self.h, slot, ptrs, _ip(steps), _ip(offs)))
+
+    def apply_voice(self, voice: "DeviceVoice", slots, eager: bool = False):
+        s = np.ascontiguousarray(slots, np.int32)
+        _check(hooks().ptts_debug_batch_apply_voice(self.h, voice.h, s.ctypes.data_as(C.POINTER(C.c_int32)), len(s), 1 if eager else 0))
+
+    def prefix_in_slot(self, slot: int) -> bool:
+        return hooks().ptts_debug_batch_prefix_in_slot(self.h, slot) == 1
 
     def prompt(self, embs: Sequence[np.ndarray]):
         d = self.model.info.d_model
diff --git a/include/ptts_debug.h b/include/ptts_debug.h
--- a/include/ptts_debug.h
+++ b/include/ptts_debug.h
@@ -128,6 +128,8 @@
 const char* ptts_debug_last_attention_kernel(void);
 
 int64_t ptts_debug_launch_counts(int32_t on, char* out, int64_t cap);
+int ptts_debug_batch_apply_voice(ptts_batch* b, const ptts_voice* voice, const int32_t* slots, int32_t n, int32_t eager);
+int ptts_debug_batch_prefix_in_slot(ptts_batch* b, int32_t slot);
 int64_t ptts_debug_resample_launches(int32_t reset);
 
 int ptts_debug_dsp_blocked_host(const float* in, int64_t n, float* out);
```

New measurement: 12790 x real-time. Within noise of the previous version (-0.1%).
